# revdotcom/reverb

Hardware: AMD Instinct MI355X
Metric: RTFx (audio-sec/wall-sec) Reverb-ASR attention_rescoring (higher is better)
Workload: dtype bf16

## Files before the change

reverb_amd/_lib.py:

```python
from __future__ import annotations

import ctypes as C
import os

_HERE = os.path.dirname(os.path.abspath(__file__))
LIB_PATH = os.path.join(_HERE, "librvb.so")

RVB_F32, RVB_BF16, RVB_FP8 = 0, 1, 2
ACT_NONE, ACT_SILU, ACT_RELU = 0, 1, 2
NORM_LN, NORM_AFFINE = 0, 1


class RvbError(RuntimeError):
    pass


class AudioInfo(C.Structure):
    _fields_ = [("container", C.c_int32), ("sample_format", C.c_int32), ("channels", C.c_int32), ("sample_rate", C.c_int32),
                ("bits_per_sample", C.c_int32), ("md5_checked", C.c_int32), ("frames", C.c_int64), ("decode_threads", C.c_int32),
                ("reserved", C.c_int32)]


class _SizedCfg(C.Structure):

# ... 51 lines not shown
    "rvb_audio_decode_i16": (C.c_int64, [C.c_void_p, C.c_int64, C.c_int, _i16p, C.c_int64, C.c_int, C.POINTER(AudioInfo)]),
    "rvb_fbank": (C.c_int, [_eng, _f32p, _i64p]),
    "rvb_encode": (C.c_int, [_eng, _f32p, C.c_int64, _i32p, C.c_int, C.c_int, C.c_int, C.c_float]),
    "rvb_stream_begin": (C.c_int, [_eng]),
    "rvb_stream_chunk": (C.c_int, [_eng, _f32p, C.c_int, C.c_int, _f32p, _i32p]),
    "rvb_stream_state": (C.c_int, [_eng, _i32p, _i32p]),
    "rvb_stream_finish": (C.c_int, [_eng, C.c_int, C.c_float]),
    "rvb_encoder_frames": (C.c_int, [_eng, _i32p]),
    "rvb_get_encoder_lens": (C.c_int, [_eng, _i32p]),
    "rvb_get_encoder_out": (C.c_int, [_eng, _f32p]),
    "rvb_get_ctc_logprobs": (C.c_int, [_eng, C.c_int, _f32p]),
    "rvb_set_encoder_tap": (C.c_int, [_eng, C.c_int]),
    "rvb_get_encoder_tap": (C.c_int, [_eng, C.c_char_p, _f32p, C.c_int64]),
    "rvb_get_ctc_topk": (C.c_int, [_eng, _f32p, _i32p]),
    "rvb_ctc_greedy": (C.c_int, [_eng, _i32p, _i32p, _i32p]),
    "rvb_ctc_align": (C.c_int, [_eng, _i32p, _i32p, C.c_int, _i32p, _i32p, _i32p, _i32p, _i32p, _i32p, _f32p, _f32p]),
    "rvb_ctc_align_wild": (C.c_int, [_eng, _i32p, _i32p, C.c_int, _i32p, _i32p, C.c_float, _i32p, _i32p, _i32p, _i32p, _f32p, _f32p]),
    "rvb_ctc_align_limits": (C.c_int, [_i32p, _i32p]),
    "rvb_ctc_align_graph": (C.c_int, [_eng, _i32p, _i32p, _i32p, _i32p, _u8p, C.c_int, _i32p, _i32p, C.c_float, _i32p, _i32p, _i32p, _i32p,
                                      _i32p, _i32p, _i32p, _f32p, _f32p]),
    "rvb_ctc_align_graph_limits": (C.c_int, [_i32p, _i32p, _i32p, _i32p]),
    "rvb_ctc_score": (C.c_int, [_eng, _i32p, _i32p, C.c_int, _i32p, _i32p, _f64p, _f32p, _f32p, _f32p, _i32p]),
    "rvb_ctc_score_graph": (C.c_int, [_eng, _i32p, _i32p, _i32p, _i32p, _u8p, C.c_int, _i32p, _i32p, _f64p, _f32p, _f32p, _f32p, _f32p,
                                      _i32p]),
    "rvb_ctc_find": (C.c_int, [_eng, _i32p, _i32p, C.c_int, _f32p, _i32p, _i32p, C.c_int, C.c_int, C.c_int, _i32p, _i32p, _i32p, _f32p,
                               _i64p]),
    "rvb_ctc_prefix_beam": (C.c_int, [_eng, C.c_int]),
    "rvb_set_context_graph": (C.c_int, [_eng, _i32p, _i32p, C.c_int, C.c_double]),
    "rvb_get_nbest_count": (C.c_int, [_eng, C.c_int, _i32p, _i32p]),
    "rvb_get_nbest": (C.c_int, [_eng, C.c_int, _i32p, _i32p, _i32p, _i32p, _f64p]),
    "rvb_prepare_rescoring": (C.c_int, [_eng, C.c_int]),
    "rvb_attention_rescore": (C.c_int, [_eng, C.c_double, C.c_double]),
    "rvb_attention_score": (C.c_int, [_eng, _i32p, _i32p, C.c_int, _i32p, C.c_double, C.c_double, _f64p, _f64p, _i32p, _i32p, _f32p, _f32p,
                                      _i32p]),
    "rvb_attention_decode": (C.c_int, [_eng, C.c_int, C.c_float]),
    "rvb_get_attention_result": (C.c_int, [_eng, C.c_int, _i32p, _i32p, _f32p]),
    "rvb_get_rescored": (C.c_int, [_eng, C.c_int, _i32p, _f32p, _f64p, _f64p]),
    "rvb_get_rescored_batch": (C.c_int, [_eng, _i32p, _i32p, _i32p, _i32p, _f32p, _f64p, _f64p]),
    "rvb_fp8_recalibrate": (C.c_int, [_eng]),
    "rvb_get_fp8_scales": (C.c_int, [_eng, _f32p, _i32p]),
    "rvb_set_fp8_scales": (C.c_int, [_eng, _f32p, C.c_int32]),
    "rvb_get_fp8_saturation": (C.c_int, [_eng, C.POINTER(C.c_uint32), _i32p, C.c_int]),
    "rvb_get_fp8_subsample": (C.c_int, [_eng, C.POINTER(C.c_float), C.POINTER(C.c_uint32), C.c_int]),
    "rvb_get_rescore_stats": (C.c_int, [_eng, _i64p, _i64p]),
    "rvb_get_rescore_logp": (C.c_int, [_eng, C.c_int, C.c_int, C.c_int, _f32p]),
    "rvb_comm_unique_id": (C.c_int, [C.c_void_p]),
    "rvb_comm_init": (C.c_int, [_eng, C.c_int, C.c_int, C.c_void_p]),
    "rvb_comm_create": (C.c_int, [C.c_int, C.c_int, C.c_int, C.c_void_p, C.POINTER(C.c_void_p)]),
    "rvb_comm_allgather": (C.c_int, [C.c_void_p, C.c_void_p, C.c_int64, C.c_void_p]),
    "rvb_comm_time_allgather": (C.c_int, [C.c_void_p, C.c_int64, C.c_int, C.POINTER(C.c_double)]),
    "rvb_comm_set_timeout": (C.c_int, [C.c_void_p, C.c_double]),
    "rvb_comm_barrier": (C.c_int, [C.c_void_p]),
    "rvb_comm_max_f64": (C.c_int, [C.c_void_p, C.POINTER(C.c_double)]),
    "rvb_comm_allgather_topk": (C.c_int, [C.c_void_p, _eng, C.c_void_p, _i64p]),
    "rvb_comm_free": (C.c_int, [C.c_void_p]),
    "rvb_allgather_results": (C.c_int, [_eng, C.c_void_p, C.c_int64, C.c_void_p]),
    "rvb_comm_destroy": (C.c_int, [_eng]),
    "rvb_set_profiling": (C.c_int, [_eng, C.c_int]),
    "rvb_reset_timings": (C.c_int, [_eng]),
    "rvb_get_timing": (C.c_int, [_eng, C.c_char_p, _f64p, _f64p, _i64p]),
    "rvb_get_timing_bytes": (C.c_int, [_eng, C.c_char_p, _f64p]),
    "rvb_wer_counts": (C.c_int, [_i32p, C.c_int64, _i32p, C.c_int64, _i64p]),
}

class AttnTestArgs(C.Structure):
    _fields_ = ([(n, C.c_int32) for n in ("dtype", "heads", "dk", "nseq")] +
                [f for b in ("q", "k", "v", "out") for f in ((b, _f32p), (b[0] + "_rows", C.c_int32), (b[0] + "_stride", C.c_int32),
                                                             (b[0] + "_col", C.c_int32), ("pad_" + b, C.c_int32))] +
                [("p", _f32p), ("p_rows", C.c_int32), ("p_stride", C.c_int32), ("p_col", C.c_int32), ("p_off", C.c_int32),
                 ("bias_u", _f32p), ("bias_v", _f32p)] +
                [(n, _i32p) for n in ("q_start", "q_len", "kv_start", "kv_len", "q_pos0", "kv_index", "work")] +
                [(n, C.c_int32) for n in ("n_index", "n_work", "max_q", "q_block", "causal", "chunk", "left", "plain_order", "fold",
                                          "k_prefolded", "fold_kv_cap", "lab")] +
                [("ran", C.c_int32 * 8)])


class NormTestArgs(C.Structure):
    _fields_ = ([(n, C.c_int32) for n in ("dtype", "x_bf16", "mode", "silu", "out_f32", "out_fp8", "out2_fp8", "M", "d", "pad0")] +
                [(n, C.c_float) for n in ("eps", "eps2", "out_scale", "out2_scale")] +
                [(n, _f32p) for n in ("x", "gamma", "beta", "add", "gamma2", "beta2", "out", "out2")] +
                [("sat", C.c_uint32), ("sat2", C.c_uint32)])


class GemmTestArgs(C.Structure):
    _fields_ = ([(n, C.c_int32) for n in ("dtype", "M", "N", "K", "lda", "ldw", "ldc", "ldres", "act", "out_f32", "out_fp8", "in_fp8",
                                          "inplace", "a_row0", "c_rows", "conv", "cT1", "cF1", "cC", "cB")] +
                [(n, C.c_float) for n in ("alpha", "a_scale", "out_scale")] +
                [("path", C.c_int32), ("a_elems", C.c_int64)] +
                [(n, _f32p) for n in ("A", "W", "bias", "res", "C", "a_deq", "w_deq")])


_u32p = C.POINTER(C.c_uint32)

TEST_SIGNATURES = {
    "rvb_test_gemm_ex": (C.c_int, [C.POINTER(GemmTestArgs)]),
    "rvb_test_rownorm_ex": (C.c_int, [C.POINTER(NormTestArgs)]),
    "rvb_test_conv1_ex": (C.c_int, [C.c_int, _f32p, _f32p, _f32p, _f32p, _f32p, _f32p, C.c_int, C.c_int, C.c_int, C.c_int, C.c_float,
                                    _f32p, _u32p]),
    "rvb_test_embed": (C.c_int, [_f32p, C.c_int, _f32p, C.c_int, _i32p, _i32p, _f32p, C.c_int, C.c_int, C.c_float]),
    "rvb_test_amax_abs": (C.c_int, [C.c_int, _f32p, C.c_int64, _f32p]),
    "rvb_test_convert_f32": (C.c_int, [C.c_int, _f32p, _f32p, C.c_int64]),
    "rvb_test_gather_cache": (C.c_int, [C.c_void_p, C.c_void_p, _i32p, C.c_int, C.c_int, C.c_int, C.c_int]),
    "rvb_test_gather_pairs": (C.c_int, [_f32p, C.c_int, C.c_int64, _i32p, _i32p, C.c_int, _f32p]),
    "rvb_test_gemm": (C.c_int, [C.c_int, _f32p, _f32p, _f32p, _f32p, _f32p, C.c_int, C.c_int, C.c_int, C.c_float,
                                C.c_int, C.c_int, C.c_int, C.c_int, C.c_int, C.c_int, C.c_int]),
    "rvb_test_rownorm": (C.c_int, [C.c_int, _f32p, _f32p, _f32p, C.c_float, C.c_int, C.c_int, _f32p, _f32p, C.c_int,
                                   C.c_int, C.c_int]),
    "rvb_test_conv_block32": (C.c_int, [_f32p, _f32p, _f32p, _f32p, _f32p, _f32p, C.c_int, C.c_int, C.c_int]),
    "rvb_test_conv_s2sc": (C.c_int, [_f32p, _f32p, _f32p, _f32p, _f32p, _f32p, _f32p, C.c_int, C.c_int, C.c_int]),
    "rvb_test_conv1": (C.c_int, [C.c_int, _f32p, _f32p, _f32p, _f32p, _f32p, _f32p, C.c_int, C.c_int, C.c_int, C.c_int]),
    "rvb_test_conv_igemm_fp8": (C.c_int, [_f32p, _f32p, _f32p, _f32p, _f32p, _f32p, C.c_int, C.c_int, C.c_int, C.c_int, C.c_int, C.c_int, C.c_int,
                                           C.c_float, C.c_float, _f32p, _f32p, _f32p]),
    "rvb_test_joint_new": (C.c_void_p, [C.c_int, C.c_int, C.c_int, C.c_int, C.c_double, C.c_double, C.c_double]),
    "rvb_test_joint_free": (None, [C.c_void_p]),
    "rvb_test_joint_begin": (C.c_int, [C.c_void_p, C.c_int, _f32p, _i32p, C.c_int, C.c_float, C.c_float, _i32p, _i32p, _i32p, _i32p, _i32p,
                                       C.c_int]),
    "rvb_test_joint_finish": (C.c_int, [C.c_void_p, _f32p]),
    "rvb_test_joint_prefix": (C.c_int, [C.c_void_p, C.c_int, _i32p, _i32p]),
    "rvb_test_joint_result": (C.c_int, [C.c_void_p, _i32p, _i32p, _i32p, _f64p, _i32p, _f64p]),
    "rvb_test_glu_dwconv": (C.c_int, [C.c_int, _f32p, _f32p, _f32p, _f32p, _i32p, _f32p, C.c_int, C.c_int, C.c_int,
                                      C.c_int, C.c_int, _f32p, C.c_int]),
    "rvb_test_attention": (C.c_int, [C.c_int, _f32p, _f32p, _f32p, _f32p, _f32p, _f32p, _f32p, C.c_int, C.c_int,
                                     C.c_int, C.c_int, C.c_int, _i32p, _i32p, _i32p, _i32p, C.c_int, C.c_int]),
    "rvb_test_attention_trie": (C.c_int, [C.c_int, _f32p, _f32p, _f32p, _f32p, C.c_int, C.c_int, C.c_int, _i32p, _i32p, _i32p,
                                          _i32p, _i32p, _i32p, C.c_int, C.c_int, C.c_int]),
    "rvb_test_attention_ex": (C.c_int, [C.POINTER(AttnTestArgs)]),
    "rvb_test_attention_pos_bias": (C.c_int, [_f32p, C.c_int, C.c_int, C.c_int, C.c_int, _f32p, _f32p, C.c_int, C.c_int, C.c_float, _f32p]),
    "rvb_test_logsoftmax_topk": (C.c_int, [_f32p, C.c_int, C.c_int, C.c_int, C.c_float, C.c_int, _f32p, _i32p, _f32p]),
    "rvb_test_lse_gather": (C.c_int, [_f32p, C.c_int, C.c_int, _i32p, _f32p]),
    "rvb_test_logsoftmax_topk_ex": (C.c_int, [_f32p, C.c_int, C.c_int, C.c_int, C.c_int, C.c_float, C.c_int, _f32p, _i32p, _f32p]),
    "rvb_test_lse_gather_ex": (C.c_int, [_f32p, C.c_int, C.c_int, C.c_int, _i32p, C.c_float, C.c_int, _f32p]),
    "rvb_test_lse_gather_multi_ex": (C.c_int, [_f32p, C.c_int, C.c_int, C.c_int, _i32p, _i32p, _f32p]),
    "rvb_test_ctc_viterbi": (C.c_int, [_f32p, C.c_int, C.c_int, _i32p, C.c_int, C.c_int, C.c_int, _i32p, _f32p]),
    "rvb_test_ctc_viterbi_wild": (C.c_int, [_f32p, C.c_int, C.c_int, _f32p, C.c_float, _i32p, C.c_int, C.c_int, C.c_int, _i32p, _f32p]),
    "rvb_test_ctc_viterbi_graph": (C.c_int, [_f32p, _i32p, C.c_int, C.c_int, _f32p, C.c_float, _i32p, _i32p, _i32p, _i32p, _u8p, C.c_int,
                                             C.c_int, _i32p, _i32p, _f32p]),
    "rvb_test_ctc_score": (C.c_int, [_f32p, C.c_int, C.c_int, _i32p, C.c_int, C.c_int, C.c_int, _f64p, _f32p, _f32p, _f32p, _i32p]),
    "rvb_test_ctc_score_graph": (C.c_int, [_f32p, _i32p, C.c_int, C.c_int, _i32p, _i32p, _i32p, _i32p, _u8p, C.c_int, C.c_int, _f64p, _f32p,
                                           _f32p, _f32p, _f32p, _i32p]),
    "rvb_test_ctc_score_batch": (C.c_int, [_f32p, _i32p, C.c_int, _i32p, _i32p, C.c_int, C.c_int, C.c_int, _f64p, _f32p, _f32p, _f32p,
                                           _i32p]),
    "rvb_test_ctc_find": (C.c_int, [_f32p, _i32p, C.c_int, C.c_int, _f32p, _i32p, _i32p, C.c_int, _f32p, C.c_int, C.c_int, C.c_int, C.c_int,
                                    _i64p, _i32p, _i32p, _f32p, _i32p, _i32p, _i32p, _f32p]),
    "rvb_test_slab_windows": (C.c_int, [C.c_char_p, _i32p, _i32p, C.c_int, _i32p, C.c_int, C.c_int, _i32p, _i32p, _i32p, _i32p, _i32p]),
    "rvb_test_gemm_glu": (C.c_int, [_f32p, _f32p, _f32p, _f32p, C.c_int, C.c_int, C.c_int]),
    "rvb_test_gemm_rowadd": (C.c_int, [_f32p, _f32p, _f32p, _f32p, _f32p, C.c_int, C.c_int, C.c_int, C.c_int, C.c_int, C.c_int]),
    "rvb_test_mp3_decode": (C.c_int64, [C.c_char_p, C.c_int64, C.c_int, _f32p, C.c_int64, _i64p, _i64p, C.c_int]),
    "rvb_test_mp3_hybrid": (C.c_int, [_f32p, _f32p, C.c_int, C.c_int, _f32p]),
    "rvb_test_mp3_polyphase": (C.c_int, [_f32p, _f32p, _i32p, _f32p]),
    "rvb_test_mp3_window": (C.c_int, [_f32p]),
    "rvb_test_mp3_huffman": (C.c_int, [C.c_int, C.POINTER(C.c_uint16), C.POINTER(C.c_uint8), _i32p]),
    "rvb_test_gemm_fp8": (C.c_int, [_f32p, _f32p, _f32p, _f32p, _f32p, C.c_int, C.c_int, C.c_int, C.c_float, C.c_float, C.c_int, C.c_int,
                                    C.c_float, _f32p, _f32p]),
    "rvb_test_rownorm_fp8": (C.c_int, [_f32p, _f32p, _f32p, C.c_float, C.c_int, C.c_int, C.c_int, C.c_float, _f32p, _f32p, _f32p,
                                       C.c_float, C.c_float, _f32p, _f32p]),
    "rvb_test_lse_gather_multi": (C.c_int, [_f32p, C.c_int, C.c_int, _i32p, _i32p, C.c_int, _f32p]),
    "rvb_test_row_xent": (C.c_int, [_f32p, C.c_int, C.c_int, C.c_int, _i32p, _i32p, _f32p, _f32p, _f64p, _i32p]),
    "rvb_test_host_pool": (C.c_int, [C.c_int, C.c_int, C.c_int]),
    "rvb_test_build_trie": (C.c_int, [_i32p, _i32p, _i32p, C.c_int, C.c_int, C.c_int, C.c_int, C.c_int, _i32p, _i32p, _i32p, _i32p, _i32p, _i32p,
                                      _i32p, _i32p, _i32p, _i32p, _i32p]),
    "rvb_test_fbank": (C.c_int, [_i16p, C.c_int64, _f32p]),
    "rvb_test_fbank_ex": (C.c_int, [_i16p, _f32p, C.c_int64, _f32p]),
    "rvb_test_fbank_batch": (C.c_int, [C.POINTER(C.c_void_p), _i32p, _i64p, _i64p, C.c_int, C.c_int, _f32p]),
    "rvb_test_set_gemm_variant": (C.c_int, [C.c_int]),
    "rvb_test_set_gemm2_opts": (C.c_int, [C.c_int, C.c_int]),
    "rvb_test_gemm_timeline": (C.c_int, [C.c_int] * 6 + [C.POINTER(C.c_longlong), C.c_int, _i32p]),
    "rvb_test_gemm_bench": (C.c_int, [C.c_int, C.c_int, C.c_int, C.c_int, C.c_int, C.c_int, C.c_int, C.c_int, C.c_int,
                                      _f64p, _f64p]),
    "rvb_test_prefix_beam": (C.c_int, [_f32p, _i32p, C.c_int, C.c_int, C.c_int, _i32p, _i32p, _i32p, _i32p, _i32p,
                                       _f64p]),
    "rvb_test_prefix_beam_context": (C.c_int, [_f32p, _i32p, C.c_int, C.c_int, C.c_int, C.c_int, _i32p, _i32p, C.c_int, C.c_double,
                                               _i32p, _i32p, _i32p, _i32p, _i32p, _f64p, _f64p]),
    "rvb_test_context_walk": (C.c_int, [_i32p, _i32p, C.c_int, C.c_double, C.c_int, C.c_int, _i32p, C.c_int, _i32p, _f64p, _i32p,
                                        _f64p]),
    "rvb_test_window_stats": (C.c_int, [_f32p, C.c_int64, C.c_int64, C.c_int, C.c_int64, C.c_int, C.c_float, _f32p]),
    "rvb_test_sinc_conv": (C.c_int, [C.c_int, _f32p, C.c_int64, _f32p, C.c_int, C.c_int, C.c_int, C.c_int64, _f32p]),
    "rvb_test_pool_norm": (C.c_int, [C.c_int, C.c_int, _f32p, C.c_int, C.c_int, C.c_int, C.c_int, C.c_int, _f32p, _f32p, C.c_float,
                                     C.c_int, _f32p, C.c_int64, C.c_int64, C.c_int, _f32p, _f32p, C.c_float, C.c_float, _f32p]),
    "rvb_test_conv1d5": (C.c_int, [C.c_int, _f32p, C.c_int64, _f32p, _f32p, _f32p, C.c_int64]),
# ... 124 lines not shown
```

reverb_amd/csrc/common.h:

```cpp
#pragma once
#include <hip/hip_runtime.h>
#include <math.h>
#include <stdint.h>
#include <stdio.h>
#include <string>

namespace rvb {

typedef uint16_t bf16_t;

typedef __attribute__((ext_vector_type(8))) __bf16 bf16x8_t;
typedef __attribute__((ext_vector_type(4))) float f32x4_t;

__host__ __device__ inline float bf16_to_f32(bf16_t v) {
  union { uint32_t u; float f; } x;
  x.u = ((uint32_t)v) << 16;
  return x.f;
}
__host__ __device__ inline bf16_t f32_to_bf16(float f) {
#if defined(__HIP_DEVICE_COMPILE__)
  const __bf16 r = (__bf16)f;
  return __builtin_bit_cast(bf16_t, r);
#else
  union { uint32_t u; float f; } x;
// ... 38 lines not shown
  }
  int M = (int)nearbyintf((m * 2.f - 1.f) * 8.f);
  if (M == 8) { M = 0; E += 1; }
  if (E > 15 || (E == 15 && M == 7)) return sgn | 0x7e;
  return sgn | (uint8_t)((E << 3) | M);
}
__host__ __device__ inline float fp8_to_f32_host(uint8_t b) {
  const int E = (b >> 3) & 15, M = b & 7;
  const float v = E == 0 ? ldexpf((float)M, -9) : ldexpf(1.f + M / 8.f, E - 7);
  return (b & 0x80) ? -v : v;
}

template <typename T> struct Cvt;
template <> struct Cvt<float> {
  __host__ __device__ static inline float to_f32(float v) { return v; }
  __host__ __device__ static inline float from_f32(float v) { return v; }
};
template <> struct Cvt<fp8_t> {
  __host__ __device__ static inline float to_f32(fp8_t v) { return fp8_to_f32_host(v); }
  __host__ __device__ static inline fp8_t from_f32(float v) { return f32_to_fp8_host(v); }
};
template <> struct Cvt<bf16_t> {
  __host__ __device__ static inline float to_f32(bf16_t v) { return bf16_to_f32(v); }
  __host__ __device__ static inline bf16_t from_f32(float v) { return f32_to_bf16(v); }
};

template <typename T> struct Mma16;
template <> struct Mma16<bf16_t> {
  static constexpr int KC = 32;
  static constexpr int VE = 8;
  __device__ static inline void run(const uint4& a, const uint4& b, f32x4_t& c) {
    union U { uint4 u; bf16x8_t v; };
    U ua, ub;
    ua.u = a; ub.u = b;
    c = __builtin_amdgcn_mfma_f32_16x16x32_bf16(ua.v, ub.v, c, 0, 0, 0);
  }
};
template <> struct Mma16<float> {
  static constexpr int KC = 16;
  static constexpr int VE = 4;
  __device__ static inline void run(const uint4& a, const uint4& b, f32x4_t& c) {
    c = __builtin_amdgcn_mfma_f32_16x16x4f32(__uint_as_float(a.x), __uint_as_float(b.x), c, 0, 0, 0);
    c = __builtin_amdgcn_mfma_f32_16x16x4f32(__uint_as_float(a.y), __uint_as_float(b.y), c, 0, 0, 0);
    c = __builtin_amdgcn_mfma_f32_16x16x4f32(__uint_as_float(a.z), __uint_as_float(b.z), c, 0, 0, 0);
    c = __builtin_amdgcn_mfma_f32_16x16x4f32(__uint_as_float(a.w), __uint_as_float(b.w), c, 0, 0, 0);
  }
};

__device__ inline float wave_sum(float v) {
#pragma unroll
  for (int o = 32; o > 0; o >>= 1) v += __shfl_xor(v, o, 64);
  return v;
}
__device__ inline float wave_max(float v) {
#pragma unroll
  for (int o = 32; o > 0; o >>= 1) v = fmaxf(v, __shfl_xor(v, o, 64));
  return v;
}

__device__ inline float rows_max(float v) {
  auto a = __builtin_amdgcn_permlane16_swap(__float_as_uint(v), __float_as_uint(v), false, false);
  v = fmaxf(__uint_as_float(a[0]), __uint_as_float(a[1]));
  auto b = __builtin_amdgcn_permlane32_swap(__float_as_uint(v), __float_as_uint(v), false, false);
  return fmaxf(__uint_as_float(b[0]), __uint_as_float(b[1]));
}
__device__ inline float rows_sum(float v) {
  auto a = __builtin_amdgcn_permlane16_swap(__float_as_uint(v), __float_as_uint(v), false, false);
  v = __uint_as_float(a[0]) + __uint_as_float(a[1]);
  auto b = __builtin_amdgcn_permlane32_swap(__float_as_uint(v), __float_as_uint(v), false, false);
  return __uint_as_float(b[0]) + __uint_as_float(b[1]);
}

template <int CTRL> __device__ inline float dpp_f32(float v) {
  return __uint_as_float(__builtin_amdgcn_update_dpp(0u, __float_as_uint(v), CTRL, 0xf, 0xf, false));
}
__device__ inline float wave_sum_dpp(float v) {
  v += dpp_f32<0xB1>(v);
  v += dpp_f32<0x4E>(v);
  v += dpp_f32<0x141>(v);
  v += dpp_f32<0x140>(v);
  return rows_sum(v);
}

inline int cdiv(int64_t a, int64_t b) { return (int)((a + b - 1) / b); }

enum { OK = 0, E_ARG = -1, E_HIP = -2, E_STATE = -3, E_NOMEM = -4, E_UNSUPPORTED = -5, E_TIMEOUT = -7  };

}

#define RVB_HIP_CHECK(expr)                                                             \
  do {                                                                                  \
    hipError_t _e = (expr);                                                             \
    if (_e != hipSuccess) {                                                             \
      rvb::set_error(std::string(#expr) + ": " + hipGetErrorString(_e));                \
      return rvb::E_HIP;                                                                \
    }                                                                                   \
  } while (0)

#define RVB_TRY(expr) do { int _r = (expr); if (_r != rvb::OK) return _r; } while (0)

namespace rvb {
void set_error(const std::string& msg);
const char* last_error();
const char* lab_env(const char* name);
}
```

reverb_amd/csrc/elementwise.hip:

```cpp
#include <algorithm>

#include "common.h"
#include "kernels.h"

namespace rvb {

static constexpr int CONV1_ROWS = 4;

template <typename T>
__global__ __launch_bounds__(256) void conv1_kernel(const float* __restrict__ feats, const float* __restrict__ mean,
                                                    const float* __restrict__ istd, const float* __restrict__ w,
                                                    const float* __restrict__ bias, T* __restrict__ out, int T0,
                                                    int F0, int T1, int F1, int d, float inv_scale, unsigned* __restrict__ amax,
                                                    unsigned* __restrict__ sat) {
  extern __shared__ float s_in[];
  const int t1_0 = blockIdx.x * CONV1_ROWS, b = blockIdx.y;
  const int nrow = min(CONV1_ROWS, T1 - t1_0);
  for (int i = threadIdx.x; i < (2 * nrow + 1) * F0; i += 256) {
    const int kh = i / F0, f = i - kh * F0;
    s_in[i] = (feats[((size_t)b * T0 + 2 * t1_0 + kh) * F0 + f] - mean[f]) * istd[f];
  }
  __syncthreads();
  const int ncg = d >> 3;
  const int per = ncg < 256 ? ncg : 256;
// ... 18 lines not shown
      for (int f1 = fslot; f1 < F1; f1 += nslots) {
        float xin[9];
#pragma unroll
        for (int kh = 0; kh < 3; ++kh)
#pragma unroll
          for (int kw = 0; kw < 3; ++kw) xin[kh * 3 + kw] = in[kh * F0 + 2 * f1 + kw];
        float o[8];
        if constexpr (sizeof(T) == 4) {
#pragma unroll
          for (int c = 0; c < 8; ++c) {
            float acc = br[c];
#pragma unroll
            for (int k = 0; k < 9; ++k) acc += wr[c][k] * xin[k];
            o[c] = fmaxf(acc, 0.f);
          }
        } else {
          typedef float c1_f32x2 __attribute__((ext_vector_type(2)));
#pragma unroll
          for (int c = 0; c < 8; c += 2) {
            c1_f32x2 acc = {br[c], br[c + 1]};
#pragma unroll
            for (int k = 0; k < 9; ++k) acc = __builtin_elementwise_fma((c1_f32x2){wr[c][k], wr[c + 1][k]}, (c1_f32x2){xin[k], xin[k]}, acc);
            o[c] = fmaxf(acc.x, 0.f); o[c + 1] = fmaxf(acc.y, 0.f);
          }
        }
        T* dst = orow + (size_t)f1 * d + cg * 8;
        if (amax) {
#pragma unroll
          for (int c = 0; c < 8; ++c) vmax = fmaxf(vmax, o[c]);
        }
        if constexpr (sizeof(T) == 1) {
#pragma unroll
          for (int c = 0; c < 8; ++c) o[c] *= inv_scale;
          if (sat) nclip += fp8_clipped(o[0], o[1], o[2], o[3]) + fp8_clipped(o[4], o[5], o[6], o[7]);
          *(uint2*)dst = make_uint2(pack4_fp8(o[0], o[1], o[2], o[3]), pack4_fp8(o[4], o[5], o[6], o[7]));
        } else if constexpr (sizeof(T) == 2) {
          *(uint4*)dst = make_uint4(pack2_bf16(o[0], o[1]), pack2_bf16(o[2], o[3]), pack2_bf16(o[4], o[5]), pack2_bf16(o[6], o[7]));
        } else {
          ((float4*)dst)[0] = make_float4(o[0], o[1], o[2], o[3]);
          ((float4*)dst)[1] = make_float4(o[4], o[5], o[6], o[7]);
        }
      }
    }
  }
  if (amax) {
    vmax = wave_max(vmax);
    if ((threadIdx.x & 63) == 0 && vmax > 0.f) atomicMax(amax, __float_as_uint(vmax));
  }
  if (sat && nclip) atomicAdd(sat, nclip);
}

int subsample_conv1(hipStream_t s, int dtype, const float* feats, const float* mean, const float* istd,
                    const float* w, const float* b, void* out, int B, int T0, int F0, int d, float out_fp8_scale, unsigned* amax,
                    unsigned* sat) {
  const int T1 = (T0 - 3) / 2 + 1, F1 = (F0 - 3) / 2 + 1;
  if (B <= 0 || T1 <= 0) return OK;
  if (d % 8) { set_error("subsample_conv1: d must be a multiple of 8"); return E_ARG; }
  dim3 grid(cdiv(T1, CONV1_ROWS), B);
  const size_t sh = (2 * CONV1_ROWS + 1) * F0 * sizeof(float);
  if (out_fp8_scale > 0.f) {
    if (dtype != DT_BF16) { set_error("subsample_conv1: fp8 output belongs to the bf16 engine"); return E_ARG; }
    hipLaunchKernelGGL(conv1_kernel<fp8_t>, grid, dim3(256), sh, s, feats, mean, istd, w, b, (fp8_t*)out, T0, F0, T1, F1, d,
                       1.f / out_fp8_scale, (unsigned*)nullptr, sat);
  } else if (dtype == DT_BF16)
    hipLaunchKernelGGL(conv1_kernel<bf16_t>, grid, dim3(256), sh, s, feats, mean, istd, w, b, (bf16_t*)out, T0, F0, T1, F1, d, 1.f, amax,
                       (unsigned*)nullptr);
  else
    hipLaunchKernelGGL(conv1_kernel<float>, grid, dim3(256), sh, s, feats, mean, istd, w, b, (float*)out, T0, F0, T1, F1, d, 1.f, amax,
                       (unsigned*)nullptr);
  RVB_HIP_CHECK(hipGetLastError());
  return OK;
}

template <int NV>
__device__ inline float sq4(float dx, float dy, float dz, float dw) {
  if constexpr (NV == 4) {
#pragma clang fp contract(off)
    return dx * dx + dy * dy + dz * dz + dw * dw;
  } else {
    return fmaf(dw, dw, fmaf(dz, dz, fmaf(dx, dx, dy * dy)));
  }
}

template <typename OutT, typename AddT, int NV, bool TWO, int SW>
__global__ __launch_bounds__(256, (NV <= 4 ? 4 : 2)) void rownorm_kernel(NormArgs a) {
  constexpr bool CT = SW >= 0;
  auto wsum = [](float x) __attribute__((always_inline)) { if constexpr (sizeof(AddT) == 2) return wave_sum_dpp(x); else return wave_sum(x); };
  const bool sw_xb = CT ? (bool)(SW & 1) : (bool)a.x_bf16;
  const bool sw_ln = CT ? (bool)(SW & 2) : a.mode == NORM_LN;
  const bool sw_silu = CT ? (bool)(SW & 4) : (bool)a.silu;
  const bool sw_add = CT ? (bool)(SW & 8) : a.add != nullptr;
  const bool sw_o2f8 = CT ? (bool)(SW & 16) : (bool)a.out2_fp8;
  const int lane = threadIdx.x & 63;
  const int d = a.d;
  const int wave0 = blockIdx.x * 4 + (threadIdx.x >> 6), nwaves = gridDim.x * 4;
#define COL(i) ((((lane) + 64 * ((i) >> 1)) << 3) + (((i) & 1) << 2))
  float4 g[NV], be[NV], g2[TWO ? NV : 1], be2[TWO ? NV : 1];
#pragma unroll
  for (int i = 0; i < NV; ++i) {
    const int c = COL(i);
    const bool ok = c < d;
    g[i] = ok ? *(const float4*)(a.gamma + c) : make_float4(0.f, 0.f, 0.f, 0.f);
    be[i] = ok ? *(const float4*)(a.beta + c) : make_float4(0.f, 0.f, 0.f, 0.f);
    if constexpr (TWO) {
      g2[i] = ok ? *(const float4*)(a.gamma2 + c) : make_float4(0.f, 0.f, 0.f, 0.f);
      be2[i] = ok ? *(const float4*)(a.beta2 + c) : make_float4(0.f, 0.f, 0.f, 0.f);
    }
  }
  auto load_row = [&](int row, float4* v) {
    const int rr = min(row, a.M - 1);
    const bool rok = row < a.M;
    if (sw_xb) {
      const bf16_t* x = (const bf16_t*)a.x + (size_t)rr * d;
#pragma unroll
      for (int i = 0; i < NV; ++i) {
        const int c = COL(i);
        const uint2 u = *(const uint2*)(x + min(c, d - 4));
        const bool ok = rok && c < d;
        v[i] = make_float4(ok ? bf16_to_f32((bf16_t)(u.x & 0xffffu)) : 0.f, ok ? bf16_to_f32((bf16_t)(u.x >> 16)) : 0.f,
                           ok ? bf16_to_f32((bf16_t)(u.y & 0xffffu)) : 0.f, ok ? bf16_to_f32((bf16_t)(u.y >> 16)) : 0.f);
      }
      return;
    }
    const float* x = a.x + (size_t)rr * d;
#pragma unroll
    for (int i = 0; i < NV; ++i) {
      const int c = COL(i);
      const float4 u = *(const float4*)(x + min(c, d - 4));
      const bool ok = rok && c < d;
      v[i] = make_float4(ok ? u.x : 0.f, ok ? u.y : 0.f, ok ? u.z : 0.f, ok ? u.w : 0.f);
    }
  };
  float4 v[NV], nx[NV];
  unsigned nsat = 0, nsat2 = 0;
  load_row(wave0, v);
  for (int row = wave0; row < a.M; row += nwaves) {
    load_row(row + nwaves, nx);
    float mean = 0.f, rstd = 1.f;
    if (sw_ln) {
      float sum = 0.f;
#pragma unroll
      for (int i = 0; i < NV; ++i) sum += v[i].x + v[i].y + v[i].z + v[i].w;
      mean = wsum(sum) / (float)d;
      float sq = 0.f;
#pragma unroll
      for (int i = 0; i < NV; ++i) {
        if (COL(i) < d) {
          sq += sq4<NV>(v[i].x - mean, v[i].y - mean, v[i].z - mean, v[i].w - mean);
        }
      }
      rstd = rsqrtf(wsum(sq) / (float)d + a.eps);
    }
    if constexpr (CT) {
#pragma unroll
      for (int i = 0; i < NV; ++i)
        asm volatile("" : "+v"(nx[i].x), "+v"(nx[i].y), "+v"(nx[i].z), "+v"(nx[i].w), "+v"(rstd));
    }
    OutT* out = (OutT*)a.out + (size_t)row * d;
    const AddT* add = sw_add ? (const AddT*)a.add + (size_t)row * d : nullptr;
    float sum2 = 0.f;
#pragma unroll
    for (int i = 0; i < NV; ++i) {
      const int c = COL(i);
      if (c >= d) continue;
      float o[4] = {(v[i].x - mean) * rstd * g[i].x + be[i].x, (v[i].y - mean) * rstd * g[i].y + be[i].y,
                    (v[i].z - mean) * rstd * g[i].z + be[i].z, (v[i].w - mean) * rstd * g[i].w + be[i].w};
      if (sw_silu) {
#pragma unroll
        for (int e = 0; e < 4; ++e) {
          if constexpr (sizeof(OutT) <= 2) o[e] = o[e] * __builtin_amdgcn_rcpf(1.0f + __builtin_amdgcn_exp2f(-1.44269504f * o[e]));
          else o[e] = o[e] / (1.0f + expf(-o[e]));
        }
      }
      if (add) {
        if constexpr (sizeof(AddT) == 2) {
          const uint2 u = *(const uint2*)(add + c);
          o[0] += bf16_to_f32((bf16_t)(u.x & 0xffffu)); o[1] += bf16_to_f32((bf16_t)(u.x >> 16));
          o[2] += bf16_to_f32((bf16_t)(u.y & 0xffffu)); o[3] += bf16_to_f32((bf16_t)(u.y >> 16));
        } else {
          const float4 u = *(const float4*)(add + c);
          o[0] += u.x; o[1] += u.y; o[2] += u.z; o[3] += u.w;
        }
      }
      if constexpr (sizeof(OutT) == 4) *(float4*)(out + c) = make_float4(o[0], o[1], o[2], o[3]);
      v[i] = make_float4(o[0], o[1], o[2], o[3]);
      sum2 += o[0] + o[1] + o[2] + o[3];
    }
    if constexpr (sizeof(OutT) <= 2) {
#pragma unroll
      for (int i = 0; i < NV; i += 2) {
        const int c = COL(i);
        if (c >= d) continue;
        if constexpr (sizeof(OutT) == 1) {
          const float qs = a.out_inv_scale;
          nsat += fp8_clipped(v[i].x * qs, v[i].y * qs, v[i].z * qs, v[i].w * qs) + fp8_clipped(v[i + 1].x * qs, v[i + 1].y * qs, v[i + 1].z * qs, v[i + 1].w * qs);
          *(uint2*)(out + c) = make_uint2(pack4_fp8(v[i].x * qs, v[i].y * qs, v[i].z * qs, v[i].w * qs),
                                          pack4_fp8(v[i + 1].x * qs, v[i + 1].y * qs, v[i + 1].z * qs, v[i + 1].w * qs));
        } else {
          *(uint4*)(out + c) = make_uint4(pack2_bf16(v[i].x, v[i].y), pack2_bf16(v[i].z, v[i].w),
                                          pack2_bf16(v[i + 1].x, v[i + 1].y), pack2_bf16(v[i + 1].z, v[i + 1].w));
        }
      }
    }
    if constexpr (TWO) {
      const float mean2 = wsum(sum2) / (float)d;
      float sq = 0.f;
#pragma unroll
      for (int i = 0; i < NV; ++i) {
        if (COL(i) < d) {
          sq += sq4<NV>(v[i].x - mean2, v[i].y - mean2, v[i].z - mean2, v[i].w - mean2);
        }
      }
      const float rstd2 = rsqrtf(wsum(sq) / (float)d + a.eps2);
      AddT* o2 = (AddT*)a.out2 + (size_t)row * d;
#pragma unroll
      for (int i = 0; i < NV; i += 2) {
        const int c = COL(i);
        if (c >= d) continue;
        float q[8];
#pragma unroll
        for (int h = 0; h < 2; ++h) {
          q[4 * h + 0] = (v[i + h].x - mean2) * rstd2 * g2[i + h].x + be2[i + h].x;
          q[4 * h + 1] = (v[i + h].y - mean2) * rstd2 * g2[i + h].y + be2[i + h].y;
          q[4 * h + 2] = (v[i + h].z - mean2) * rstd2 * g2[i + h].z + be2[i + h].z;
          q[4 * h + 3] = (v[i + h].w - mean2) * rstd2 * g2[i + h].w + be2[i + h].w;
        }
        if (sw_o2f8) {
          const float qs = a.out2_inv_scale;
          nsat2 += fp8_clipped(q[0] * qs, q[1] * qs, q[2] * qs, q[3] * qs) + fp8_clipped(q[4] * qs, q[5] * qs, q[6] * qs, q[7] * qs);
          *(uint2*)((fp8_t*)a.out2 + (size_t)row * d + c) = make_uint2(pack4_fp8(q[0] * qs, q[1] * qs, q[2] * qs, q[3] * qs),
                                                                       pack4_fp8(q[4] * qs, q[5] * qs, q[6] * qs, q[7] * qs));
        } else if constexpr (sizeof(AddT) == 2) {
          *(uint4*)(o2 + c) = make_uint4(pack2_bf16(q[0], q[1]), pack2_bf16(q[2], q[3]), pack2_bf16(q[4], q[5]), pack2_bf16(q[6], q[7]));
        } else {
          *(float4*)(o2 + c) = make_float4(q[0], q[1], q[2], q[3]);
          *(float4*)(o2 + c + 4) = make_float4(q[4], q[5], q[6], q[7]);
        }
      }
    }
#pragma unroll
    for (int i = 0; i < NV; ++i) v[i] = nx[i];
  }
  if (nsat != 0 && a.sat) atomicAdd(a.sat, nsat);
  if (nsat2 != 0 && a.sat2) atomicAdd(a.sat2, nsat2);
#undef COL
}

template <typename OutT, typename AddT>
static void launch_rownorm(hipStream_t s, const NormArgs& a) {
  const int blocks = std::min(cdiv(a.M, 4), 256 * 8);
  const int sw = (a.x_bf16 ? 1 : 0) | (a.mode == NORM_LN ? 2 : 0) | (a.silu ? 4 : 0) | (a.add ? 8 : 0) | (a.out2_fp8 ? 16 : 0);
  if (a.d > 512 && a.d <= 1024) {
#define RVB_NORM_CASE(TWO_, SW_) \
    if ((a.out2 != nullptr) == (TWO_) && sw == (SW_)) { hipLaunchKernelGGL((rownorm_kernel<OutT, AddT, 4, TWO_, SW_>), dim3(blocks), dim3(256), 0, s, a); return; }
    RVB_NORM_CASE(false, 2)
    RVB_NORM_CASE(false, 2 | 4 | 1)
    RVB_NORM_CASE(false, 4 | 1)
    RVB_NORM_CASE(false, 2 | 4)
    RVB_NORM_CASE(false, 4)
    RVB_NORM_CASE(true, 2)
    RVB_NORM_CASE(true, 2 | 8)
    RVB_NORM_CASE(true, 2 | 16)
    RVB_NORM_CASE(true, 2 | 8 | 16)
#undef RVB_NORM_CASE
  }
  if (a.out2) {
    if (a.d <= 512) hipLaunchKernelGGL((rownorm_kernel<OutT, AddT, 2, true, -1>), dim3(blocks), dim3(256), 0, s, a);
    else if (a.d <= 1024) hipLaunchKernelGGL((rownorm_kernel<OutT, AddT, 4, true, -1>), dim3(blocks), dim3(256), 0, s, a);
    else hipLaunchKernelGGL((rownorm_kernel<OutT, AddT, 8, true, -1>), dim3(blocks), dim3(256), 0, s, a);
  } else {
    if (a.d <= 512) hipLaunchKernelGGL((rownorm_kernel<OutT, AddT, 2, false, -1>), dim3(blocks), dim3(256), 0, s, a);
    else if (a.d <= 1024) hipLaunchKernelGGL((rownorm_kernel<OutT, AddT, 4, false, -1>), dim3(blocks), dim3(256), 0, s, a);
    else hipLaunchKernelGGL((rownorm_kernel<OutT, AddT, 8, false, -1>), dim3(blocks), dim3(256), 0, s, a);
  }
}

int rownorm(hipStream_t s, int dtype, const NormArgs& a) {
  if (a.M <= 0) return OK;
  if (a.d % 8 || a.d > 2048) { set_error("rownorm: d must be a multiple of 8 and <= 2048"); return E_ARG; }
  if (a.x_bf16 && dtype != DT_BF16) { set_error("rownorm: bf16 input belongs to the bf16 engine"); return E_ARG; }
  if (a.out2 && (a.mode != NORM_LN || !(a.out_f32 || dtype == DT_F32))) {
    set_error("rownorm: the fused second LayerNorm follows a LayerNorm with fp32 output"); return E_ARG;
  }
  if ((a.out_fp8 || a.out2_fp8) && dtype != DT_BF16) { set_error("rownorm: fp8 outputs belong to the bf16 engine"); return E_ARG; }
  if (dtype == DT_BF16) {
    if (a.out_fp8) launch_rownorm<fp8_t, bf16_t>(s, a);
    else if (a.out_f32) launch_rownorm<float, bf16_t>(s, a);
    else launch_rownorm<bf16_t, bf16_t>(s, a);
  } else {
    launch_rownorm<float, float>(s, a);
  }
  RVB_HIP_CHECK(hipGetLastError());
  return OK;
}

static constexpr int DW_TT = 128, DW_CT = 128, DW_KMAX = 31, DW_THREADS = 512;

template <typename T> struct Gate;
template <> struct Gate<float> {
  typedef float2 pair_t;
  __device__ static inline float put(float v) { return v; }
  __device__ static inline void get(pair_t p, float& x, float& y) { x = p.x; y = p.y; }
};
template <> struct Gate<bf16_t> {
  typedef uint32_t pair_t;
  __device__ static inline bf16_t put(float v) { return f32_to_bf16(v); }
  __device__ static inline void get(pair_t p, float& x, float& y) { x = __uint_as_float(p << 16); y = __uint_as_float(p & 0xffff0000u); }
};

template <typename T>
__global__ __launch_bounds__(DW_THREADS) void glu_dw_kernel(GluDwArgs a) {
  typedef decltype(Gate<T>::put(0.f)) S;
  constexpr int rows = DW_TT + DW_KMAX - 1;
  __shared__ __attribute__((aligned(16))) S s_g[rows][DW_CT];
  const int c = threadIdx.x & 63, slot = threadIdx.x >> 6;
  const int t0 = blockIdx.x * DW_TT, c0 = blockIdx.y * DW_CT, b = blockIdx.z;
  const int ch = c0 + 2 * c;
  const bool cok = ch < a.d;
  const int K = a.K, pad = a.causal ? K - 1 : (K - 1) / 2;
  const int len = a.lens[b];
  const int lorder = K - 1;
  const T* G = (const T*)a.G;
  const bool gated = a.gated != 0;
  const size_t gstride = gated ? (size_t)a.d : (size_t)2 * a.d;
  typedef float f32x2_t __attribute__((ext_vector_type(2)));
  f32x2_t wk[DW_KMAX];
#pragma unroll
  for (int k = 0; k < DW_KMAX; ++k)
    wk[k] = (k < K && cok) ? *(const f32x2_t*)(a.dw_w + (size_t)k * a.d + ch) : (f32x2_t){0.f, 0.f};
  constexpr int VE = 16 / (int)sizeof(T);
  constexpr int NG = DW_CT / VE;
  const bool vec_ok = (a.d % VE) == 0;
  if (vec_ok) {
    constexpr int ITEMS_ALL = (rows * NG + DW_THREADS - 1) / DW_THREADS;
    constexpr int ITEMS = 3;
#pragma unroll
    for (int it0 = 0; it0 < ITEMS_ALL; it0 += ITEMS) {
    uint4 ra[ITEMS], rb[ITEMS];
#pragma unroll
    for (int it = 0; it < ITEMS; ++it) {
      const int v = min((int)threadIdx.x + (it0 + it) * DW_THREADS, rows * NG - 1);
      const int r = v / NG, grp = v - r * NG;
      const int t = t0 - pad + r;
      const int cg = min(c0 + grp * VE, a.d - VE);
      const bool from_hist = a.causal && t < 0 && t >= -a.hist_rows;
      const T* gr = from_hist ? (const T*)a.hist + (size_t)(lorder + t) * 2 * a.d
                              : G + ((size_t)b * a.T + min(max(t, 0), a.T - 1)) * gstride;
      ra[it] = *(const uint4*)(gr + cg);
      rb[it] = gated ? make_uint4(0, 0, 0, 0) : *(const uint4*)(gr + a.d + cg);
    }
#pragma unroll
    for (int it = 0; it < ITEMS; ++it) {
      const int v = threadIdx.x + (it0 + it) * DW_THREADS;
      if (v >= rows * NG) break;
      const int r = v / NG, grp = v - r * NG;
      const int t = t0 - pad + r;
      const int cg = c0 + grp * VE;
      float g[VE];
#pragma unroll
      for (int e = 0; e < VE; ++e) g[e] = 0.f;
      const bool from_hist = a.causal && t < 0 && t >= -a.hist_rows;
      if (cg < a.d && (t >= 0 || a.causal) && t < a.T && r < DW_TT + K - 1) {
        if ((t >= 0 && t < len) || from_hist) {
          T av[VE], bvv[VE];
          *(uint4*)av = ra[it];
          *(uint4*)bvv = rb[it];
#pragma unroll
// ... 181 lines not shown
```

reverb_amd/csrc/engine.h:

```cpp
#pragma once
#include <condition_variable>
#include <functional>
#include <map>
#include <memory>
#include <mutex>
#include <string>
#include <thread>
#include <vector>

#include "../../include/rvb.h"
#include "ctc_slabs.h"
#include "kernels.h"
#include "search.h"

namespace rvb {

struct HostTensor {
  std::vector<float> data;
  std::vector<int64_t> shape;
  size_t numel() const { size_t n = 1; for (auto s : shape) n *= (size_t)s; return n; }
};

struct DevBuf {
  void* p = nullptr;
// ... 167 lines not shown
  std::vector<uint8_t> h_fin;
  DevBuf d_rem, d_csum, d_loglik, d_llhat, d_coff, d_arows, d_beta, d_acc, d_succ_off, d_succs, d_fin;
  int plan(const char* who, const int32_t* node_tokens, const int32_t* n_nodes, const int32_t* pred_off, const int32_t* preds,
           const uint8_t* is_final, int n_seq, const std::vector<std::vector<int32_t>>& seq_rows, int V, int blank_id, bool posteriors);
  int begin(hipStream_t s);
  int advance(hipStream_t s, const float* lp, int ld, int r0, int nrows);
  int finish_forward(hipStream_t s, double* loglik );
  int advance_backward(hipStream_t s, const float* lp, int ld, int r0, int nrows);
  int finish_backward(hipStream_t s, float* visit, float* occupancy, float* mean_frame, float* peak_post, int32_t* peak_frame );
  void release();
};

struct CtcFinder {
  std::vector<FindSeq> seq;
  std::vector<FindPhrase> phr;
  std::vector<int32_t> h_tokens, h_rows;
  int blank = 0, max_cand = 0;
  DevBuf d_tokens, d_rows, d_seqs, d_phr, d_h, d_st, d_count, d_cend, d_cstart, d_cscore;
  int plan(const char* who, const int32_t* tokens, const int32_t* tok_lens, int n_phrases, const float* threshold,
           const std::vector<std::vector<int32_t>>& seq_rows, int V, int blank_id, int max_candidates);
  int begin(hipStream_t s);
  bool touches(int r0, int nrows) const { return slab_touches(seq, h_rows, r0, nrows); }
  int advance(hipStream_t s, const float* lp, int ld, int r0, int nrows, const float* wmax);
  int finish(hipStream_t s, int max_hits, int32_t* n_hits, int32_t* start, int32_t* end, float* score, int64_t* n_candidates,
             int32_t* raw_end = nullptr, int32_t* raw_start = nullptr, float* raw_score = nullptr);
  void release();
};

}

struct rvb_engine {
  rvb_model_cfg cfg;
  int device = 0;
  int dtype = 0;
  bool fp8 = false;
  int f8_state = 0;
  std::vector<rvb::F8Scales> f8;
  std::vector<unsigned> f8_groups;
  rvb::DevBuf d_amax;
  bool f8_conv2 = false;
  float f8_x1 = 0.f;
  rvb::DevBuf d_f8sat;
  hipStream_t stream = nullptr;
  bool finalized = false;

  std::map<std::string, rvb::HostTensor> host;

  rvb::DevBuf cmvn_mean, cmvn_istd, conv1_w, conv1_b;
  rvb::Linear conv2, embed_out, ctc;
  rvb::LNorm enc_after;
  std::vector<rvb::EncLayer> enc;
  rvb::Decoder dec_l, dec_r;
  rvb::DevBuf pe_f32;
  int pe_rows = 0;
  rvb::DevBuf fb_window, fb_twiddle, fb_melw, fb_lo, fb_hi;
  rvb::DevBuf stage;

  rvb::DevBuf pcm, feats;
  rvb::DevBuf pcm_next;
  hipStream_t copy_stream = nullptr;
  hipEvent_t pcm_ready = nullptr, pcm_free = nullptr;
  bool pcm_pending = false;
  int64_t n_samples_next = 0;
  rvb::DevBuf wave_f32, rs_kernel;
  rvb::DevBuf wave_in;
  bool pcm_is_float = false;
  int dec_chunk = 0, dec_left = -1;
  int64_t n_samples = 0, n_frames = 0, feat_rows = 0;
  bool batch = false;
  std::vector<int64_t> batch_n, batch_src;
  std::vector<int32_t> batch_is_float;
  std::vector<int64_t> h_frame0;
  std::vector<rvb::FbankRec> h_rec;
  rvb::DevBuf d_frame0, d_rec;
  int feat_kind = 0;
  bool packed = false;
  int64_t packed_rows = 0;
  rvb::DevBuf feats_packed, pc_loud, pc_rec, pc_frame0, pc_table, pc_count, pc_pieces;

  int B = 0, T0 = 0, T1 = 0, F1 = 0, T2 = 0, F2 = 0, beam = 0;
  std::vector<int32_t> in_lens, enc_lens;
  rvb::DevBuf d_feats_in, X1, X2, x, xn, y, h, ao, dconv, enc_out, logits, topv, topi;
  rvb::DevBuf d_enc_lens, d_seq_start, d_seq_len, d_aux_i32;
  float* h_topv = nullptr;
  int32_t* h_topi = nullptr;
  size_t h_top_cap = 0;
  struct Slice { int c0, nb; hipEvent_t ev; bool done; };
  std::vector<Slice> slices;
  std::vector<hipEvent_t> slice_event_pool;
  int xattn_max_rows = 0;
  const int* cur_lens = nullptr;
  std::vector<rvb::PrefixResult> nbest;
  std::shared_ptr<const rvb::ContextGraph> context_graph;
  std::vector<rvb::RescoreResult> rescored;
  std::vector<rvb::TrieBatch> trie_l;
  rvb::HostPool pool;
  std::vector<rvb::JointResult> joint;
  std::vector<rvb::DevBuf> jkv;
  rvb::DevBuf jlogp, jpair_row, jpair_tok, jpair_out;
  int64_t joint_rows = 0, joint_steps = 0;
  float last_blank_penalty = 0.f;
  std::vector<std::vector<int>> attn_tokens;
  std::vector<float> attn_scores;
  rvb::DevBuf atopv, atopi;
  std::vector<rvb::DevBuf> kcache, vcache, kcache2, vcache2, memkv;
  rvb::DevBuf dx, dxn, dy, dh, dqkv, dq, dao, kvmem, d_tok, d_pos, d_tgt, d_logp;
  rvb::DevBuf d_hq_start, d_hq_len, d_hkv_start, d_hkv_len;
  rvb::DevBuf d_hq_pos0, d_hpath_start, d_hpath_len, d_path, d_work, d_tgt_ptr;
  int64_t rescore_rows = 0, rescore_pairs = 0;
  rvb::DevBuf d_xlse, d_xsum, d_xtop;

  struct StreamState {
    bool active = false;
    int offset = 0;
    int cache_len = 0;
    std::vector<rvb::DevBuf> kv, kv2;
    int cnn_rows = 0;
    std::vector<rvb::DevBuf> cnn, cnn2;
  } stream_st;
  rvb::DevBuf d_stream_i32;

  int tap_block = -1;
  bool tap_live = false;
  struct Tap { rvb::DevBuf buf; size_t elems = 0; bool bf16 = false; };
  std::map<std::string, Tap> taps;
  std::vector<float> tap_forms;

  rvb::CtcAligner aligner;
  rvb::CtcScorer scorer;
  rvb::CtcFinder finder;
  rvb::CtcGraphAligner graph_aligner;
  rvb::CtcGraphScorer graph_scorer;
  rvb::DevBuf align_lp, align_tv, align_ti, align_row, align_col, align_out;

  void* comm = nullptr;
  int comm_world = 1, comm_rank = 0;
  rvb::DevBuf comm_send, comm_recv;

  int profiling = 0;
  std::map<std::string, rvb::ProfEntry> prof;
  struct Pending { hipEvent_t a, b; std::string name; };
  std::vector<Pending> pending;
  std::vector<hipEvent_t> event_pool;
};
```

reverb_amd/csrc/engine.hip:

```cpp
#include "engine_impl.h"

#include <algorithm>
#include <cmath>
#include <cstdlib>
#include <cstring>

namespace rvb {

static thread_local std::string g_err;
void set_error(const std::string& msg) { g_err = msg; }
const char* last_error() { return g_err.c_str(); }

int DevBuf::ensure(size_t n) {
  if (n <= bytes && p) return OK;
  if (p) { (void)hipFree(p); p = nullptr; bytes = 0; }
  if (n == 0) n = 16;
  hipError_t err = hipMalloc(&p, n);
  if (err != hipSuccess) {
    p = nullptr;
    (void)hipGetLastError();
    set_error("hipMalloc of " + std::to_string(n) + " bytes failed: " + hipGetErrorString(err));
    return E_NOMEM;
  }
  bytes = n;
  return OK;
}
void DevBuf::release() { if (p) (void)hipFree(p); p = nullptr; bytes = 0; }

static void drain_prof(rvb_engine* e) {
  if (e->pending.empty()) return;
  (void)hipStreamSynchronize(e->stream);
  for (auto& p : e->pending) {
    float ms = 0.f;
    (void)hipEventElapsedTime(&ms, p.a, p.b);
    e->prof[p.name].ms += ms;
    e->event_pool.push_back(p.a); e->event_pool.push_back(p.b);
  }
  e->pending.clear();
}

int upload_f32(rvb_engine* e, DevBuf& dst, const float* src, size_t n) {
  RVB_TRY(dst.ensure(n * 4));
  RVB_HIP_CHECK(hipMemcpyAsync(dst.p, src, n * 4, hipMemcpyHostToDevice, e->stream));
  return OK;
}
int upload_i32(rvb_engine* e, DevBuf& dst, const int32_t* src, size_t n) {
  RVB_TRY(dst.ensure(n * 4 + 16));
  if (n) RVB_HIP_CHECK(hipMemcpyAsync(dst.p, src, n * 4, hipMemcpyHostToDevice, e->stream));
  return OK;
}

const AttnArgs& with_lab(AttnArgs& a) { attention_lab_switches(a); return a; }

int reset_f8sat(rvb_engine* e) {
  static const int on = lab_env("RVB_FP8_SAT") ? atoi(lab_env("RVB_FP8_SAT")) : 1;
  if (!on) return OK;
  RVB_TRY(e->d_f8sat.ensure((e->enc.size() + 1) * 8 * 4));
  RVB_HIP_CHECK(hipMemsetAsync(e->d_f8sat.p, 0, (e->enc.size() + 1) * 8 * 4, e->stream));
  return OK;
}

double gemm_alg_bytes(const rvb_engine* e, const GemmArgs& g) {
  const double es = g.in_fp8 ? 1.0 : (double)dt_size(e->dtype);
  const double a = g.conv ? (double)(g.M / (g.cT2 * g.cF2)) * g.cT1 * g.cF1 * g.cC * es : (double)g.M * g.K * es;
  const double c = (double)g.M * (g.act == ACT_GLU ? g.N / 2 : g.N) * (g.out_fp8 ? 1.0 : (g.out_f32 ? 4.0 : (double)dt_size(e->dtype)));
  return a + (double)g.N * g.K * es + (g.bias ? 4.0 * g.N : 0.0) + c + (g.res ? 4.0 * (double)g.M * g.N : 0.0);
}

int run_gemm(rvb_engine* e, const void* A, int lda, const Linear& L, void* C, int ldc, int M, bool out_f32, float alpha,
             int act, const float* res, int ldres) {
  GemmArgs g;
  memset(&g, 0, sizeof(g));
  g.A = A; g.W = L.w.p; g.bias = L.b.as<float>(); g.res = res; g.C = C;
  g.M = M; g.N = L.out; g.K = L.in; g.lda = lda; g.ldw = L.in; g.ldc = ldc; g.ldres = ldres;
  g.alpha = alpha; g.act = act; g.out_f32 = out_f32 ? 1 : 0;
  Scope sc(e, "gemm", 2.0 * M * (double)L.out * L.in, gemm_alg_bytes(e, g));
  const int rc = gemm(e->stream, e->dtype, g);
  tap_note_gemm(e);
  return rc;
}
int tap_keep(rvb_engine* e, const char* name, const void* src, size_t elems, bool is_bf16) {
  if (!e->tap_live) return OK;
  auto& t = e->taps[name];
  const size_t bytes = elems * (is_bf16 ? 2 : 4);
  RVB_TRY(t.buf.ensure(bytes));
  t.elems = elems; t.bf16 = is_bf16;
  RVB_HIP_CHECK(hipMemcpyAsync(t.buf.p, src, bytes, hipMemcpyDeviceToDevice, e->stream));
  return OK;
}
void tap_note_gemm(rvb_engine* e) {
  if (e->tap_live) e->tap_forms.push_back((float)gemm_last_path());
}
int run_norm(rvb_engine* e, const float* x, const LNorm& n, void* out, bool out_f32, int M, int d, int mode,
             int silu, const void* add, const LNorm* second, void* out2, float out8, float out2_8, bool x_bf16, unsigned* sat,
             unsigned* sat2) {
  NormArgs a;
  a.sat = sat; a.sat2 = sat2;
  a.x_bf16 = x_bf16 ? 1 : 0;
  a.x = x; a.gamma = n.g.as<float>(); a.beta = n.b.as<float>(); a.eps = n.eps; a.mode = mode; a.silu = silu;
  a.add = add; a.out = out; a.out_f32 = out_f32 ? 1 : 0; a.M = M; a.d = d;
  if (second) { a.gamma2 = second->g.as<float>(); a.beta2 = second->b.as<float>(); a.eps2 = second->eps; a.out2 = out2; }
  if (out8 > 0.f) { a.out_fp8 = 1; a.out_inv_scale = 1.f / out8; }
  if (out2_8 > 0.f) { a.out2_fp8 = 1; a.out2_inv_scale = 1.f / out2_8; }
  Scope sc(e, "rownorm");
  return rownorm(e->stream, e->dtype, a);
}
int run_gemm8(rvb_engine* e, const void* A8, int lda, const Linear& L, void* C, int ldc, int M, float a_scale, int out_kind,
              float out_scale, float alpha, int act, const float* res, int ldres, unsigned* sat) {
  GemmArgs g;
  memset(&g, 0, sizeof(g));
  g.sat = sat;
  g.A = A8; g.W = L.w8.p; g.bias = L.b.as<float>(); g.res = res; g.C = C;
  g.M = M; g.N = L.out; g.K = L.in; g.lda = lda; g.ldw = L.in; g.ldc = ldc; g.ldres = ldres;
  g.alpha = alpha; g.act = act; g.out_f32 = out_kind == 1; g.out_fp8 = out_kind == 2; g.in_fp8 = 1;
  g.a_scale = a_scale; g.w_scale = L.wscale.as<float>(); g.out_inv_scale = 1.f / out_scale;
  if (!L.w8.p) { set_error("fp8 GEMM on a layer without fp8 weights"); return E_STATE; }
  Scope sc(e, "gemm_fp8", 2.0 * M * (double)L.out * L.in, gemm_alg_bytes(e, g));
  return gemm(e->stream, e->dtype, g);
}

void attention_lab_switches(AttnArgs& a) {
  static const int sw[2] = {
      (lab_env("RVB_ATTN_OCC") && atoi(lab_env("RVB_ATTN_OCC")) == 3 ? ATTN_LAB_OCC3 : 0) |
          (lab_env("RVB_ATTN_MF") && atoi(lab_env("RVB_ATTN_MF")) == 0 ? ATTN_LAB_MF1 : 0) |
          (lab_env("RVB_ATTN_PADK") && atoi(lab_env("RVB_ATTN_PADK")) == 16 ? ATTN_LAB_PADK16 : 0),
      lab_env("RVB_ATTN_PLAIN") ? atoi(lab_env("RVB_ATTN_PLAIN")) : 0};
  a.lab |= sw[0];
  if (sw[1]) a.plain_order = 1;
}

static int drop_pending_upload(rvb_engine* e) {
  if (e->pcm_pending) {
    RVB_HIP_CHECK(hipStreamSynchronize(e->copy_stream));
    e->pcm_pending = false;
  }
  return OK;
}

static int resample_uploaded(rvb_engine* e, bool src_float, int64_t n, int sample_rate) {
  const int target = 16000;
  std::vector<float> ker;
  int orig, nw, width, K;
  resample_taps(sample_rate, target, &ker, &orig, &nw, &width, &K);
  const int64_t n_out = (nw * n + orig - 1) / orig;
  RVB_TRY(e->rs_kernel.ensure(ker.size() * 4));
  RVB_TRY(e->wave_f32.ensure((size_t)std::max<int64_t>(n_out, 1) * 4));
  RVB_HIP_CHECK(hipMemcpyAsync(e->rs_kernel.p, ker.data(), ker.size() * 4, hipMemcpyHostToDevice, e->stream));
  {
    Scope sc(e, "resample");
    if (src_float) RVB_TRY(resample_f32(e->stream, e->wave_in.as<float>(), n, e->rs_kernel.as<float>(), orig, nw, width, K, e->wave_f32.as<float>(), n_out));
    else RVB_TRY(resample(e->stream, e->pcm.as<int16_t>(), n, e->rs_kernel.as<float>(), orig, nw, width, K, e->wave_f32.as<float>(), n_out));
  }
  RVB_HIP_CHECK(hipStreamSynchronize(e->stream));
  e->n_samples = n_out;
  e->pcm_is_float = true;
  e->batch = false;
  return OK;
}

static void fill_nbest(const PrefixResult& pr, int ml, int32_t* tokens, int32_t* lens, int32_t* times, int32_t* times_lens, double* scores) {
  for (size_t i = 0; i < pr.nbest.size(); ++i) {
    if (lens) lens[i] = (int32_t)pr.nbest[i].size();
    if (times_lens) times_lens[i] = (int32_t)pr.times[i].size();
    if (scores) scores[i] = pr.scores[i];
    for (int j = 0; j < ml; ++j) {
      if (tokens) tokens[i * ml + j] = j < (int)pr.nbest[i].size() ? pr.nbest[i][j] : -1;
      if (times) times[i * ml + j] = j < (int)pr.times[i].size() ? pr.times[i][j] : -1;
    }
  }
}

}

using namespace rvb;

extern "C" {

const char* rvb_last_error(void) { return last_error(); }
const char* rvb_version(void) { return "librvb 0.1 (gfx950)"; }

int rvb_model_cfg_size(void) { return (int)sizeof(rvb_model_cfg); }

int rvb_wer_counts(const int32_t* ref, int64_t n_ref, const int32_t* hyp, int64_t n_hyp, int64_t* counts) {
  if ((!ref && n_ref > 0) || (!hyp && n_hyp > 0) || !counts || n_ref < 0 || n_hyp < 0) { set_error("rvb_wer_counts: bad argument"); return E_ARG; }
  edit_counts(ref, n_ref, hyp, n_hyp, counts);
  return OK;
}

int rvb_create(const rvb_model_cfg* cfg, int device, rvb_engine** out) {
  if (!cfg || !out) { set_error("rvb_create: null argument"); return E_ARG; }
  if (cfg->struct_size != (int32_t)sizeof(rvb_model_cfg)) {
    set_error("rvb_create: ABI mismatch: rvb_model_cfg.struct_size is " + std::to_string(cfg->struct_size) + ", this library's struct has " +
              std::to_string(sizeof(rvb_model_cfg)) + " bytes (bind it field by field from include/rvb.h)");
    return E_ARG;
  }
  if (cfg->dtype != RVB_F32 && cfg->dtype != RVB_BF16 && cfg->dtype != RVB_FP8) { set_error("rvb_create: bad dtype"); return E_ARG; }
  if (cfg->d_model <= 0 || cfg->heads <= 0 || cfg->d_model % cfg->heads || cfg->d_model % 8 || cfg->ffn_dim % 8 ||
      cfg->dec_ffn_dim % 8 || cfg->input_dim != 80 || cfg->vocab < 2 || cfg->num_blocks < 1 ||
      cfg->cnn_kernel < 1 || cfg->cnn_kernel > 31 || (!cfg->cnn_causal && (cfg->cnn_kernel % 2) == 0) ||
      cfg->chunk_frames < 7 || cfg->max_chunks < 1 ||
      (cfg->dec_blocks > 0 && (cfg->dec_heads <= 0 || cfg->d_model % cfg->dec_heads))) {
    set_error("rvb_create: unsupported model dimensions (need d, ffn dims % 8 == 0, d % heads == 0, input_dim 80, cnn kernel <= 31 and odd unless causal)");
    return E_ARG;
  }
  int ndev = 0;
  hipError_t err = hipGetDeviceCount(&ndev);
  if (err != hipSuccess || ndev <= 0) { set_error("no HIP device available: librvb has no CPU fallback"); return E_HIP; }
  if (device < 0 || device >= ndev) { set_error("rvb_create: device index out of range"); return E_ARG; }
  RVB_HIP_CHECK(hipSetDevice(device));
  rvb_engine* e = new rvb_engine();
  e->cfg = *cfg; e->device = device;
  e->fp8 = cfg->dtype == RVB_FP8;
  e->dtype = e->fp8 ? (int)DT_BF16 : cfg->dtype;
  hipError_t se = hipStreamCreateWithFlags(&e->stream, hipStreamNonBlocking);
  if (se != hipSuccess) { delete e; set_error("hipStreamCreate failed"); return E_HIP; }
  *out = e;
  return OK;
}

void rvb_destroy(rvb_engine* e) {
  if (!e) return;
  (void)rvb_comm_destroy(e);
  (void)hipSetDevice(e->device);
  (void)hipStreamSynchronize(e->stream);
  DevBuf* bufs[] = {&e->cmvn_mean, &e->cmvn_istd, &e->conv1_w, &e->conv1_b, &e->pe_f32, &e->stage, &e->pcm, &e->feats,
                    &e->d_feats_in, &e->X1, &e->X2, &e->x, &e->xn, &e->y, &e->h, &e->ao, &e->dconv, &e->enc_out,
                    &e->logits, &e->topv, &e->topi, &e->d_enc_lens, &e->d_seq_start, &e->d_seq_len, &e->d_aux_i32,
                    &e->dx, &e->dxn, &e->dy, &e->dh, &e->dqkv, &e->dq, &e->dao, &e->kvmem, &e->d_tok, &e->d_pos,
                    &e->d_tgt, &e->d_logp, &e->d_hq_start, &e->d_hq_len, &e->d_hkv_start, &e->d_hkv_len,
                    &e->d_hq_pos0, &e->d_hpath_start, &e->d_hpath_len, &e->d_path, &e->d_work, &e->d_tgt_ptr,
                    &e->fb_window, &e->fb_twiddle, &e->fb_melw, &e->fb_lo, &e->fb_hi,
                    &e->conv2.w, &e->conv2.b, &e->embed_out.w, &e->embed_out.b, &e->ctc.w, &e->ctc.b,
                    &e->enc_after.g, &e->enc_after.b};
  for (DevBuf* b : bufs) b->release();
  e->aligner.release();
  e->graph_aligner.release();
  e->graph_scorer.release();
  e->finder.release();
  e->scorer.release();
  for (DevBuf* b : {&e->align_lp, &e->align_tv, &e->align_ti, &e->align_row, &e->align_col, &e->align_out}) b->release();
  e->d_xlse.release(); e->d_xsum.release(); e->d_xtop.release();
  e->atopv.release(); e->atopi.release(); e->d_stream_i32.release(); e->d_amax.release(); e->d_f8sat.release();
  e->wave_f32.release(); e->wave_in.release(); e->rs_kernel.release(); e->d_frame0.release(); e->d_rec.release();
  for (DevBuf* b : {&e->feats_packed, &e->pc_loud, &e->pc_rec, &e->pc_frame0, &e->pc_table, &e->pc_count, &e->pc_pieces}) b->release();
  e->jlogp.release(); e->jpair_row.release(); e->jpair_tok.release(); e->jpair_out.release();
  for (auto& b : e->jkv) b.release();
  for (auto* v : {&e->stream_st.kv, &e->stream_st.kv2, &e->stream_st.cnn, &e->stream_st.cnn2}) for (auto& b : *v) b.release();
  for (auto* v : {&e->kcache, &e->vcache, &e->kcache2, &e->vcache2, &e->memkv}) for (auto& b : *v) b.release();
  auto rel_lin = [](Linear& l) { l.w.release(); l.b.release(); l.w8.release(); l.wscale.release(); };
  auto rel_n = [](LNorm& n) { n.g.release(); n.b.release(); };
  for (auto& L : e->enc) {
    for (Linear* l : {&L.ffm1, &L.ffm2, &L.ff1, &L.ff2, &L.qkv, &L.att_out, &L.pw1, &L.pw1_glu, &L.pw2, &L.lsl}) rel_lin(*l);
    for (LNorm* n : {&L.n_ffm, &L.n_mha, &L.n_conv, &L.n_ff, &L.n_final, &L.n_cnn}) rel_n(*n);
    L.pos_keys.release(); L.pos_bias.release(); L.bias_u.release(); L.bias_v.release(); L.dw_w.release(); L.dw_b.release();
  }
  for (Decoder* D : {&e->dec_l, &e->dec_r}) {
    D->embed.release(); rel_lin(D->out); rel_n(D->after);
    for (auto& L : D->layers) {
      for (Linear* l : {&L.self_qkv, &L.self_out, &L.src_q, &L.src_kv, &L.src_out, &L.ff1, &L.ff2, &L.lsl}) rel_lin(*l);
      for (LNorm* n : {&L.n1, &L.n2, &L.n3}) rel_n(*n);
      L.kvmem.release();
    }
  }
  if (e->h_topv) (void)hipHostFree(e->h_topv);
  if (e->h_topi) (void)hipHostFree(e->h_topi);
  for (auto& sl : e->slices) if (!sl.done) (void)hipEventDestroy(sl.ev);
  for (auto ev : e->slice_event_pool) (void)hipEventDestroy(ev);
  for (auto& p : e->pending) { (void)hipEventDestroy(p.a); (void)hipEventDestroy(p.b); }
  for (auto ev : e->event_pool) (void)hipEventDestroy(ev);
  if (e->copy_stream) (void)hipStreamDestroy(e->copy_stream);
  if (e->pcm_ready) (void)hipEventDestroy(e->pcm_ready);
  if (e->pcm_free) (void)hipEventDestroy(e->pcm_free);
  e->pcm_next.release();
  for (auto& t : e->taps) t.second.buf.release();
  (void)hipStreamDestroy(e->stream);
  delete e;
}

int rvb_load_tensor(rvb_engine* e, const char* name, const float* host, const int64_t* shape, int ndim) {
  if (!e || !name || !host || ndim < 0 || (ndim > 0 && !shape)) { set_error("rvb_load_tensor: null argument"); return E_ARG; }
  HostTensor t;
  size_t n = 1;
  for (int i = 0; i < ndim; ++i) { if (shape[i] < 0) { set_error("negative dim"); return E_ARG; } t.shape.push_back(shape[i]); n *= (size_t)shape[i]; }
  t.data.assign(host, host + n);
  e->host[name] = std::move(t);
  return OK;
}

int rvb_finalize(rvb_engine* e, const float* cat_embs, int n_cat) {
  if (!e || (n_cat > 0 && !cat_embs)) { set_error("rvb_finalize: null argument"); return E_ARG; }
  return finalize_impl(e, cat_embs, n_cat);
}

int64_t rvb_num_frames(int64_t n) { return n < 400 ? 0 : 1 + (n - 400) / 160; }

int rvb_upload_pcm(rvb_engine* e, const int16_t* pcm, int64_t n) {
  if (!e || (!pcm && n > 0) || n < 0) { set_error("rvb_upload_pcm: bad argument"); return E_ARG; }
  RVB_HIP_CHECK(hipSetDevice(e->device));
  RVB_TRY(drop_pending_upload(e));
  e->packed = false;
  RVB_TRY(e->pcm.ensure((size_t)n * 2 + 16));
  if (n) RVB_HIP_CHECK(hipMemcpyAsync(e->pcm.p, pcm, (size_t)n * 2, hipMemcpyHostToDevice, e->stream));
  RVB_HIP_CHECK(hipStreamSynchronize(e->stream));
  e->n_samples = n;
  e->pcm_is_float = false;
  e->batch = false;
  return OK;
}

// ... 486 lines not shown
```

reverb_amd/csrc/engine_encode.hip:

```cpp
#include "engine_impl.h"

#include <algorithm>
#include <cmath>
#include <cstdlib>
#include <cstring>

namespace rvb {

static constexpr int GLU_FUSE_DEFAULT = 1;

static int encoder_layer(rvb_engine* e, EncLayer& L, int lidx, int M, int B, int T, const LNorm& next, void* next_out,
                         float next8 = 0.f, int li = -1) {
  const int d = e->cfg.d_model, ff = e->cfg.ffn_dim, heads = e->cfg.heads, dk = d / heads;
  float* x = e->x.as<float>();
  const bool f8 = e->fp8 && e->f8_state == 2 && li < 0;
  const bool cal = e->fp8 && e->f8_state == 1 && li < 0;
  struct TapLive { rvb_engine* e; ~TapLive() { e->tap_live = false; } } tap_guard{e};
  e->tap_live = e->tap_block == lidx && li < 0;
  const bool t16 = e->dtype == DT_BF16;
  const size_t Md = (size_t)M * d;
  RVB_TRY(tap_keep(e, "x_in", x, Md, false));
  RVB_TRY(tap_keep(e, "xn_ffm", e->xn.p, Md, t16));
  const unsigned grp = f8 ? e->f8_groups[lidx] : 0u;
  const bool f8_ffm = grp & 1u, f8_qkv = grp & 2u, f8_pw1 = grp & 4u, f8_pw2 = grp & 8u, f8_ff = (grp & 16u) && !L.is_lsl;
  const F8Scales sc8 = f8 ? e->f8[lidx] : F8Scales();
  const char* prefold_env = lab_env("RVB_ATTN_PREFOLD");
  const int prefold_on = prefold_env ? atoi(prefold_env) : 1;
  const bool prefold = prefold_on && e->dtype == DT_BF16 && li < 0 && !f8_qkv && L.pos_bias.p != nullptr && dk > 32 && dk <= 64 &&
                       T <= e->pe_rows && T <= 16384 && (d % 8) == 0;
  if (e->tap_live) {
    e->tap_forms.assign(2, 0.f);
    e->tap_forms[0] = prefold ? 1.f : 0.f;
    RVB_TRY(tap_keep(e, "pos_keys", L.pos_keys.p, (size_t)T * d, t16));
    if (L.pos_bias.p) {
      auto& t = e->taps["pos_bias"];
      RVB_TRY(t.buf.ensure((size_t)heads * T * 4));
      t.elems = (size_t)heads * T; t.bf16 = false;
      RVB_HIP_CHECK(hipMemcpy2DAsync(t.buf.p, (size_t)T * 4, L.pos_bias.p, (size_t)e->pe_rows * 4, (size_t)T * 4, heads, hipMemcpyDeviceToDevice, e->stream));
    }
  }
  auto note = [&](int slot, const void* t, size_t n) -> int {
    return cal ? amax_abs(e->stream, e->dtype, t, n, e->d_amax.as<float>() + (size_t)lidx * 8 + slot) : OK;
  };
  auto satp = [&](int slot) -> unsigned* { return e->d_f8sat.p ? e->d_f8sat.as<unsigned>() + (size_t)lidx * 8 + slot : nullptr; };
  if (f8_ffm) {
    RVB_TRY(run_gemm8(e, e->xn.p, d, L.ffm1, e->h.p, ff, M, sc8.in_ffm1, 2, sc8.h_ffm, 1.f, ACT_SILU, nullptr, 0, satp(1)));
    RVB_TRY(run_gemm8(e, e->h.p, ff, L.ffm2, x, d, M, sc8.h_ffm, 1, 1.f, 0.5f, ACT_NONE, x, d));
  } else {
    RVB_TRY(note(0, e->xn.p, (size_t)M * d));
    RVB_TRY(run_gemm(e, e->xn.p, d, L.ffm1, e->h.p, ff, M, false, 1.f, ACT_SILU));
    RVB_TRY(note(1, e->h.p, (size_t)M * ff));
    RVB_TRY(tap_keep(e, "h_ffm", e->h.p, (size_t)M * ff, t16));
    RVB_TRY(run_gemm(e, e->h.p, ff, L.ffm2, x, d, M, true, 0.5f, ACT_NONE, x, d));
  }
  RVB_TRY(tap_keep(e, "x_ffm", x, Md, false));
  if (f8_qkv) {
    RVB_TRY(run_norm(e, x, L.n_mha, e->xn.p, false, M, d, NORM_LN, 0, nullptr, nullptr, nullptr, sc8.in_qkv, 0.f, false, satp(2)));
    RVB_TRY(run_gemm8(e, e->xn.p, d, L.qkv, e->h.p, 3 * d, M, sc8.in_qkv, 0));
  } else {
    RVB_TRY(run_norm(e, x, L.n_mha, e->xn.p, false, M, d));
    RVB_TRY(note(2, e->xn.p, (size_t)M * d));
    if (prefold) {
      GemmArgs g;
      memset(&g, 0, sizeof(g));
      g.A = e->xn.p; g.W = L.qkv.w.p; g.bias = L.qkv.b.as<float>(); g.C = e->h.p;
      g.M = M; g.N = 3 * d; g.K = d; g.lda = d; g.ldw = d; g.ldc = 3 * d; g.alpha = 1.f; g.act = ACT_NONE;
      g.rowadd = L.pos_keys.p; g.rowadd_rows = T; g.rowadd_ld = d; g.rowadd_col0 = d; g.rowadd_cols = d;
      Scope sc(e, "gemm", 2.0 * M * (double)g.N * g.K, gemm_alg_bytes(e, g));
      RVB_TRY(gemm(e->stream, e->dtype, g));
      tap_note_gemm(e);
    } else {
      RVB_TRY(run_gemm(e, e->xn.p, d, L.qkv, e->h.p, 3 * d, M, false));
    }
  }
  RVB_TRY(tap_keep(e, "xn_mha", e->xn.p, Md, t16));
  RVB_TRY(tap_keep(e, "qkv", e->h.p, 3 * Md, t16));
  {
    AttnArgs a;
    memset(&a, 0, sizeof(a));
    const size_t es = dt_size(e->dtype);
    a.q = e->h.p; a.k = (const char*)e->h.p + (size_t)d * es; a.v = (const char*)e->h.p + (size_t)2 * d * es;
    a.p = L.pos_keys.p;
    {
      static const int fold = lab_env("RVB_ATTN_FOLD") ? atoi(lab_env("RVB_ATTN_FOLD")) : 0;
      const int cap = (T + 63) / 64 * 64;
      if (fold && li < 0 && L.pos_bias.p && cap <= 16384) { a.pos_bias = L.pos_bias.as<float>(); a.pos_bias_stride = e->pe_rows; a.fold_kv_cap = cap; }
      if (prefold && cap <= 16384) { a.pos_bias = L.pos_bias.as<float>(); a.pos_bias_stride = e->pe_rows; a.k_prefolded = 1; a.fold_kv_cap = cap; }
    }
    a.q_stride = a.k_stride = a.v_stride = 3 * d; a.p_stride = d; a.o_stride = d;
    a.bias_u = L.bias_u.as<float>(); a.bias_v = L.bias_v.as<float>();
    a.out = e->ao.p;
    a.q_start = e->d_seq_start.as<int>(); a.q_len = e->d_seq_len.as<int>();
    a.kv_start = e->d_seq_start.as<int>(); a.kv_len = e->cur_lens;
    a.nseq = B; a.heads = heads; a.dk = dk; a.max_q = T; a.causal = 0; a.sqrt_dk = std::sqrt((float)dk);
    a.chunk = e->dec_chunk; a.left = e->dec_left;
    { static const int qb = lab_env("RVB_ATTN_QBLOCK") ? atoi(lab_env("RVB_ATTN_QBLOCK")) : 0; a.q_block = qb; }
    double keys = T;
    if (li >= 0) {
      auto& st = e->stream_st;
      char* kvb = (char*)st.kv[li].p;
      RVB_HIP_CHECK(hipMemcpy2DAsync(kvb + (size_t)st.cache_len * 2 * d * es, (size_t)2 * d * es, (const char*)e->h.p + (size_t)d * es,
                                     (size_t)3 * d * es, (size_t)2 * d * es, M, hipMemcpyDeviceToDevice, e->stream));
      a.k = kvb; a.v = kvb + (size_t)d * es; a.k_stride = a.v_stride = 2 * d;
      a.p = (const char*)L.pos_keys.p + (size_t)(st.offset - st.cache_len) * d * es;
      if (a.pos_bias) a.pos_bias += (st.offset - st.cache_len);
      a.kv_start = e->d_stream_i32.as<int>(); a.kv_len = e->d_stream_i32.as<int>() + 1;
      a.chunk = 0; a.left = -1;
      keys = st.cache_len + M;
    }
    Scope sc(e, "attention", 6.0 * B * (double)T * keys * d);
    RVB_TRY(attention(e->stream, e->dtype, with_lab(a)));
  }
  RVB_TRY(tap_keep(e, "ao", e->ao.p, Md, t16));
  RVB_TRY(run_gemm(e, e->ao.p, d, L.att_out, x, d, M, true, 1.f, ACT_NONE, x, d));
  RVB_TRY(tap_keep(e, "x_att", x, Md, false));
  bool glu_fused = false;
  if (f8_pw1) {
    RVB_TRY(run_norm(e, x, L.n_conv, e->xn.p, false, M, d, NORM_LN, 0, nullptr, nullptr, nullptr, sc8.in_pw1, 0.f, false, satp(3)));
    RVB_TRY(run_gemm8(e, e->xn.p, d, L.pw1, e->h.p, 2 * d, M, sc8.in_pw1, 0));
  } else {
    RVB_TRY(run_norm(e, x, L.n_conv, e->xn.p, false, M, d));
    RVB_TRY(note(3, e->xn.p, (size_t)M * d));
    {
      const char* ge = lab_env("RVB_GLU_FUSE");
      const int glu_on = ge ? atoi(ge) : GLU_FUSE_DEFAULT;
      GemmArgs t;
      memset(&t, 0, sizeof(t));
      t.A = e->xn.p; t.W = L.pw1_glu.w.p; t.bias = L.pw1_glu.b.as<float>(); t.C = e->h.p; t.M = M; t.N = 2 * d; t.K = d; t.lda = d; t.ldw = d;
      t.ldc = d; t.alpha = 1.f; t.act = ACT_GLU;
      glu_fused = glu_on && li < 0 && L.pw1_glu.w.p != nullptr && !cal && gemm_glu_supported(e->dtype, t);
      if (glu_fused) {
        Scope sc(e, "gemm", 2.0 * M * (double)t.N * t.K, gemm_alg_bytes(e, t));
        RVB_TRY(gemm(e->stream, e->dtype, t));
        tap_note_gemm(e);
      } else {
        RVB_TRY(run_gemm(e, e->xn.p, d, L.pw1, e->h.p, 2 * d, M, false));
      }
    }
  }
  if (e->tap_live) e->tap_forms[1] = glu_fused ? 1.f : 0.f;
  RVB_TRY(tap_keep(e, "xn_conv", e->xn.p, Md, t16));
  RVB_TRY(tap_keep(e, "glu", e->h.p, glu_fused ? Md : 2 * Md, t16));
  {
    GluDwArgs g;
    g.gated = glu_fused ? 1 : 0;
    g.G = e->h.p; g.pw1_bias = L.pw1.b.as<float>(); g.dw_w = L.dw_w.as<float>(); g.dw_b = L.dw_b.as<float>();
    g.lens = e->cur_lens; g.out = e->dconv.as<float>(); g.B = B; g.T = T; g.d = d; g.K = e->cfg.cnn_kernel;
    g.causal = e->cfg.cnn_causal ? 1 : 0;
    g.out_bf16 = e->dtype == DT_BF16 ? 1 : 0;
    const int lorder = g.K - 1;
    const bool cached = li >= 0 && g.causal && lorder > 0;
    if (cached) { g.hist = e->stream_st.cnn[li].p; g.hist_rows = e->stream_st.cnn_rows; }
    {
      Scope sc(e, "glu_dwconv");
      RVB_TRY(glu_dwconv(e->stream, e->dtype, g));
    }
    if (cached) {
      auto& st = e->stream_st;
      const size_t es = dt_size(e->dtype), rb = (size_t)2 * d * es;
      if (M >= lorder) {
        RVB_HIP_CHECK(hipMemcpyAsync(st.cnn[li].p, (const char*)e->h.p + (size_t)(M - lorder) * rb, (size_t)lorder * rb,
                                     hipMemcpyDeviceToDevice, e->stream));
      } else {
        RVB_HIP_CHECK(hipMemcpyAsync(st.cnn2[li].p, (const char*)st.cnn[li].p + (size_t)M * rb, (size_t)(lorder - M) * rb,
                                     hipMemcpyDeviceToDevice, e->stream));
        RVB_HIP_CHECK(hipMemcpyAsync((char*)st.cnn2[li].p + (size_t)(lorder - M) * rb, e->h.p, (size_t)M * rb,
                                     hipMemcpyDeviceToDevice, e->stream));
        std::swap(st.cnn[li], st.cnn2[li]);
      }
    }
  }
  const int cmode = e->cfg.cnn_norm == 0 ? NORM_LN : NORM_AFFINE;
  const bool dw16 = e->dtype == DT_BF16;
  RVB_TRY(tap_keep(e, "dconv", e->dconv.p, Md, dw16));
  if (f8_pw2) {
    RVB_TRY(run_norm(e, e->dconv.as<float>(), L.n_cnn, e->xn.p, false, M, d, cmode, 1, nullptr, nullptr, nullptr, sc8.in_pw2, 0.f, dw16, satp(4)));
    RVB_TRY(run_gemm8(e, e->xn.p, d, L.pw2, x, d, M, sc8.in_pw2, 1, 1.f, 1.f, ACT_NONE, x, d));
  } else {
    RVB_TRY(run_norm(e, e->dconv.as<float>(), L.n_cnn, e->xn.p, false, M, d, cmode, 1, nullptr, nullptr, nullptr, 0.f, 0.f, dw16));
    RVB_TRY(note(4, e->xn.p, (size_t)M * d));
    RVB_TRY(tap_keep(e, "xn_cnn", e->xn.p, Md, t16));
    RVB_TRY(run_gemm(e, e->xn.p, d, L.pw2, x, d, M, true, 1.f, ACT_NONE, x, d));
  }
  RVB_TRY(tap_keep(e, "x_conv", x, Md, false));
  if (f8_ff) {
    RVB_TRY(run_norm(e, x, L.n_ff, e->xn.p, false, M, d, NORM_LN, 0, nullptr, nullptr, nullptr, sc8.in_ff1, 0.f, false, satp(5)));
    RVB_TRY(run_gemm8(e, e->xn.p, d, L.ff1, e->h.p, ff, M, sc8.in_ff1, 2, sc8.h_ff, 1.f, ACT_SILU, nullptr, 0, satp(6)));
    RVB_TRY(run_gemm8(e, e->h.p, ff, L.ff2, x, d, M, sc8.h_ff, 1, 1.f, 0.5f, ACT_NONE, x, d));
  } else {
    RVB_TRY(run_norm(e, x, L.n_ff, e->xn.p, false, M, d));
    RVB_TRY(tap_keep(e, "xn_ff", e->xn.p, Md, t16));
    const void* ffin = e->xn.p;
    if (L.is_lsl) {
      RVB_TRY(run_gemm(e, e->xn.p, d, L.lsl, e->y.p, d, M, false));
      RVB_TRY(tap_keep(e, "y", e->y.p, Md, t16));
      ffin = e->y.p;
    } else {
      RVB_TRY(note(5, e->xn.p, (size_t)M * d));
    }
    RVB_TRY(run_gemm(e, ffin, d, L.ff1, e->h.p, ff, M, false, 1.f, ACT_SILU));
    if (!L.is_lsl) RVB_TRY(note(6, e->h.p, (size_t)M * ff));
    RVB_TRY(tap_keep(e, "h_ff", e->h.p, (size_t)M * ff, t16));
    RVB_TRY(run_gemm(e, e->h.p, ff, L.ff2, x, d, M, true, 0.5f, ACT_NONE, x, d));
  }
  RVB_TRY(tap_keep(e, "x_ff", x, Md, false));
  RVB_TRY(run_norm(e, x, L.n_final, x, true, M, d, NORM_LN, 0, L.is_lsl ? e->y.p : nullptr, &next, next_out, 0.f, f8 ? next8 : 0.f, false,
                   nullptr, (f8 && next8 > 0.f && e->d_f8sat.p) ? e->d_f8sat.as<unsigned>() + (size_t)(lidx + 1) * 8 : nullptr));
  RVB_TRY(tap_keep(e, "x_out", x, Md, false));
  RVB_TRY(tap_keep(e, "next", next_out, Md, t16));
  return OK;
}

int encode_impl(rvb_engine* e, const float* feats, int64_t first_chunk, const int32_t* lens, int B, int T0,
                       int beam, float blank_penalty) {
  const rvb_model_cfg& c = e->cfg;
  if (!e->finalized) { set_error("rvb_encode before rvb_finalize"); return E_STATE; }
  if (B <= 0 || B > c.max_chunks || T0 < 7 || T0 > c.chunk_frames) {
    set_error("rvb_encode: need 1 <= B <= max_chunks and 7 <= T0 <= chunk_frames"); return E_ARG;
  }
  if (beam < 1 || beam > 64 || beam > c.vocab) { set_error("rvb_encode: beam must be in [1,64]"); return E_ARG; }
  int SB = B >= 16 ? (B * 7 + 9) / 10 : B;
  if (B >= 64) SB = B - 32;
  if (const char* ov = lab_env("RVB_SLICE0")) { const int v = atoi(ov); if (v > 0 && v <= B) SB = v; }
  if (e->tap_block >= 0 && (SB < B || e->fp8)) {
    set_error(SB < B ? "rvb_encode: rvb_set_encoder_tap is on, and this batch is encoded in two slices (B >= 16): tap a smaller batch"
                     : "rvb_encode: rvb_set_encoder_tap is on, and the engine runs its fp8 calibration / fp8 pass");
    return E_UNSUPPORTED;
  }
  RVB_HIP_CHECK(hipSetDevice(e->device));
  RVB_TRY(wait_slices(e, -1));
  e->stream_st.active = false;
  const int d = c.d_model, F0 = c.input_dim, V = c.vocab;
  const int T1 = (T0 - 3) / 2 + 1, F1 = (F0 - 3) / 2 + 1, T2 = (T1 - 3) / 2 + 1, F2 = (F1 - 3) / 2 + 1;
  const int M = B * T2;
  const size_t es = dt_size(e->dtype);
  e->B = B; e->T0 = T0; e->T1 = T1; e->F1 = F1; e->T2 = T2; e->F2 = F2; e->beam = beam;
  e->dec_l.kv_ready = e->dec_r.kv_ready = false;
  e->last_blank_penalty = blank_penalty;
  e->in_lens.assign(lens, lens + B);
  e->enc_lens.resize(B);
  std::vector<int32_t> starts(B), qlens(B, T2);
  for (int b = 0; b < B; ++b) {
    if (lens[b] < 0 || lens[b] > T0) { set_error("rvb_encode: lens out of range"); return E_ARG; }
    e->enc_lens[b] = lens[b] > 6 ? (lens[b] - 7) / 4 + 1 : 0;
    starts[b] = b * T2;
  }
  e->nbest.clear(); e->trie_l.clear(); e->rescored.clear();
  RVB_TRY(upload_i32(e, e->d_enc_lens, e->enc_lens.data(), B));
  RVB_TRY(upload_i32(e, e->d_seq_start, starts.data(), B));
  RVB_TRY(upload_i32(e, e->d_seq_len, qlens.data(), B));

  const float* d_feats;
  if (feats) {
    RVB_TRY(upload_f32(e, e->d_feats_in, feats, (size_t)B * T0 * F0));
    d_feats = e->d_feats_in.as<float>();
  } else {
    const DevBuf& fb = e->packed ? e->feats_packed : e->feats;
    if (!fb.p || first_chunk < 0 || (first_chunk + B) * (int64_t)T0 > (e->packed ? e->packed_rows : e->feat_rows)) {
      set_error("rvb_encode: device features missing or too short (call rvb_fbank first)"); return E_STATE;
    }
    d_feats = fb.as<float>() + (size_t)first_chunk * T0 * F0;
  }
  const int Ms = SB * T2;
  RVB_TRY(e->X1.ensure((size_t)SB * T1 * F1 * d * es));
  RVB_TRY(e->X2.ensure((size_t)SB * T2 * F2 * d * es));
  RVB_TRY(e->x.ensure((size_t)Ms * d * 4));
  RVB_TRY(e->xn.ensure((size_t)Ms * d * es));
  RVB_TRY(e->y.ensure((size_t)Ms * d * es));
  RVB_TRY(e->ao.ensure((size_t)Ms * d * es));
  RVB_TRY(e->dconv.ensure((size_t)Ms * d * 4));
  RVB_TRY(e->enc_out.ensure((size_t)M * d * es));
  RVB_TRY(e->h.ensure((size_t)Ms * std::max(c.ffn_dim, 3 * d) * es));
  const int Vld = (V + 3) & ~3;
  RVB_TRY(e->logits.ensure((size_t)LOGIT_SLAB * Vld * 4));
  RVB_TRY(e->topv.ensure((size_t)M * beam * 4));
  RVB_TRY(e->topi.ensure((size_t)M * beam * 4));
  if (e->h_top_cap < (size_t)M * beam) {
    if (e->h_topv) (void)hipHostFree(e->h_topv);
    if (e->h_topi) (void)hipHostFree(e->h_topi);
    e->h_topv = nullptr; e->h_topi = nullptr; e->h_top_cap = 0;
    RVB_HIP_CHECK(hipHostMalloc((void**)&e->h_topv, (size_t)M * beam * 4, hipHostMallocDefault));
    RVB_HIP_CHECK(hipHostMalloc((void**)&e->h_topi, (size_t)M * beam * 4, hipHostMallocDefault));
    e->h_top_cap = (size_t)M * beam;
  }
  e->slices.clear();
  if (e->fp8 && e->f8_state == 0) {
    RVB_TRY(e->d_amax.ensure((e->enc.size() + 1) * 8 * 4));
    RVB_HIP_CHECK(hipMemsetAsync(e->d_amax.p, 0, (e->enc.size() + 1) * 8 * 4, e->stream));
    RVB_TRY(reset_f8sat(e));
    e->f8_state = 1;
  }
  for (int c0 = 0; c0 < B; c0 += SB) {
    const int nb = std::min(SB, B - c0);
    const int m = nb * T2;
    const int row0 = c0 * T2;
    e->cur_lens = e->d_enc_lens.as<int>() + c0;
    const bool f8c2 = e->fp8 && e->f8_state == 2 && e->f8_conv2 && e->f8_x1 > 0.f && e->conv2.w8.p && d % 128 == 0;
    const bool calx = e->fp8 && e->f8_state == 1;
    struct TapLive { rvb_engine* e; ~TapLive() { e->tap_live = false; } } tap_guard{e};
    e->tap_live = e->tap_block == (int)e->enc.size();
    if (e->tap_live) e->tap_forms.clear();
    const bool t16 = e->dtype == DT_BF16;
    {
      Scope sc(e, "subsample");
      RVB_TRY(subsample_conv1(e->stream, e->dtype, d_feats + (size_t)c0 * T0 * F0, e->cmvn_mean.as<float>(),
                              e->cmvn_istd.as<float>(), e->conv1_w.as<float>(), e->conv1_b.as<float>(), e->X1.p, nb, T0, F0, d,
                              f8c2 ? e->f8_x1 : 0.f, calx ? e->d_amax.as<unsigned>() + e->enc.size() * 8 : nullptr,
                              (f8c2 && e->d_f8sat.p) ? e->d_f8sat.as<unsigned>() + e->enc.size() * 8 + 1 : nullptr));
    }
    {
      GemmArgs g;
      memset(&g, 0, sizeof(g));
      g.A = e->X1.p; g.W = e->conv2.w.p; g.bias = e->conv2.b.as<float>(); g.C = e->X2.p;
      g.M = nb * T2 * F2; g.N = d; g.K = 9 * d; g.lda = d; g.ldw = 9 * d; g.ldc = d;
      g.alpha = 1.f; g.act = ACT_RELU; g.conv = 1; g.cT1 = T1; g.cF1 = F1; g.cT2 = T2; g.cF2 = F2; g.cC = d;
      if (f8c2) { g.W = e->conv2.w8.p; g.in_fp8 = 1; g.a_scale = e->f8_x1; g.w_scale = e->conv2.wscale.as<float>(); }
      Scope sc(e, f8c2 ? "gemm_fp8" : "gemm", 2.0 * g.M * (double)g.N * g.K, gemm_alg_bytes(e, g));
      RVB_TRY(gemm(e->stream, e->dtype, g));
      tap_note_gemm(e);
    }
    RVB_TRY(tap_keep(e, "X1", e->X1.p, (size_t)nb * T1 * F1 * d, t16));
    RVB_TRY(tap_keep(e, "X2", e->X2.p, (size_t)m * F2 * d, t16));
    RVB_TRY(run_gemm(e, e->X2.p, F2 * d, e->embed_out, e->x.p, d, m, true, std::sqrt((float)d)));
    RVB_TRY(tap_keep(e, "x0", e->x.p, (size_t)m * d, false));
    void* eo = (char*)e->enc_out.p + (size_t)row0 * d * es;
    const bool f8 = e->fp8 && e->f8_state == 2;
    RVB_TRY(run_norm(e, e->x.as<float>(), e->enc[0].n_ffm, e->xn.p, false, m, d, NORM_LN, 0, nullptr, nullptr, nullptr,
                     (f8 && (e->f8_groups[0] & 1u)) ? e->f8[0].in_ffm1 : 0.f, 0.f, false, e->d_f8sat.as<unsigned>()));
    RVB_TRY(tap_keep(e, "xn0", e->xn.p, (size_t)m * d, t16));
    e->tap_live = false;
    for (size_t li = 0; li < e->enc.size(); ++li) {
      const bool last = li + 1 == e->enc.size();
      RVB_TRY(encoder_layer(e, e->enc[li], (int)li, m, nb, T2, last ? e->enc_after : e->enc[li + 1].n_ffm, last ? eo : e->xn.p,
                            (f8 && !last && (e->f8_groups[li + 1] & 1u)) ? e->f8[li + 1].in_ffm1 : 0.f));
    }
    for (int r0 = 0; r0 < m; r0 += LOGIT_SLAB) {
      const int rows = std::min(LOGIT_SLAB, m - r0);
      RVB_TRY(run_gemm(e, (const char*)eo + (size_t)r0 * d * es, d, e->ctc, e->logits.p, Vld, rows, true));
      Scope sc(e, "ctc_topk");
      RVB_TRY(logsoftmax_topk(e->stream, e->logits.as<float>(), rows, V, Vld, beam, blank_penalty, c.blank_id,
                              e->topv.as<float>() + (size_t)(row0 + r0) * beam, e->topi.as<int>() + (size_t)(row0 + r0) * beam, nullptr));
    }
    RVB_HIP_CHECK(hipMemcpyAsync(e->h_topv + (size_t)row0 * beam, e->topv.as<float>() + (size_t)row0 * beam, (size_t)m * beam * 4, hipMemcpyDeviceToHost, e->stream));
    RVB_HIP_CHECK(hipMemcpyAsync(e->h_topi + (size_t)row0 * beam, e->topi.as<int>() + (size_t)row0 * beam, (size_t)m * beam * 4, hipMemcpyDeviceToHost, e->stream));
    hipEvent_t ev;
    if (!e->slice_event_pool.empty()) { ev = e->slice_event_pool.back(); e->slice_event_pool.pop_back(); }
    else RVB_HIP_CHECK(hipEventCreateWithFlags(&ev, hipEventDisableTiming));
    RVB_HIP_CHECK(hipEventRecord(ev, e->stream));
    e->slices.push_back({c0, nb, ev, false});
  }
  if (e->f8_state == 1) {
    std::vector<float> am((e->enc.size() + 1) * 8);
    RVB_HIP_CHECK(hipMemcpyAsync(am.data(), e->d_amax.p, am.size() * 4, hipMemcpyDeviceToHost, e->stream));
    RVB_HIP_CHECK(hipStreamSynchronize(e->stream));
    e->f8.resize(e->enc.size());
    auto sc = [](float a) { return a > 0.f ? std::exp2(std::ceil(std::log2(2.f * a / 448.f))) : 1.f; };
    for (size_t l = 0; l < e->enc.size(); ++l) {
      const float* a = am.data() + l * 8;
      e->f8[l] = {sc(a[0]), sc(a[1]), sc(a[2]), sc(a[3]), sc(a[4]), sc(a[5]), sc(a[6])};
    }
    e->f8_x1 = am[e->enc.size() * 8] > 0.f ? sc(am[e->enc.size() * 8]) : 0.f;
    if (e->f8_groups.size() != e->enc.size()) RVB_TRY(set_fp8_policy_impl(e, -1, 0, -1));
    e->f8_state = 2;
  }
  return OK;
}

int wait_slices(rvb_engine* e, int i) {
  for (size_t k = 0; k < e->slices.size(); ++k) {
    if (i >= 0 && (int)k != i) continue;
    auto& sl = e->slices[k];
    if (sl.done) continue;
    RVB_HIP_CHECK(hipEventSynchronize(sl.ev));
    e->slice_event_pool.push_back(sl.ev);
    sl.done = true;
  }
  return OK;
}

int stream_begin_impl(rvb_engine* e) {
  if (!e->finalized) { set_error("rvb_stream_begin before rvb_finalize"); return E_STATE; }
  RVB_HIP_CHECK(hipSetDevice(e->device));
  RVB_TRY(wait_slices(e, -1));
  const int d = e->cfg.d_model;
  const size_t es = dt_size(e->dtype);
  auto& st = e->stream_st;
  st.kv.resize(e->enc.size()); st.kv2.resize(e->enc.size());
  for (size_t l = 0; l < e->enc.size(); ++l) {
    RVB_TRY(st.kv[l].ensure((size_t)e->pe_rows * 2 * d * es));
    RVB_TRY(st.kv2[l].ensure((size_t)e->pe_rows * 2 * d * es));
  }
  RVB_TRY(e->enc_out.ensure((size_t)e->pe_rows * d * es));
  if (e->cfg.cnn_causal && e->cfg.cnn_kernel > 1) {
    st.cnn.resize(e->enc.size()); st.cnn2.resize(e->enc.size());
    for (size_t l = 0; l < e->enc.size(); ++l) {
      RVB_TRY(st.cnn[l].ensure((size_t)(e->cfg.cnn_kernel - 1) * 2 * d * es));
      RVB_TRY(st.cnn2[l].ensure((size_t)(e->cfg.cnn_kernel - 1) * 2 * d * es));
    }
  }
  st.active = true; st.offset = 0; st.cache_len = 0; st.cnn_rows = 0;
  e->B = 0; e->nbest.clear(); e->trie_l.clear(); e->rescored.clear(); e->slices.clear();
  e->dec_l.kv_ready = e->dec_r.kv_ready = false;
  return OK;
}

int stream_chunk_impl(rvb_engine* e, const float* feats, int T0, int required_cache_size, float* out, int32_t* n_out) {
  const rvb_model_cfg& c = e->cfg;
  auto& st = e->stream_st;
  if (!st.active) { set_error("rvb_stream_chunk before rvb_stream_begin"); return E_STATE; }
  if (T0 < 7) { set_error("rvb_stream_chunk: a chunk needs at least 7 input frames (Conv2dSubsampling4)"); return E_ARG; }
  if (e->tap_block >= 0) { set_error("rvb_stream_chunk: rvb_set_encoder_tap is on (the taps are the offline encoder's)"); return E_UNSUPPORTED; }
  RVB_HIP_CHECK(hipSetDevice(e->device));
  const int d = c.d_model, F0 = c.input_dim;
  const int T1 = (T0 - 3) / 2 + 1, F1 = (F0 - 3) / 2 + 1, T2 = (T1 - 3) / 2 + 1, F2 = (F1 - 3) / 2 + 1;
  const int M = T2;
  const size_t es = dt_size(e->dtype);
  if (st.offset + M > e->pe_rows) {
    set_error("rvb_stream_chunk: more than " + std::to_string(e->pe_rows) + " encoder frames in one stream (the reference's positional "
              "table has max_len 5000 rows, embedding.py:33)");
    return E_UNSUPPORTED;
  }
  RVB_TRY(e->X1.ensure((size_t)T1 * F1 * d * es));
  RVB_TRY(e->X2.ensure((size_t)T2 * F2 * d * es));
  RVB_TRY(e->x.ensure((size_t)M * d * 4));
  RVB_TRY(e->xn.ensure((size_t)M * d * es));
  RVB_TRY(e->y.ensure((size_t)M * d * es));
  RVB_TRY(e->ao.ensure((size_t)M * d * es));
  RVB_TRY(e->dconv.ensure((size_t)M * d * 4));
  RVB_TRY(e->h.ensure((size_t)M * std::max(c.ffn_dim, 3 * d) * es));
  RVB_TRY(upload_f32(e, e->d_feats_in, feats, (size_t)T0 * F0));
  const int32_t zero = 0, mm = M, kv[2] = {0, st.cache_len + M};
  RVB_TRY(upload_i32(e, e->d_seq_start, &zero, 1));
  RVB_TRY(upload_i32(e, e->d_seq_len, &mm, 1));
  RVB_TRY(upload_i32(e, e->d_enc_lens, &mm, 1));
  RVB_TRY(upload_i32(e, e->d_stream_i32, kv, 2));
  e->cur_lens = e->d_enc_lens.as<int>();
  {
    Scope sc(e, "subsample");
    RVB_TRY(subsample_conv1(e->stream, e->dtype, e->d_feats_in.as<float>(), e->cmvn_mean.as<float>(), e->cmvn_istd.as<float>(),
                            e->conv1_w.as<float>(), e->conv1_b.as<float>(), e->X1.p, 1, T0, F0, d));
  }
  {
    GemmArgs g;
    memset(&g, 0, sizeof(g));
    g.A = e->X1.p; g.W = e->conv2.w.p; g.bias = e->conv2.b.as<float>(); g.C = e->X2.p;
    g.M = T2 * F2; g.N = d; g.K = 9 * d; g.lda = d; g.ldw = 9 * d; g.ldc = d;
    g.alpha = 1.f; g.act = ACT_RELU; g.conv = 1; g.cT1 = T1; g.cF1 = F1; g.cT2 = T2; g.cF2 = F2; g.cC = d;
    Scope sc(e, "gemm", 2.0 * g.M * (double)g.N * g.K, gemm_alg_bytes(e, g));
    RVB_TRY(gemm(e->stream, e->dtype, g));
  }
  RVB_TRY(run_gemm(e, e->X2.p, F2 * d, e->embed_out, e->x.p, d, M, true, std::sqrt((float)d)));
  void* eo = (char*)e->enc_out.p + (size_t)st.offset * d * es;
  RVB_TRY(run_norm(e, e->x.as<float>(), e->enc[0].n_ffm, e->xn.p, false, M, d));
  for (size_t li = 0; li < e->enc.size(); ++li) {
    const bool last = li + 1 == e->enc.size();
    RVB_TRY(encoder_layer(e, e->enc[li], (int)li, M, 1, M, last ? e->enc_after : e->enc[li + 1].n_ffm, last ? eo : e->xn.p, 0.f, (int)li));
  }
  if (out) {
    if (e->dtype == DT_F32) {
      RVB_HIP_CHECK(hipMemcpyAsync(out, eo, (size_t)M * d * 4, hipMemcpyDeviceToHost, e->stream));
      RVB_HIP_CHECK(hipStreamSynchronize(e->stream));
    } else {
      std::vector<bf16_t> tmp((size_t)M * d);
      RVB_HIP_CHECK(hipMemcpyAsync(tmp.data(), eo, tmp.size() * 2, hipMemcpyDeviceToHost, e->stream));
      RVB_HIP_CHECK(hipStreamSynchronize(e->stream));
      for (size_t i = 0; i < tmp.size(); ++i) out[i] = bf16_to_f32(tmp[i]);
    }
  }
  const int key_size = st.cache_len + M;
  int start = 0;
  if (required_cache_size == 0) start = key_size;
  else if (required_cache_size > 0) start = std::max(key_size - required_cache_size, 0);
  const int keep = key_size - start;
  if (start > 0 && keep > 0) {
    for (size_t l = 0; l < e->enc.size(); ++l) {
      RVB_HIP_CHECK(hipMemcpyAsync(st.kv2[l].p, (const char*)st.kv[l].p + (size_t)start * 2 * d * es, (size_t)keep * 2 * d * es,
                                   hipMemcpyDeviceToDevice, e->stream));
      std::swap(st.kv[l], st.kv2[l]);
    }
  }
  st.cache_len = keep;
  st.cnn_rows = std::min(st.cnn_rows + M, std::max(c.cnn_kernel - 1, 0));
  st.offset += M;
  if (n_out) *n_out = M;
  return OK;
}

int stream_finish_impl(rvb_engine* e, int beam, float blank_penalty) {
  const rvb_model_cfg& c = e->cfg;
  auto& st = e->stream_st;
  if (!st.active) { set_error("rvb_stream_finish before rvb_stream_begin"); return E_STATE; }
  if (beam < 1 || beam > 64 || beam > c.vocab) { set_error("rvb_stream_finish: beam must be in [1,64]"); return E_ARG; }
  RVB_HIP_CHECK(hipSetDevice(e->device));
  const int d = c.d_model, V = c.vocab, M = st.offset;
  const size_t es = dt_size(e->dtype);
  if (M <= 0) { set_error("rvb_stream_finish: the stream produced no encoder frame"); return E_STATE; }
  e->B = 1; e->T2 = M; e->beam = beam; e->T0 = 0;
  e->dec_l.kv_ready = e->dec_r.kv_ready = false;
  e->last_blank_penalty = blank_penalty;
  e->in_lens.assign(1, 0); e->enc_lens.assign(1, M);
  e->nbest.clear(); e->trie_l.clear(); e->rescored.clear();
  const int Vld = (V + 3) & ~3;
  RVB_TRY(e->logits.ensure((size_t)LOGIT_SLAB * Vld * 4));
  RVB_TRY(e->topv.ensure((size_t)M * beam * 4));
  RVB_TRY(e->topi.ensure((size_t)M * beam * 4));
  if (e->h_top_cap < (size_t)M * beam) {
    if (e->h_topv) (void)hipHostFree(e->h_topv);
    if (e->h_topi) (void)hipHostFree(e->h_topi);
    e->h_topv = nullptr; e->h_topi = nullptr; e->h_top_cap = 0;
    RVB_HIP_CHECK(hipHostMalloc((void**)&e->h_topv, (size_t)M * beam * 4, hipHostMallocDefault));
    RVB_HIP_CHECK(hipHostMalloc((void**)&e->h_topi, (size_t)M * beam * 4, hipHostMallocDefault));
    e->h_top_cap = (size_t)M * beam;
  }
  for (int r0 = 0; r0 < M; r0 += LOGIT_SLAB) {
    const int rows = std::min(LOGIT_SLAB, M - r0);
    RVB_TRY(run_gemm(e, (const char*)e->enc_out.p + (size_t)r0 * d * es, d, e->ctc, e->logits.p, Vld, rows, true));
    Scope sc(e, "ctc_topk");
    RVB_TRY(logsoftmax_topk(e->stream, e->logits.as<float>(), rows, V, Vld, beam, blank_penalty, c.blank_id,
                            e->topv.as<float>() + (size_t)r0 * beam, e->topi.as<int>() + (size_t)r0 * beam, nullptr));
  }
  RVB_HIP_CHECK(hipMemcpyAsync(e->h_topv, e->topv.p, (size_t)M * beam * 4, hipMemcpyDeviceToHost, e->stream));
  RVB_HIP_CHECK(hipMemcpyAsync(e->h_topi, e->topi.p, (size_t)M * beam * 4, hipMemcpyDeviceToHost, e->stream));
  RVB_HIP_CHECK(hipStreamSynchronize(e->stream));
  e->slices.clear();
  e->slices.push_back({0, 1, nullptr, true});
  st.active = false;
  return OK;
}

}
```

reverb_amd/csrc/engine_impl.h:

```cpp
#pragma once
#include "engine.h"

namespace rvb {

struct Scope {
  rvb_engine* e; hipEvent_t a = nullptr, b = nullptr; std::string name;
  Scope(rvb_engine* e_, const char* n, double flops = 0.0, double bytes = 0.0) : e(e_), name(n) {
    auto& pe = e->prof[name];
    pe.launches += 1; pe.flops += flops; pe.bytes += bytes;
    if (e->profiling == 0 || (e->profiling == 2 && name != "gemm" && name != "gemm_fp8")) return;
    auto get = [&]() { hipEvent_t ev; if (!e->event_pool.empty()) { ev = e->event_pool.back(); e->event_pool.pop_back(); } else (void)hipEventCreate(&ev); return ev; };
    a = get(); b = get();
    (void)hipEventRecord(a, e->stream);
  }
  ~Scope() {
    if (!a) return;
    (void)hipEventRecord(b, e->stream);
    e->pending.push_back({a, b, name});
  }
};
int upload_f32(rvb_engine* e, DevBuf& dst, const float* src, size_t n);
int upload_i32(rvb_engine* e, DevBuf& dst, const int32_t* src, size_t n);
const AttnArgs& with_lab(AttnArgs& a);
int reset_f8sat(rvb_engine* e);
double gemm_alg_bytes(const rvb_engine* e, const GemmArgs& g);
int run_gemm(rvb_engine* e, const void* A, int lda, const Linear& L, void* C, int ldc, int M, bool out_f32,
             float alpha = 1.f, int act = ACT_NONE, const float* res = nullptr, int ldres = 0);
int run_norm(rvb_engine* e, const float* x, const LNorm& n, void* out, bool out_f32, int M, int d,
             int mode = NORM_LN, int silu = 0, const void* add = nullptr, const LNorm* second = nullptr,
             void* out2 = nullptr, float out8 = 0.f, float out2_8 = 0.f, bool x_bf16 = false, unsigned* sat = nullptr,
             unsigned* sat2 = nullptr);
int run_gemm8(rvb_engine* e, const void* A8, int lda, const Linear& L, void* C, int ldc, int M, float a_scale, int out_kind,
              float out_scale = 1.f, float alpha = 1.f, int act = ACT_NONE, const float* res = nullptr, int ldres = 0,
              unsigned* sat = nullptr);

int tap_keep(rvb_engine* e, const char* name, const void* src, size_t elems, bool is_bf16);
void tap_note_gemm(rvb_engine* e);
int gemm_last_path();

int make_fbank_tables(rvb_engine* e);
int finalize_impl(rvb_engine* e, const float* cat, int ncat);
int set_fp8_policy_impl(rvb_engine* e, int groups, int first_block, int last_block);

constexpr int LOGIT_SLAB = 8192;
int wait_slices(rvb_engine* e, int i);
int encode_impl(rvb_engine* e, const float* feats, int64_t first_chunk, const int32_t* lens, int B, int T0, int beam, float blank_penalty);
int stream_begin_impl(rvb_engine* e);
int stream_chunk_impl(rvb_engine* e, const float* feats, int T0, int required_cache_size, float* out, int32_t* n_out);
int stream_finish_impl(rvb_engine* e, int beam, float blank_penalty);

int prefix_beam_impl(rvb_engine* e, int beam);
int decoder_memory_kv(rvb_engine* e, Decoder& D, int M);
int rescore_impl(rvb_engine* e, double ctc_weight, double reverse_weight);
int attention_decode_impl(rvb_engine* e, int N, float length_penalty);
int joint_decode_impl(rvb_engine* e, int beam, double ctc_weight, double pre_beam_ratio, double length_bonus);

}
```

reverb_amd/csrc/gemm.hip:

```cpp
#include "common.h"
#include "kernels.h"

namespace rvb {

static constexpr int BM = 128, BN = 128;
static constexpr int ROWB = 128;
static constexpr int LDSB = 144;
static constexpr int GEMM_LDS = 2 * (BM + BN) * LDSB;

__device__ inline float act_apply(float v, int act) {
  if (act == ACT_SILU) return v / (1.0f + expf(-v));
  if (act == ACT_RELU) return fmaxf(v, 0.0f);
  if (act == ACT_LRELU) return v > 0.0f ? v : 0.01f * v;
  return v;
}

template <typename T, typename OutT, bool CONV>
__global__ __launch_bounds__(256) void gemm_kernel(GemmArgs p) {
  extern __shared__ __attribute__((aligned(16))) char smem[];
  constexpr int VE = Mma16<T>::VE;
  constexpr int BKE = ROWB / sizeof(T);
  const int tid = threadIdx.x;
  const int lane = tid & 63;
  const int wave = tid >> 6;
// ... 75 lines not shown
  __syncthreads();

  const int frow = lane & 15;
  const int fk = (lane >> 4) * 16;
  for (int kt = 0; kt < nk; ++kt) {
    const int cur = kt & 1;
    if (kt + 1 < nk) load_tile((kt + 1) * BKE);
    const char* sA = smem + cur * (BM + BN) * LDSB + (wr * 64 + frow) * LDSB + fk;
    const char* sB = smem + cur * (BM + BN) * LDSB + BM * LDSB + (wc * 64 + frow) * LDSB + fk;
#pragma unroll
    for (int ch = 0; ch < 2; ++ch) {
      uint4 a[4], b[4];
#pragma unroll
      for (int i = 0; i < 4; ++i) {
        a[i] = *(const uint4*)(sA + i * 16 * LDSB + ch * 64);
        b[i] = *(const uint4*)(sB + i * 16 * LDSB + ch * 64);
      }
#pragma unroll
      for (int i = 0; i < 4; ++i)
#pragma unroll
        for (int j = 0; j < 4; ++j) Mma16<T>::run(a[i], b[j], acc[i][j]);
    }
    if (kt + 1 < nk) store_tile(cur ^ 1);
    __syncthreads();
  }

  OutT* __restrict__ C = (OutT*)p.C;
  const int crow = (lane >> 4) * 4;
  const int ccol = lane & 15;
#pragma unroll
  for (int j = 0; j < 4; ++j) {
    const int col = n0 + wc * 64 + j * 16 + ccol;
    if (col >= p.N) continue;
    const float bv = p.bias ? p.bias[col] : 0.0f;
#pragma unroll
    for (int i = 0; i < 4; ++i) {
#pragma unroll
      for (int r = 0; r < 4; ++r) {
        const int row = m0 + wr * 64 + i * 16 + crow + r;
        if (row >= p.M) continue;
        float v = acc[i][j][r] + bv;
        v = act_apply(v, p.act) * p.alpha;
        if (p.res) v += p.res[(size_t)row * p.ldres + col];
        if (p.rowadd && col >= p.rowadd_col0 && col < p.rowadd_col0 + p.rowadd_cols)
          v += bf16_to_f32(((const bf16_t*)p.rowadd)[(size_t)(row % p.rowadd_rows) * p.rowadd_ld + (col - p.rowadd_col0)]);
        C[(size_t)row * p.ldc + col] = Cvt<OutT>::from_f32(v);
      }
    }
  }
}

template <typename T, typename OutT, bool CONV>
static int launch(hipStream_t s, const GemmArgs& p) {
  static bool attr_set = false;
  auto kern = gemm_kernel<T, OutT, CONV>;
  if (!attr_set) {
    RVB_HIP_CHECK(hipFuncSetAttribute((const void*)kern, hipFuncAttributeMaxDynamicSharedMemorySize, GEMM_LDS));
    attr_set = true;
  }
  const int tiles = cdiv(p.M, BM) * cdiv(p.N, BN);
  if (tiles <= 0) return OK;
  hipLaunchKernelGGL(kern, dim3(tiles), dim3(256), GEMM_LDS, s, p);
  RVB_HIP_CHECK(hipGetLastError());
  return OK;
}

int g_gemm_variant = 0;

static thread_local int t_last_path = 0;
int gemm_last_path() { return t_last_path; }

int gemm(hipStream_t s, int dtype, const GemmArgs& p) {
  const int ve = dtype == DT_BF16 ? 8 : 4;
  if (p.M < 0 || p.N <= 0 || p.K <= 0 || (p.K % ve) || (p.lda % ve) || (p.ldw % ve) ||
      (p.conv && (p.cC % ve))) {
    set_error("gemm: K, lda, ldw (and conv channels) must be multiples of the 16-byte vector width");
    return E_ARG;
  }
  if (p.M == 0) return OK;
  if (p.rowadd && (dtype != DT_BF16 || p.out_f32 || p.in_fp8 || p.out_fp8 || p.rowadd_rows <= 0)) {
    set_error("gemm: the row-periodic addend exists for bf16 operands and bf16 output only");
    return E_UNSUPPORTED;
  }
  if (p.act == ACT_GLU) {
    if (g_gemm_variant == 1 || !gemm_glu_supported(dtype, p)) { set_error("gemm: ACT_GLU needs the bf16 LDS-DMA kernel (see gemm_glu_supported)"); return E_UNSUPPORTED; }
    t_last_path = 2;
    return gemm2(s, dtype, p);
  }
  if (p.in_fp8) {
    if (!gemm2_applicable(dtype, p)) { set_error("gemm: fp8 operands need the bf16 engine, K % 128 == 0 and per-channel weight scales"); return E_ARG; }
    t_last_path = 2;
    return gemm2(s, dtype, p);
  }
  if (g_gemm_variant != 1 && (dtype == DT_BF16 || g_gemm_variant == 2) && gemm2_applicable(dtype, p)) {
    t_last_path = 2;
    return gemm2(s, dtype, p);
  }
  t_last_path = 1;
  if (dtype == DT_BF16) {
    if (p.out_f32) return p.conv ? launch<bf16_t, float, true>(s, p) : launch<bf16_t, float, false>(s, p);
    return p.conv ? launch<bf16_t, bf16_t, true>(s, p) : launch<bf16_t, bf16_t, false>(s, p);
  }
  return p.conv ? launch<float, float, true>(s, p) : launch<float, float, false>(s, p);
}

}
```

reverb_amd/csrc/gemm2.hip:

```cpp
#include "kernels.h"
#include "wave_asm.h"

#include <cstdlib>
#include <type_traits>

namespace rvb {

static constexpr int B2M = 256, B2N = 256;
static constexpr int ROW2 = 128;
static constexpr int STAGE2 = (B2M + B2N) * ROW2;
static constexpr int GEMM2_LDS = 2 * STAGE2;
static constexpr int GEMM2_DEFAULT_FLAGS = 0;
static constexpr int GROUP_M_AUTO = -2, GEMM2_DEFAULT_GROUP_M = GROUP_M_AUTO;

__device__ inline float act_apply2(float v, int act) {
  if (act == ACT_SILU) return v / (1.0f + expf(-v));
  if (act == ACT_RELU) return fmaxf(v, 0.0f);
  return v;
}

__device__ inline void glds16(const void* g, char* lds_wave_base) {
  __builtin_amdgcn_global_load_lds((const __attribute__((address_space(1))) void*)g,
                                   (__attribute__((address_space(3))) void*)lds_wave_base, 16, 0, 0);
}
// ... 544 lines not shown
      } else {
        finish_v(actf);
      }
    };
    if (p.act == ACT_SILU) {
      if constexpr (sizeof(T) <= 2) run([](float x) { return x * __builtin_amdgcn_rcpf(1.0f + __builtin_amdgcn_exp2f(-1.44269504f * x)); });
      else run([](float x) { return x / (1.0f + expf(-x)); });
    } else if (p.act == ACT_RELU) {
      run([](float x) { return fmaxf(x, 0.0f); });
    } else {
      run([](float x) { return x; });
    }
    if (p.dbg && tid == 0) { wait_vm<0>(); p.dbg[blockIdx.x * 6 + 3] = wall_clock64(); }
    return;
  }
  if constexpr (M32) {
    auto finish32 = [&](auto actf) {
#pragma unroll
      for (int bi = 0; bi < 4; ++bi)
#pragma unroll
        for (int bj = 0; bj < 2; ++bj) {
          const int col = n0 + wc * 64 + bj * 32 + (lane & 31);
          const float bvv = (p.bias && col < p.N) ? p.bias[col] : 0.0f;
#pragma unroll
          for (int r = 0; r < 16; ++r) {
            const int row = m0 + wr * 128 + bi * 32 + (r & 3) + 8 * (r >> 2) + 4 * (lane >> 5);
            if (row >= p.M || col >= p.N) continue;
            float av = acc32[bi][bj][r];
            if constexpr (F8) av *= (col < p.N ? p.a_scale * p.w_scale[col] : 0.f);
            float v = actf(av + bvv) * p.alpha;
            if (p.res) v += p.res[(size_t)row * p.ldres + col];
            if constexpr (sizeof(OutT) == 1) C[(size_t)row * p.ldc + col] = (OutT)(pack4_fp8(v * p.out_inv_scale, 0.f, 0.f, 0.f) & 0xffu);
            else C[(size_t)row * p.ldc + col] = Cvt<OutT>::from_f32(v);
          }
        }
    };
    if (p.act == ACT_SILU) finish32([](float v) { return v * __builtin_amdgcn_rcpf(1.0f + __builtin_amdgcn_exp2f(-1.44269504f * v)); });
    else if (p.act == ACT_RELU) finish32([](float v) { return fmaxf(v, 0.0f); });
    else finish32([](float v) { return v; });
    return;
  }
  if constexpr (!M32) {
  float bv[4];
#pragma unroll
  for (int j = 0; j < 4; ++j) {
    const int col = n0 + wc * 64 + j * 16 + ccol;
    bv[j] = (p.bias && col < p.N) ? p.bias[col] : 0.0f;
  }
  auto finish = [&](auto actf) {
#pragma unroll
    for (int i = 0; i < 8; ++i) {
#pragma unroll
      for (int r = 0; r < 4; ++r) {
        const int row = m0 + wr * 128 + i * 16 + crow + r;
        if (!full && row >= p.M) continue;
        const float* rrow = (p.res && !res_acc) ? p.res + (size_t)row * p.ldres : nullptr;
        OutT* crow_p = C + (size_t)row * p.ldc;
#pragma unroll
        for (int j = 0; j < 4; ++j) {
          const int col = n0 + wc * 64 + j * 16 + ccol;
          if (!full && col >= p.N) continue;
          float v = actf(acc[i][j][r] + bv[j]) * p.alpha;
          if (rrow) v += rrow[col];
          crow_p[col] = Cvt<OutT>::from_f32(v);
        }
      }
    }
  };
  if (p.act == ACT_SILU) {
    if constexpr (sizeof(T) == 2) finish([](float v) { return v * __builtin_amdgcn_rcpf(1.0f + __builtin_amdgcn_exp2f(-1.44269504f * v)); });
    else finish([](float v) { return v / (1.0f + expf(-v)); });
  } else if (p.act == ACT_RELU) {
    finish([](float v) { return fmaxf(v, 0.0f); });
  } else {
    finish([](float v) { return v; });
  }
  }
}

extern int g_gemm2_flags;
static constexpr int P_NSLOT = 7, P_HT = 128 * ROW2, P_LEAD = P_NSLOT - 2, P_DEPTH = P_LEAD - 2;
static constexpr int P_SROW = 64 * 4 + 16;
static constexpr int GEMM2P_LDS = P_NSLOT * P_HT + 8 * 16 * P_SROW;

template <typename T, typename OutT, bool CONV, int PMODE = 0, bool M32 = false, bool PH2 = false>
__global__ __launch_bounds__(512) void gemm2p_kernel(GemmArgs p) {
  static_assert(!PH2 || (sizeof(T) == 2 && !M32 && PMODE == 0), "PH2: bf16, 16x16x32 fragments, one tile per workgroup");
  static_assert(!M32 || sizeof(T) == 2, "M32 is the bf16 form");
  constexpr bool PERSIST = PMODE != 0;
  constexpr bool XPF = PMODE == 1;
  static_assert(!(PERSIST && CONV), "the persistent form reuses the per-lane DMA offsets from tile to tile");
  extern __shared__ __attribute__((aligned(16))) char smem[];
  constexpr bool F8 = std::is_same<T, fp8_t>::value;
  constexpr bool B32 = F8 || M32;
  constexpr int BKE = ROW2 / (int)sizeof(T);
  const int tid = threadIdx.x;
  const int lane = tid & 63;
  const int wave = __builtin_amdgcn_readfirstlane(tid >> 6);
  const int wr = wave >> 2, wc = wave & 3;
  const int tiles_n = (p.N + B2N - 1) / B2N, tiles_m = (p.M + B2M - 1) / B2M;
  int lin, lin_end, lin_step;
  {
    const int ntile = PERSIST ? tiles_m * tiles_n : (int)gridDim.x;
    const int q = ntile >> 3, r = ntile & 7;
    const int xcd = blockIdx.x & 7, idx = blockIdx.x >> 3;
    const int start = xcd < r ? xcd * (q + 1) : r * (q + 1) + (xcd - r) * q;
    lin = start + idx;
    lin_end = PERSIST ? start + q + (xcd < r ? 1 : 0) : lin + 1;
    lin_step = PERSIST ? (int)(gridDim.x >> 3) : 1;
  }
  auto tile_of = [&](int bid, int& tm, int& tn) __attribute__((always_inline)) {
    if (p.group_m > 1) {
      const int per_group = p.group_m * tiles_n;
      const int g = bid / per_group;
      const int first_m = g * p.group_m;
      const int gsz = min(tiles_m - first_m, p.group_m);
      const int in_g = bid - g * per_group;
      tm = first_m + in_g % gsz;
      tn = in_g / gsz;
    } else {
      tm = bid / tiles_n; tn = bid - tm * tiles_n;
    }
  };
  const unsigned lds_base = (unsigned)(size_t)(__attribute__((address_space(3))) char*)smem;
  int s_cur = 0;
  int s_rd = 1;
  int s_st = P_LEAD;
  bool first_tile = true;
  if constexpr (!XPF) {
    if (p.stagger_ticks > 0 && blockIdx.x < (unsigned)p.stagger_first && ((blockIdx.x >> 5) & 1)) {
      const long long t0 = wall_clock64();
      while (wall_clock64() - t0 < p.stagger_ticks) __builtin_amdgcn_s_sleep(32);
    }
  }
  for (;;) {
  const int dbg_i = PERSIST ? lin : (int)blockIdx.x;
  if (p.dbg && tid == 0) {
    p.dbg[dbg_i * 6 + 0] = wall_clock64();
    p.dbg[dbg_i * 6 + 4] = __builtin_amdgcn_s_getreg(63492);
    p.dbg[dbg_i * 6 + 5] = __builtin_amdgcn_s_getreg(63508);
  }
  int tm, tn;
  tile_of(lin, tm, tn);
  const int m0 = tm * B2M, n0 = tn * B2N;
  const bool has_next = PERSIST && lin + lin_step < lin_end;

  auto a_elem = [&](int m) -> size_t {
    if (CONV) {
      const int tf = p.cT2 * p.cF2;
      const int b = m / tf;
      const int rem = m - b * tf;
      const int t2 = rem / p.cF2, f2 = rem - t2 * p.cF2;
      return (((size_t)b * p.cT1 + 2 * t2) * p.cF1 + 2 * f2) * (size_t)p.cC;
    }
    return (size_t)m * p.lda;
  };
  const size_t a_row0 = a_elem(m0);
  const int lr = lane >> 3, lc = lane & 7;
  unsigned offA[2][2], offW[2][2];
#pragma unroll
  for (int i = 0; i < 2; ++i) {
    const int r = 16 * wave + 8 * i + lr;
    const unsigned col = (unsigned)((lc ^ ((r >> 1) & 7)) * 16);
#pragma unroll
    for (int hlf = 0; hlf < 2; ++hlf) {
      const int m = min(m0 + (r >> 6) * 128 + hlf * 64 + (r & 63), p.M - 1);
      const int n = min(n0 + (r >> 5) * 64 + hlf * 32 + (r & 31), p.N - 1);
      offA[hlf][i] = (unsigned)((a_elem(m) - a_row0) * sizeof(T)) + col;
      offW[hlf][i] = (unsigned)((size_t)(n - n0) * p.ldw * sizeof(T)) + col;
    }
  }
  const char* a_base = uniform_ptr((const char*)((const T*)p.A + a_row0));
  const char* w_base = uniform_ptr((const char*)((const T*)p.W + (size_t)n0 * p.ldw));
  const char* a_next = a_base;
  const char* w_next = w_base;
  if (XPF && has_next) {
    int tm2, tn2;
    tile_of(lin + lin_step, tm2, tn2);
    a_next = uniform_ptr((const char*)((const T*)p.A + (size_t)tm2 * B2M * p.lda));
    w_next = uniform_ptr((const char*)((const T*)p.W + (size_t)tn2 * B2N * p.ldw));
  }
  const int nk = p.K / BKE, nh = 4 * nk;
  const bool k_rev = !CONV && !PERSIST && p.k_serp && ((blockIdx.x >> 8) & 1);
  const unsigned lds_wave = lds_base + wave * 2048;
  const int row_steps = CONV ? 3 * p.cC / BKE : 0x7fffffff;
  const size_t row_jump = CONV ? (size_t)(p.cF1 - 3) * p.cC * sizeof(T) : 0;
  auto advance = [&](size_t& off, int& cnt) __attribute__((always_inline)) {
    off += ROW2;
    if (++cnt == row_steps) { cnt = 0; off += row_jump; }
  };
  size_t ak1 = 0, ak2 = 0;
  int ac1 = 0, ac2 = 0;
  advance(ak1, ac1);
  ak2 = ak1; ac2 = ac1;
  advance(ak2, ac2);
  auto stage_ty = [&](auto tyc, int t, size_t ak, int slot) __attribute__((always_inline)) {
    constexpr int ty = decltype(tyc)::value;
    if constexpr (!CONV && !PERSIST) {
      if (k_rev) { t = nk - 1 - t; ak = (size_t)t * ROW2; }
    }
    const unsigned dst = __builtin_amdgcn_readfirstlane(lds_wave + slot * P_HT);
    if constexpr (ty == 0) lds_dma2(offA[0][0], offA[0][1], uniform_ptr(a_base + ak), dst);
    else if constexpr (ty == 1) lds_dma2(offW[0][0], offW[0][1], uniform_ptr(w_base + (size_t)t * ROW2), dst);
    else if constexpr (ty == 2) lds_dma2(offW[1][0], offW[1][1], uniform_ptr(w_base + (size_t)t * ROW2), dst);
    else lds_dma2(offA[1][0], offA[1][1], uniform_ptr(a_base + ak), dst);
  };
  auto stage_next = [&](auto tyc, int t2, int slot) __attribute__((always_inline)) {
    constexpr int ty = decltype(tyc)::value;
    const unsigned dst = __builtin_amdgcn_readfirstlane(lds_wave + slot * P_HT);
    if constexpr (ty == 0) lds_dma2(offA[0][0], offA[0][1], uniform_ptr(a_next + (size_t)t2 * ROW2), dst);
    else if constexpr (ty == 1) lds_dma2(offW[0][0], offW[0][1], uniform_ptr(w_next + (size_t)t2 * ROW2), dst);
    else if constexpr (ty == 2) lds_dma2(offW[1][0], offW[1][1], uniform_ptr(w_next + (size_t)t2 * ROW2), dst);
    else lds_dma2(offA[1][0], offA[1][1], uniform_ptr(a_next + (size_t)t2 * ROW2), dst);
  };
  auto stage = [&](int h, int slot) __attribute__((always_inline)) {
    const int t = h >> 2, ty = h & 3;
    const size_t ak = t == 0 ? 0 : ak1;
    if (ty == 0) stage_ty(std::integral_constant<int, 0>(), t, ak, slot);
    else if (ty == 1) stage_ty(std::integral_constant<int, 1>(), t, ak, slot);
    else if (ty == 2) stage_ty(std::integral_constant<int, 2>(), t, ak, slot);
    else stage_ty(std::integral_constant<int, 3>(), t, ak, slot);
  };
  static_assert(P_LEAD - 1 < 8, "the prologue requests half-tiles of K steps 0 and 1 only");
  static_assert(P_DEPTH == 3, "the tail's counted waits enumerate the counts below P_DEPTH");

  f32x4_t acc[B32 ? 1 : 8][B32 ? 1 : 4];
  f32x16_t acc32[B32 ? 4 : 1][B32 ? 2 : 1];
  const bool res_acc = !PH2 && !p.res_epilogue && p.res != nullptr && p.act == ACT_NONE && p.alpha != 0.f && (p.N & 3) == 0 && (p.ldres & 3) == 0 &&
                       ((size_t)p.res & 15) == 0;
  if constexpr (PMODE == 2) { s_cur = 0; s_rd = 1; s_st = P_LEAD; }
  if constexpr (PH2) {
    for (int h = 0; h < 4; ++h) stage(h, h);
  } else if (first_tile || !XPF) {
    for (int h = 0; h < P_LEAD && h < nh; ++h) stage(h, h);
  }
  if (res_acc) {
    const float inv_alpha = 1.0f / p.alpha;
    const int lr4 = lane >> 4, lc4 = (lane & 15) * 4;
    const int colr = min(n0 + wc * 64 + lc4, p.N - 4);
    char* tb = smem + P_NSLOT * P_HT + wave * (16 * P_SROW);
    float csc[2] = {inv_alpha, inv_alpha};
    if constexpr (F8) {
#pragma unroll
      for (int bj = 0; bj < 2; ++bj) {
        const int col = n0 + wc * 64 + bj * 32 + (lane & 31);
        const float sc = col < p.N ? p.a_scale * p.w_scale[col] : 1.0f;
        csc[bj] = sc != 0.f ? inv_alpha / sc : 0.f;
      }
    }
    constexpr int NPART = B32 ? 2 : 1, QP = 32 / NPART;
#pragma unroll
    for (int part = 0; part < NPART; ++part) {
      f32x4_t rv[QP];
#pragma unroll
      for (int q = 0; q < QP; ++q) {
        const int qq = part * QP + q;
        const int row = min(m0 + wr * 128 + (qq >> 2) * 16 + (qq & 3) * 4 + lr4, p.M - 1);
        rv[q] = *(const f32x4_t*)(p.res + (size_t)row * p.ldres + colr);
      }
#pragma unroll
      for (int ii = 0; ii < 8 / NPART; ++ii) {
        const int i = part * (8 / NPART) + ii;
#pragma unroll
        for (int q = 0; q < 4; ++q) *(f32x4_t*)(tb + (q * 4 + lr4) * P_SROW + lc4 * 4) = rv[ii * 4 + q];
        __builtin_amdgcn_wave_barrier();
        if constexpr (B32) {
          const int bi = i >> 1, hh = i & 1;
          const int r32 = 4 * (lane >> 5), c32 = lane & 31;
#pragma unroll
          for (int bj = 0; bj < 2; ++bj)
#pragma unroll
            for (int qq = 0; qq < 2; ++qq)
#pragma unroll
              for (int r = 0; r < 4; ++r)
                acc32[bi][bj][8 * hh + 4 * qq + r] = *(const float*)(tb + (8 * qq + r32 + r) * P_SROW + (bj * 32 + c32) * 4) * csc[bj];
        } else {
#pragma unroll
          for (int j = 0; j < 4; ++j)
#pragma unroll
            for (int r = 0; r < 4; ++r) acc[i][j][r] = *(const float*)(tb + (lr4 * 4 + r) * P_SROW + (j * 16 + (lane & 15)) * 4) * inv_alpha;
        }
        __builtin_amdgcn_wave_barrier();
      }
    }
  } else {
    if constexpr (B32) {
#pragma unroll
      for (int i = 0; i < 4; ++i)
#pragma unroll
        for (int j = 0; j < 2; ++j)
#pragma unroll
          for (int r = 0; r < 16; ++r) acc32[i][j][r] = 0.f;
    } else {
#pragma unroll
      for (int i = 0; i < 8; ++i)
#pragma unroll
        for (int j = 0; j < 4; ++j) acc[i][j] = (f32x4_t){0.f, 0.f, 0.f, 0.f};
    }
  }
  if constexpr (PH2) {
    wait_vm<2>();
  } else if (first_tile || !XPF) {
    const int infl = (nh < P_LEAD ? nh : P_LEAD) - 2;
    if (infl >= P_DEPTH) wait_vm<2 * P_DEPTH>(); else wait_vm<0>();
  }
  __builtin_amdgcn_s_barrier();
  if (p.dbg && tid == 0) p.dbg[dbg_i * 6 + 1] = wall_clock64();

  const int frow = B32 ? (lane & 31) : (lane & 15), lgrp = B32 ? (lane >> 5) : (lane >> 4);
  const int swz = (frow >> 1) & 7;
  const int ro0 = F8 ? ((0 * 4 + 2 * lgrp) ^ swz) << 4 : ((0 * 4 + lgrp) ^ swz) << 4;
// ... 135 lines not shown
    auto ph_wait = [&](auto jc) __attribute__((always_inline)) {
      constexpr int j = decltype(jc)::value;
      if constexpr (TAIL) {
        constexpr int infl = 4 * R - 3 - j;
        if constexpr (infl >= P_DEPTH) wait_vm<2 * P_DEPTH>();
        else if constexpr (infl >= 0) wait_vm<2 * (infl < 0 ? 0 : infl)>();
      } else if constexpr (MODE == 4 && j < 3) {
        wait_vm<2 * P_DEPTH + NST>();
      } else {
        wait_vm<2 * P_DEPTH>();
      }
    };
    ph_head(std::integral_constant<int, 0>());
    if constexpr (F8) {
      read_a_half(h1, fa_hi, s_cur); read_b(fb0, s_rd);
    } else {
      read_b_khalf(h0, fb0, s_rd); read_a_half(h1, fa_hi, s_cur); read_b_khalf(h1, fb0, s_rd);
    }
    ph_wait(std::integral_constant<int, 0>());
    mid(); mma_q(c0, c0, fh, fa_hi, fb0); end(); adv();
    ph_head(std::integral_constant<int, 1>()); read_b(fb1, s_rd); ph_wait(std::integral_constant<int, 1>());
    mid(); mma_q(c0, c1, fh, fa_hi, fb1); end(); adv();
    ph_head(std::integral_constant<int, 2>()); read_a_half(h0, fa_lo, s_rd); read_a_half(h1, fa_hi, s_rd); ph_wait(std::integral_constant<int, 2>());
    mid(); mma_q(c1, c1, fa_lo, fa_hi, fb1); end(); adv();
    ph_head(std::integral_constant<int, 3>()); if constexpr (MODE == 0 || MODE == 2 || MODE == 4 || (MODE == 1 && R > 1)) read_a_half(h0, fh, s_rd); ph_wait(std::integral_constant<int, 3>());
    mid(); mma_q(c1, c0, fa_lo, fa_hi, fb0); end(); adv();
    ak1 = ak2; ac1 = ac2;
    advance(ak2, ac2);
  };
  constexpr int NTAIL = (P_LEAD + 3) / 4 + 1;
  int t = 0;
  if constexpr (XPF) {
    if (!first_tile) { kstep(std::integral_constant<int, 4>(), c0, 0); t = 1; }
    for (; t < nk - 2; ++t) kstep(std::integral_constant<int, 0>(), c0, t);
    kstep(std::integral_constant<int, 2>(), c0, nk - 2);
    kstep(std::integral_constant<int, 3>(), c0, nk - 1);
  } else {
    static_assert(NTAIL == 3, "the tail is unrolled by hand: K steps with 3, 2 and 1 steps left");
    for (; t < nk - NTAIL; ++t) kstep(std::integral_constant<int, 0>(), c0, t);
    if (nk >= 3) kstep(c1, std::integral_constant<int, 3>(), nk - 3);
    if (nk >= 2) kstep(c1, std::integral_constant<int, 2>(), nk - 2);
    kstep(c1, c1, nk - 1);
  }
  }
  if (wr == 0) __builtin_amdgcn_s_barrier();
  if (p.dbg && tid == 0) p.dbg[dbg_i * 6 + 2] = wall_clock64();
  auto epilogue = [&]() __attribute__((always_inline)) {

  OutT* __restrict__ C = (OutT*)p.C;
  const int crow = (lane >> 4) * 4;
  const int ccol = lane & 15;
  const bool full = (m0 + B2M <= p.M) && (n0 + B2N <= p.N);
  const bool vec_ok = ((p.ldc * (int)sizeof(OutT)) % 16 == 0) && (((size_t)p.C & 15) == 0) &&
                      (p.res == nullptr || ((p.ldres % 4) == 0 && ((size_t)p.res & 15) == 0));
  if (vec_ok) {
    char* slab = smem + (PH2 ? 0 : P_NSLOT * P_HT) + wave * (16 * P_SROW);
    constexpr int CPL = sizeof(OutT) == 4 ? 4 : (sizeof(OutT) == 2 ? 8 : 16);
    constexpr int LPR = 64 / CPL;
    constexpr int RPP = 64 / LPR;
    constexpr int NQ = 16 / RPP;
    const int orow = lane / LPR;
    const int ocol = (lane % LPR) * CPL;
    const int col0 = n0 + wc * 64 + ocol;
    float biasv[CPL], scv[F8 ? CPL : 1];
#pragma unroll
    for (int e = 0; e < CPL; ++e) biasv[e] = (p.bias && col0 + e < p.N) ? p.bias[col0 + e] : 0.0f;
    if constexpr (F8) {
#pragma unroll
      for (int e = 0; e < CPL; ++e) scv[e] = col0 + e < p.N ? p.a_scale * p.w_scale[col0 + e] : 0.0f;
    }
    const bool seg_full = col0 + CPL <= p.N;
    constexpr bool RA_OK = sizeof(OutT) == 2 && !F8;
    const bool glu = sizeof(OutT) == 2 && !F8 && p.act == ACT_GLU;
    const bool ra_any = RA_OK && p.rowadd != nullptr && n0 < p.rowadd_col0 + p.rowadd_cols && n0 + B2N > p.rowadd_col0;
    const bool ra_tile = ra_any && n0 >= p.rowadd_col0 && n0 + B2N <= p.rowadd_col0 + p.rowadd_cols && (p.rowadd_ld & 7) == 0 &&
                         ((p.rowadd_col0 - n0) & 7) == 0 && ((size_t)p.rowadd & 15) == 0;
    const int ra_t0 = ra_any ? (m0 + wr * 128) % p.rowadd_rows : 0;
    auto ra_row = [&](int local) __attribute__((always_inline)) -> int {
      int t = ra_t0 + local;
      if (t >= p.rowadd_rows) { t -= p.rowadd_rows; if (t >= p.rowadd_rows) t %= p.rowadd_rows; }
      return t;
    };
    const bf16_t* ra_base = (const bf16_t*)p.rowadd + (col0 - p.rowadd_col0);
    constexpr int RING = sizeof(OutT) == 4 ? 3 : 2, RV = NQ * (CPL / 4);
    float4 rring[RING][RV];
    const bool res_pre = p.res != nullptr && !res_acc && seg_full;
    const int colc = min(col0, p.N - CPL);
    auto res_issue = [&](int i, int slot) __attribute__((always_inline)) {
#pragma unroll
      for (int q = 0; q < NQ; ++q) {
        const int row = min(m0 + wr * 128 + i * 16 + q * RPP + orow, p.M - 1);
        const float4* rp = (const float4*)(p.res + (size_t)row * p.ldres + colc);
#pragma unroll
        for (int c4 = 0; c4 < CPL / 4; ++c4) rring[slot][q * (CPL / 4) + c4] = rp[c4];
      }
    };
    auto finish_v = [&](auto actf) {
      if (res_pre) {
#pragma unroll
        for (int i = 0; i < RING; ++i) res_issue(i, i);
      }
#pragma unroll
      for (int i = 0; i < 8; ++i) {
        __builtin_amdgcn_wave_barrier();
        if constexpr (B32) {
          const int bi = i >> 1, hh = i & 1;
          const int r32 = 4 * (lane >> 5), c32 = lane & 31;
#pragma unroll
          for (int bj = 0; bj < 2; ++bj)
#pragma unroll
            for (int qq = 0; qq < 2; ++qq)
#pragma unroll
              for (int r = 0; r < 4; ++r)
                *(float*)(slab + (8 * qq + r32 + r) * P_SROW + (bj * 32 + c32) * 4) = acc32[bi][bj][8 * hh + 4 * qq + r];
        } else {
#pragma unroll
          for (int j = 0; j < 4; ++j)
#pragma unroll
            for (int r = 0; r < 4; ++r)
              *(float*)(slab + (crow + r) * P_SROW + (j * 16 + ccol) * 4) = acc[i][j][r];
        }
        __builtin_amdgcn_wave_barrier();
#pragma unroll
        for (int q = 0; q < NQ; ++q) {
          const int srow = q * RPP + orow;
          float v[CPL];
#pragma unroll
          for (int c4 = 0; c4 < CPL / 4; ++c4) {
            const float4 tt = *(const float4*)(slab + srow * P_SROW + (ocol + c4 * 4) * 4);
            v[c4 * 4 + 0] = tt.x; v[c4 * 4 + 1] = tt.y; v[c4 * 4 + 2] = tt.z; v[c4 * 4 + 3] = tt.w;
          }
          const int row = m0 + wr * 128 + i * 16 + srow;
          if (row >= p.M || col0 >= p.N) continue;
          if constexpr (F8) {
#pragma unroll
            for (int e = 0; e < CPL; ++e) v[e] *= scv[e];
          }
#pragma unroll
          for (int e = 0; e < CPL; ++e) v[e] = actf(v[e] + biasv[e]) * p.alpha;
          OutT* cp = C + (size_t)row * p.ldc + col0;
          if (seg_full) {
            if (res_pre) {
#pragma unroll
              for (int c4 = 0; c4 < CPL / 4; ++c4) {
                const float4 tt = rring[i % RING][q * (CPL / 4) + c4];
                v[c4 * 4 + 0] += tt.x; v[c4 * 4 + 1] += tt.y; v[c4 * 4 + 2] += tt.z; v[c4 * 4 + 3] += tt.w;
              }
            }
            if constexpr (RA_OK) {
              if (ra_any) {
                const bf16_t* ar = ra_base + (size_t)ra_row(i * 16 + srow) * p.rowadd_ld;
#pragma unroll
                for (int e = 0; e < CPL; ++e)
                  if (col0 + e >= p.rowadd_col0 && col0 + e < p.rowadd_col0 + p.rowadd_cols) v[e] += bf16_to_f32(ar[e]);
              }
            }
            if constexpr (sizeof(OutT) == 1) {
              const float qs = p.out_inv_scale;
              if (p.sat) {
                float mx = fmaxf(fabsf(v[0]), fabsf(v[1]));
#pragma unroll
                for (int e2 = 2; e2 < 16; ++e2) mx = fmaxf(mx, fabsf(v[e2]));
                if (mx * qs > 448.f) {
                  const unsigned ns = fp8_clipped(v[0] * qs, v[1] * qs, v[2] * qs, v[3] * qs) + fp8_clipped(v[4] * qs, v[5] * qs, v[6] * qs, v[7] * qs) +
                                      fp8_clipped(v[8] * qs, v[9] * qs, v[10] * qs, v[11] * qs) + fp8_clipped(v[12] * qs, v[13] * qs, v[14] * qs, v[15] * qs);
                  atomicAdd(p.sat, ns);
                }
              }
              *(uint4*)cp = make_uint4(pack4_fp8(v[0] * qs, v[1] * qs, v[2] * qs, v[3] * qs), pack4_fp8(v[4] * qs, v[5] * qs, v[6] * qs, v[7] * qs),
                                       pack4_fp8(v[8] * qs, v[9] * qs, v[10] * qs, v[11] * qs), pack4_fp8(v[12] * qs, v[13] * qs, v[14] * qs, v[15] * qs));
            } else if constexpr (sizeof(OutT) == 2) {
              if (glu) {
                uint2 o0;
                o0.x = pack2_bf16(glu_gate(v[0], v[1]), glu_gate(v[2], v[3]));
                o0.y = pack2_bf16(glu_gate(v[4], v[5]), glu_gate(v[6], v[7]));
                *(uint2*)(C + (size_t)row * p.ldc + (col0 >> 1)) = o0;
              } else {
                uint4 o0;
                o0.x = pack2_bf16(v[0], v[1]);
                o0.y = pack2_bf16(v[2], v[3]);
                o0.z = pack2_bf16(v[4], v[5]);
                o0.w = pack2_bf16(v[6], v[7]);
                *(uint4*)cp = o0;
              }
            } else {
              *(float4*)cp = make_float4(v[0], v[1], v[2], v[3]);
            }
          } else {
            for (int e = 0; e < CPL && col0 + e < p.N; ++e) {
              float o = v[e];
              if (p.res && !res_acc) o += p.res[(size_t)row * p.ldres + col0 + e];
              if constexpr (RA_OK) {
                if (ra_any && col0 + e >= p.rowadd_col0 && col0 + e < p.rowadd_col0 + p.rowadd_cols)
                  o += bf16_to_f32(ra_base[(size_t)ra_row(i * 16 + srow) * p.rowadd_ld + e]);
              }
              if constexpr (sizeof(OutT) == 1) cp[e] = (OutT)(pack4_fp8(o * p.out_inv_scale, 0.f, 0.f, 0.f) & 0xffu);
              else cp[e] = Cvt<OutT>::from_f32(o);
            }
          }
        }
        if (res_pre && i + RING < 8) res_issue(i + RING, i % RING);
      }
    };
    auto finish_fast = [&](auto actf, auto resc, auto addc) {
      constexpr bool HR = decltype(resc)::value;
      constexpr bool RA = decltype(addc)::value && RA_OK;
      uint4 aring[RA ? RING : 1][RA ? NQ : 1];
      auto add_issue = [&](int i, int slot) __attribute__((always_inline)) {
#pragma unroll
        for (int q = 0; q < NQ; ++q)
          aring[RA ? slot : 0][RA ? q : 0] = *(const uint4*)(ra_base + (size_t)ra_row(i * 16 + q * RPP + orow) * p.rowadd_ld);
      };
      if constexpr (RA) {
#pragma unroll
        for (int i = 0; i < RING; ++i) add_issue(i, i);
      }
      auto res_issue_f = [&](int i, int slot) __attribute__((always_inline)) {
#pragma unroll
        for (int q = 0; q < NQ; ++q) {
          const float4* rp = (const float4*)(p.res + (size_t)(m0 + wr * 128 + i * 16 + q * RPP + orow) * p.ldres + col0);
#pragma unroll
          for (int c4 = 0; c4 < CPL / 4; ++c4) rring[slot][q * (CPL / 4) + c4] = rp[c4];
        }
      };
      if constexpr (HR) {
#pragma unroll
        for (int i = 0; i < RING; ++i) res_issue_f(i, i);
      }
#pragma unroll
      for (int i = 0; i < 8; ++i) {
        __builtin_amdgcn_wave_barrier();
        if constexpr (B32) {
          const int bi = i >> 1, hh = i & 1;
          const int r32 = 4 * (lane >> 5), c32 = lane & 31;
#pragma unroll
          for (int bj = 0; bj < 2; ++bj)
#pragma unroll
            for (int qq = 0; qq < 2; ++qq)
#pragma unroll
              for (int r = 0; r < 4; ++r)
                *(float*)(slab + (8 * qq + r32 + r) * P_SROW + (bj * 32 + c32) * 4) = acc32[bi][bj][8 * hh + 4 * qq + r];
        } else {
#pragma unroll
          for (int j = 0; j < 4; ++j)
#pragma unroll
            for (int r = 0; r < 4; ++r)
              *(float*)(slab + (crow + r) * P_SROW + (j * 16 + ccol) * 4) = acc[i][j][r];
        }
        __builtin_amdgcn_wave_barrier();
#pragma unroll
        for (int q = 0; q < NQ; ++q) {
          const int srow = q * RPP + orow;
          float v[CPL];
#pragma unroll
          for (int c4 = 0; c4 < CPL / 4; ++c4) {
            const float4 tt = *(const float4*)(slab + srow * P_SROW + (ocol + c4 * 4) * 4);
            v[c4 * 4 + 0] = tt.x; v[c4 * 4 + 1] = tt.y; v[c4 * 4 + 2] = tt.z; v[c4 * 4 + 3] = tt.w;
          }
          if constexpr (F8) {
#pragma unroll
            for (int e = 0; e < CPL; ++e) v[e] *= scv[e];
          }
#pragma unroll
          for (int e = 0; e < CPL; ++e) v[e] = actf(v[e] + biasv[e]) * p.alpha;
          if constexpr (HR) {
#pragma unroll
            for (int c4 = 0; c4 < CPL / 4; ++c4) {
              const float4 tt = rring[i % RING][q * (CPL / 4) + c4];
              v[c4 * 4 + 0] += tt.x; v[c4 * 4 + 1] += tt.y; v[c4 * 4 + 2] += tt.z; v[c4 * 4 + 3] += tt.w;
            }
          }
          if constexpr (RA) {
            const uint4 av = aring[i % RING][q];
            v[0] += __uint_as_float(av.x << 16); v[1] += __uint_as_float(av.x & 0xffff0000u);
            v[2] += __uint_as_float(av.y << 16); v[3] += __uint_as_float(av.y & 0xffff0000u);
            v[4] += __uint_as_float(av.z << 16); v[5] += __uint_as_float(av.z & 0xffff0000u);
            v[6] += __uint_as_float(av.w << 16); v[7] += __uint_as_float(av.w & 0xffff0000u);
          }
          OutT* cp = C + (size_t)(m0 + wr * 128 + i * 16 + srow) * p.ldc + col0;
          if constexpr (sizeof(OutT) == 1) {
            const float qs = p.out_inv_scale;
            if (p.sat) {
              float mx = fmaxf(fabsf(v[0]), fabsf(v[1]));
#pragma unroll
              for (int e2 = 2; e2 < 16; ++e2) mx = fmaxf(mx, fabsf(v[e2]));
              if (mx * qs > 448.f) {
                const unsigned ns = fp8_clipped(v[0] * qs, v[1] * qs, v[2] * qs, v[3] * qs) + fp8_clipped(v[4] * qs, v[5] * qs, v[6] * qs, v[7] * qs) +
                                    fp8_clipped(v[8] * qs, v[9] * qs, v[10] * qs, v[11] * qs) + fp8_clipped(v[12] * qs, v[13] * qs, v[14] * qs, v[15] * qs);
                atomicAdd(p.sat, ns);
              }
            }
            store16_hidden(cp, pack4_fp8(v[0] * qs, v[1] * qs, v[2] * qs, v[3] * qs), pack4_fp8(v[4] * qs, v[5] * qs, v[6] * qs, v[7] * qs),
                           pack4_fp8(v[8] * qs, v[9] * qs, v[10] * qs, v[11] * qs), pack4_fp8(v[12] * qs, v[13] * qs, v[14] * qs, v[15] * qs));
          } else if constexpr (sizeof(OutT) == 2) {
            if (glu) store8_hidden(C + (size_t)(m0 + wr * 128 + i * 16 + srow) * p.ldc + (col0 >> 1),
                                   pack2_bf16(glu_gate(v[0], v[1]), glu_gate(v[2], v[3])), pack2_bf16(glu_gate(v[4], v[5]), glu_gate(v[6], v[7])));
            else store16_hidden(cp, pack2_bf16(v[0], v[1]), pack2_bf16(v[2], v[3]), pack2_bf16(v[4], v[5]), pack2_bf16(v[6], v[7]));
          } else {
            store16_hidden(cp, __float_as_uint(v[0]), __float_as_uint(v[1]), __float_as_uint(v[2]), __float_as_uint(v[3]));
          }
        }
        if constexpr (HR) {
          if (i + RING < 8) res_issue_f(i + RING, i % RING);
        }
        if constexpr (RA) {
          if (i + RING < 8) add_issue(i + RING, i % RING);
        }
      }
    };
    const bool hr = p.res != nullptr && !res_acc;
    const bool fast = full && (p.fast_epilogue & (hr ? 2 : 1)) && (!ra_any || (ra_tile && !hr));
    auto run = [&](auto actf) __attribute__((always_inline)) {
      if (fast) {
        if (hr) finish_fast(actf, std::true_type(), std::false_type());
        else if (ra_any) finish_fast(actf, std::false_type(), std::true_type());
        else finish_fast(actf, std::false_type(), std::false_type());
      } else {
        finish_v(actf);
      }
    };
    if (p.act == ACT_SILU) run([](float x) { return x * __builtin_amdgcn_rcpf(1.0f + __builtin_amdgcn_exp2f(-1.44269504f * x)); });
    else if (p.act == ACT_RELU) run([](float x) { return fmaxf(x, 0.0f); });
    else run([](float x) { return x; });
    if (p.dbg && tid == 0) { if (!has_next) wait_vm<0>(); p.dbg[dbg_i * 6 + 3] = wall_clock64(); }
    return;
  }
  if constexpr (B32) {
    auto finish32 = [&](auto actf) {
#pragma unroll
      for (int bi = 0; bi < 4; ++bi)
#pragma unroll
        for (int bj = 0; bj < 2; ++bj) {
          const int col = n0 + wc * 64 + bj * 32 + (lane & 31);
          const float bvv = (p.bias && col < p.N) ? p.bias[col] : 0.0f;
          float sc = 1.f;
          if constexpr (F8) sc = col < p.N ? p.a_scale * p.w_scale[col] : 0.f;
#pragma unroll
          for (int r = 0; r < 16; ++r) {
            const int row = m0 + wr * 128 + bi * 32 + (r & 3) + 8 * (r >> 2) + 4 * (lane >> 5);
            if (row >= p.M || col >= p.N) continue;
            float v = actf(acc32[bi][bj][r] * sc + bvv) * p.alpha;
            if (p.res && !res_acc) v += p.res[(size_t)row * p.ldres + col];
            if constexpr (sizeof(OutT) == 2 && !F8) {
              if (p.rowadd && col >= p.rowadd_col0 && col < p.rowadd_col0 + p.rowadd_cols)
                v += bf16_to_f32(((const bf16_t*)p.rowadd)[(size_t)(row % p.rowadd_rows) * p.rowadd_ld + (col - p.rowadd_col0)]);
            }
            if constexpr (sizeof(OutT) == 1) C[(size_t)row * p.ldc + col] = (OutT)(pack4_fp8(v * p.out_inv_scale, 0.f, 0.f, 0.f) & 0xffu);
            else C[(size_t)row * p.ldc + col] = Cvt<OutT>::from_f32(v);
          }
        }
    };
// ... 13 lines not shown
    for (int i = 0; i < 8; ++i) {
#pragma unroll
      for (int r = 0; r < 4; ++r) {
        const int row = m0 + wr * 128 + i * 16 + crow + r;
        if (!full && row >= p.M) continue;
        const float* rrow = (p.res && !res_acc) ? p.res + (size_t)row * p.ldres : nullptr;
        OutT* crow_p = C + (size_t)row * p.ldc;
#pragma unroll
        for (int j = 0; j < 4; ++j) {
          const int col = n0 + wc * 64 + j * 16 + ccol;
          if (!full && col >= p.N) continue;
          float v = actf(acc[i][j][r] + bv[j]) * p.alpha;
          if (rrow) v += rrow[col];
          if constexpr (sizeof(OutT) == 2) {
            if (p.rowadd && col >= p.rowadd_col0 && col < p.rowadd_col0 + p.rowadd_cols)
              v += bf16_to_f32(((const bf16_t*)p.rowadd)[(size_t)(row % p.rowadd_rows) * p.rowadd_ld + (col - p.rowadd_col0)]);
          }
          crow_p[col] = Cvt<OutT>::from_f32(v);
        }
      }
    }
  };
  if (p.act == ACT_SILU) finish([](float v) { return v * __builtin_amdgcn_rcpf(1.0f + __builtin_amdgcn_exp2f(-1.44269504f * v)); });
  else if (p.act == ACT_RELU) finish([](float v) { return fmaxf(v, 0.0f); });
  else finish([](float v) { return v; });
  }
  };
  epilogue();
  if (!has_next) {
    if (XPF) wait_vm<0>();
    break;
  }
  lin += lin_step;
  first_tile = false;
  }
}

template <typename T, typename OutT, bool CONV, bool M32 = false, bool PH2 = false>
static int launch2p(hipStream_t s, const GemmArgs& p) {
  static bool attr_set = false;
  static int ncu = 0;
  auto kern = gemm2p_kernel<T, OutT, CONV, 0, M32, PH2>;
  if (!attr_set) {
    RVB_HIP_CHECK(hipFuncSetAttribute((const void*)kern, hipFuncAttributeMaxDynamicSharedMemorySize, GEMM2P_LDS));
    if constexpr (!CONV && !M32 && !PH2 && std::is_same<T, bf16_t>::value) {
      RVB_HIP_CHECK(hipFuncSetAttribute((const void*)gemm2p_kernel<T, OutT, false, 1>, hipFuncAttributeMaxDynamicSharedMemorySize, GEMM2P_LDS));
      RVB_HIP_CHECK(hipFuncSetAttribute((const void*)gemm2p_kernel<T, OutT, false, 2>, hipFuncAttributeMaxDynamicSharedMemorySize, GEMM2P_LDS));
    }
    int dev = 0;
    hipDeviceProp_t pr;
    RVB_HIP_CHECK(hipGetDevice(&dev));
    RVB_HIP_CHECK(hipGetDeviceProperties(&pr, dev));
    ncu = pr.multiProcessorCount & ~7;
    attr_set = true;
  }
  const int tiles = cdiv(p.M, B2M) * cdiv(p.N, B2N);
  if constexpr (!CONV && !M32 && !PH2 && std::is_same<T, bf16_t>::value) {
    if ((g_gemm2_flags & (16 | 4096)) && ncu >= 8 && p.M % B2M == 0 && p.N % B2N == 0 && tiles >= 2 * ncu && p.K >= 4 * (ROW2 / 2)) {
      if (g_gemm2_flags & 16) hipLaunchKernelGGL((gemm2p_kernel<T, OutT, false, 1>), dim3(ncu), dim3(512), GEMM2P_LDS, s, p);
      else hipLaunchKernelGGL((gemm2p_kernel<T, OutT, false, 2>), dim3(ncu), dim3(512), GEMM2P_LDS, s, p);
      RVB_HIP_CHECK(hipGetLastError());
      return OK;
    }
  }
  hipLaunchKernelGGL(kern, dim3(tiles), dim3(512), GEMM2P_LDS, s, p);
  RVB_HIP_CHECK(hipGetLastError());
  return OK;
}

template <typename T, typename OutT, bool CONV, bool MMA32 = false>
static int launch2(hipStream_t s, const GemmArgs& p) {
  static bool attr_set = false;
  auto kern = gemm2_kernel<T, OutT, CONV, MMA32>;
  if (!attr_set) {
    RVB_HIP_CHECK(hipFuncSetAttribute((const void*)kern, hipFuncAttributeMaxDynamicSharedMemorySize, GEMM2_LDS));
    attr_set = true;
  }
  const int tiles = cdiv(p.M, B2M) * cdiv(p.N, B2N);
  hipLaunchKernelGGL(kern, dim3(tiles), dim3(512), GEMM2_LDS, s, p);
  RVB_HIP_CHECK(hipGetLastError());
  return OK;
}

bool gemm_glu_supported(int dtype, const GemmArgs& p) {
  return dtype == DT_BF16 && p.act == ACT_GLU && gemm2_applicable(dtype, p) && !p.in_fp8 && !p.out_fp8 && !p.out_f32 && !p.conv && p.res == nullptr &&
         p.rowadd == nullptr && (p.N % 16) == 0 && p.ldc >= p.N / 2 && (p.ldc % 8) == 0 && ((size_t)p.C & 15) == 0 && p.alpha == 1.f;
}

bool gemm2_applicable(int dtype, const GemmArgs& p) {
  if (p.in_fp8 && p.conv) return dtype == DT_BF16 && p.K % 128 == 0 && p.cC % 128 == 0 && p.ldw % 16 == 0 && p.M >= 1 && p.N >= 64 &&
                                 p.act != ACT_LRELU && p.w_scale != nullptr && !p.out_f32 && !p.out_fp8 && p.res == nullptr;
  if (p.in_fp8) return dtype == DT_BF16 && p.K % 128 == 0 && p.lda % 16 == 0 && p.ldw % 16 == 0 && p.M >= 1 && p.N >= 64 &&
                       p.act != ACT_LRELU && p.w_scale != nullptr;
  const int bke = dtype == DT_BF16 ? 64 : 32;
  if (p.K % bke || p.lda % (bke / 8) || p.ldw % (bke / 8)) return false;
  if (p.conv && (p.cC % bke)) return false;
  if (p.M < 128 || p.N < 64 || p.act == ACT_LRELU) return false;
  return true;
}

#ifndef GEMM2_STAGGER_DEFAULT
#define GEMM2_STAGGER_DEFAULT 1
#endif
int g_gemm2_flags = -1, g_gemm2_group_m = -1;
static void gemm2_opts_from_env() {
  if (g_gemm2_flags < 0) { const char* e = lab_env("RVB_GEMM2_FLAGS"); g_gemm2_flags = e ? atoi(e) : GEMM2_DEFAULT_FLAGS; }
  if (g_gemm2_group_m == -1) { const char* e = lab_env("RVB_GEMM2_GROUP_M"); g_gemm2_group_m = e ? atoi(e) : GEMM2_DEFAULT_GROUP_M; }
}

int gemm2(hipStream_t s, int dtype, const GemmArgs& p0) {
  gemm2_opts_from_env();
  GemmArgs p = p0;
  if (p.rowadd && (dtype != DT_BF16 || p.in_fp8 || p.out_f32 || p.out_fp8 || (g_gemm2_flags & (1 | 4)))) {
    set_error("gemm2: the row-periodic addend exists on the phase-interleaved bf16 kernel with bf16 output only");
    return E_UNSUPPORTED;
  }
  if (p.act == ACT_GLU && (!gemm_glu_supported(dtype, p) || (g_gemm2_flags & (1 | 4 | 16 | 4096 | 8192 | 16384)))) {
    set_error("gemm2: ACT_GLU runs on the default phase-interleaved bf16 kernel only (bf16 output, no residual / addend / fp8, N % 16 == 0)");
    return E_UNSUPPORTED;
  }
  p.group_m = g_gemm2_group_m == GROUP_M_AUTO ? (p.K * (p.in_fp8 ? 1 : 2) >= 4096 ? 0 : 8) : g_gemm2_group_m;
  p.prio = (g_gemm2_flags >> 1) & 1;
  p.res_epilogue = ((g_gemm2_flags >> 5) & 1) ^ 1;
  p.fast_epilogue = (g_gemm2_flags & 1024) ? 0 : (1 | ((!(g_gemm2_flags & 2048) || p.K * (p.in_fp8 ? 1 : 2) <= 4096) ? 2 : 0));
  p.k_serp = (g_gemm2_flags & 128) ? 1 : ((g_gemm2_flags & 256) ? (p.N <= 2048 ? 1 : 0) : 0);
  {
    static int mode = -1, ncu = 0;
    if (mode < 0) {
      const char* e = lab_env("RVB_GEMM2_STAGGER"); mode = e ? atoi(e) : GEMM2_STAGGER_DEFAULT;
      int dev = 0; hipDeviceProp_t pr;
      if (hipGetDevice(&dev) == hipSuccess && hipGetDeviceProperties(&pr, dev) == hipSuccess) ncu = pr.multiProcessorCount;
    }
    p.stagger_ticks = 0; p.stagger_first = 0;
    if (mode > 0 && ncu > 0 && p.res != nullptr && p.out_f32 && !p.in_fp8 && dtype == DT_BF16 && !p.conv && (p.fast_epilogue & 2)) {
      const long long tiles = (long long)cdiv(p.M, B2M) * cdiv(p.N, B2N);
      const long long last = tiles % ncu;
      if (tiles > ncu && last > 0 && last <= ncu / 2) {
        const double us = mode > 1 ? (double)mode : 0.5 * (1.4 * (p.K * 2 / ROW2) + 18.0);
        p.stagger_ticks = (int)(us * 100.0);
        p.stagger_first = ncu;
      }
    }
  }
  if (p.in_fp8 && p.conv) return launch2p<fp8_t, bf16_t, true>(s, p);
  if (p.in_fp8 && (g_gemm2_flags & 8)) {
    if (p.out_fp8) return launch2p<fp8_t, fp8_t, false>(s, p);
    if (p.out_f32) return launch2p<fp8_t, float, false>(s, p);
    return launch2p<fp8_t, bf16_t, false>(s, p);
  }
  if (p.in_fp8) {
    if (p.out_fp8) return launch2<fp8_t, fp8_t, false, true>(s, p);
    if (p.out_f32) return launch2<fp8_t, float, false, true>(s, p);
    return launch2<fp8_t, bf16_t, false, true>(s, p);
  }
  if (dtype == DT_BF16) {
    if (g_gemm2_flags & 1) {
      if (p.out_f32) return p.conv ? launch2<bf16_t, float, true, true>(s, p) : launch2<bf16_t, float, false, true>(s, p);
      return p.conv ? launch2<bf16_t, bf16_t, true, true>(s, p) : launch2<bf16_t, bf16_t, false, true>(s, p);
    }
#ifdef RVB_GEMM2_PH2
    if (!(g_gemm2_flags & 4) && (g_gemm2_flags & 16384) && p.res_epilogue) {
      if (p.out_f32) return p.conv ? launch2p<bf16_t, float, true, false, true>(s, p) : launch2p<bf16_t, float, false, false, true>(s, p);
      return p.conv ? launch2p<bf16_t, bf16_t, true, false, true>(s, p) : launch2p<bf16_t, bf16_t, false, false, true>(s, p);
    }
#endif
    if (!(g_gemm2_flags & 4) && (g_gemm2_flags & 8192) && !p.conv) {
      return p.out_f32 ? launch2p<bf16_t, float, false, true>(s, p) : launch2p<bf16_t, bf16_t, false, true>(s, p);
    }
    if (!(g_gemm2_flags & 4)) {
      if (p.out_f32) return p.conv ? launch2p<bf16_t, float, true>(s, p) : launch2p<bf16_t, float, false>(s, p);
      return p.conv ? launch2p<bf16_t, bf16_t, true>(s, p) : launch2p<bf16_t, bf16_t, false>(s, p);
    }
    if (p.out_f32) return p.conv ? launch2<bf16_t, float, true>(s, p) : launch2<bf16_t, float, false>(s, p);
    return p.conv ? launch2<bf16_t, bf16_t, true>(s, p) : launch2<bf16_t, bf16_t, false>(s, p);
  }
  return p.conv ? launch2<float, float, true>(s, p) : launch2<float, float, false>(s, p);
}

}
```

reverb_amd/csrc/kernels.h:

```cpp
#pragma once
#include <vector>
#include "common.h"

namespace rvb {

enum { DT_F32 = 0, DT_BF16 = 1 };
enum { ACT_NONE = 0, ACT_SILU = 1, ACT_RELU = 2, ACT_LRELU = 3  };
enum { ACT_GLU = 4 };

inline size_t dt_size(int dt) { return dt == DT_BF16 ? 2 : 4; }

struct GemmArgs {
  const void* A;
  const void* W;
  const float* bias;
  const float* res;
  void* C;
  int M, N, K;
  int lda, ldw, ldc, ldres;
  float alpha;
  int act;
  int out_f32;
  int conv;
  int cT1, cF1, cT2, cF2, cC;
  int group_m, prio;
  int res_epilogue;
  int fast_epilogue;
  int stagger_ticks, stagger_first;
  int k_serp;
  int in_fp8, out_fp8;
  float a_scale, out_inv_scale;
  const float* w_scale;
  unsigned* sat;
  long long* dbg;
  const void* rowadd;
  int rowadd_rows, rowadd_ld, rowadd_col0, rowadd_cols;
};
int gemm(hipStream_t s, int dtype, const GemmArgs& a);
bool gemm2_applicable(int dtype, const GemmArgs& a);
bool gemm_glu_supported(int dtype, const GemmArgs& a);
int gemm2(hipStream_t s, int dtype, const GemmArgs& a);
extern int g_gemm_variant;
extern int g_gemm2_flags, g_gemm2_group_m;

struct FbankTables {
  const float* window;
  const float* twiddle;
  const float* mel_w;
  const int* mel_lo;
  const int* mel_hi;
};
int fbank(hipStream_t s, const int16_t* pcm, int64_t n_frames, float* feats, const FbankTables& t);
int fbank_f32(hipStream_t s, const float* wave, int64_t n_frames, float* feats, const FbankTables& t);
struct FbankRec {
  int64_t src;
  int64_t row0;
  int32_t is_float;
  int32_t reserved;
};
int fbank_batch(hipStream_t s, const int16_t* pcm, const float* wave, const int64_t* frame0, const FbankRec* rec, int n_rec,
                int64_t total_frames, float* feats, int64_t n_rows, const FbankTables& t);
void resample_taps(int sample_rate, int target, std::vector<float>* ker, int* orig, int* new_, int* width, int* K);
int round_to_i16(hipStream_t s, const float* x, int64_t n, int16_t* out);
int resample(hipStream_t s, const int16_t* pcm, int64_t n_in, const float* ker, int orig, int new_, int width, int K, float* out,
             int64_t n_out);
int resample_f32(hipStream_t s, const float* wave, int64_t n_in, const float* ker, int orig, int new_, int width, int K, float* out,
             int64_t n_out);

int subsample_conv1(hipStream_t s, int dtype, const float* feats, const float* mean, const float* istd,
                    const float* w , const float* b , void* out, int B, int T0, int F0,
                    int d, float out_fp8_scale = 0.f , unsigned* amax = nullptr ,
                    unsigned* sat = nullptr );

enum { NORM_LN = 0, NORM_AFFINE = 1 };
struct NormArgs {
  const float* x;
  int x_bf16 = 0;
  const float* gamma;
  const float* beta;
  float eps;
  int mode;
  int silu;
  const void* add;
  void* out;
  int out_f32;
  int M, d;
  const float* gamma2 = nullptr;
  const float* beta2 = nullptr;
  float eps2 = 0.f;
  void* out2 = nullptr;
  int out_fp8 = 0, out2_fp8 = 0;
  float out_inv_scale = 1.f, out2_inv_scale = 1.f;
  unsigned* sat = nullptr;
  unsigned* sat2 = nullptr;
};
int rownorm(hipStream_t s, int dtype, const NormArgs& a);

struct GluDwArgs {
  const void* G;
  const float* pw1_bias;
  const float* dw_w;
  const float* dw_b;
  const int* lens;
  float* out;
  int B, T, d, K;
  int out_bf16 = 0;
  int gated = 0;
  int causal = 0;
  const void* hist = nullptr;
  int hist_rows = 0;
};
int glu_dwconv(hipStream_t s, int dtype, const GluDwArgs& a);

int embed_tokens(hipStream_t s, const float* E, const float* pe, const int* tok, const int* pos, float* out,
                 int rows, int d, float scale);

int logsoftmax_topk(hipStream_t s, const float* logits, int M, int V, int ld, int k, float blank_penalty,
                    int blank_id, float* topk_val, int* topk_idx, float* logp_out);

int lse_gather(hipStream_t s, const float* logits, int R, int V, int ld, const int* target, float* out, float blank_penalty = 0.f,
               int blank_id = -1);
int lse_gather_multi(hipStream_t s, const float* logits, int R, int V, int ld, const int* ptr, const int* target, float* out);
int row_xent(hipStream_t s, const float* logits, int R, int V, int ld, const int* ptr, const int* target, float* logp, float* lse,
             double* sum_x, int* top1);

int gather_pairs(hipStream_t s, const float* table, size_t ld, const int* row, const int* col, int n, float* out);

int gather_cache(hipStream_t s, const void* src, void* dst, const int* parent, int R, int L, int rows, int row_bytes);

int amax_abs(hipStream_t s, int dtype, const void* x, size_t n, float* slot);

int convert_f32(hipStream_t s, int dtype, const float* src, void* dst, size_t n);

enum { CTC_ALIGN_MAX_TOKENS = 16383,
       CTC_ALIGN_MAX_STATES = 2 * CTC_ALIGN_MAX_TOKENS + 1,
       CTC_ALIGN_MAX_FRAMES = 1 << 20 };
inline int ctc_spt_for(int S) { return S <= 4096 ? 4 : S <= 16384 ? 16 : 32; }
inline int ctc_graph_npt_for(int N) { return N <= 1024 ? 1 : N <= 2048 ? 2 : N <= 4096 ? 4 : 8; }
inline int ctc_threads(int n, int per_thread) { const int t = ((n + per_thread - 1) / per_thread + 63) / 64 * 64; return t < 1024 ? t : 1024; }
struct VitSeq {
  int L, S, T;
  int tok_off;
  int frame_off;
  int f0, f1;
  int pad_;
  long long alpha_off;
  long long bp_off;
  long long bp_stride;
};
int ctc_viterbi_forward(hipStream_t s, const VitSeq* seqs, int n_seq, int max_S, const float* lp, int ld, int r0, const int* rows,
                        const int* tokens, int blank, float* alpha, uint8_t* bp, const float* wmax = nullptr, float bias = 0.f);
int ctc_viterbi_backtrace(hipStream_t s, const VitSeq* seqs, int n_seq, const float* alpha, const uint8_t* bp, int* states, float* score);

enum { CTC_GRAPH_MAX_NODES = 8192,
       CTC_GRAPH_MAX_IN_DEGREE = 64,
       CTC_GRAPH_MAX_ARCS = 32768 };
struct GraphSeq {
  int N, T;
  int index;
  int node_off;
  int arc_off;
  int frame_off;
  int fin_off, n_final;
  int f0, f1;
  long long alpha_off;
  long long bp_off;
  long long bp_stride;
};
constexpr unsigned ARC_SLOT = 0x3fffu, ARC_T = 0x8000u;
int ctc_graph_forward(hipStream_t s, const GraphSeq* seqs, int n_seq, int max_N, const float* lp, int ld, int r0, const int* rows,
                      const int* node_tok, const int* arc_off, const unsigned* arcs, int blank, float* alpha, uint8_t* bp,
                      const float* wmax = nullptr, float bias = 0.f);
int ctc_graph_backtrace(hipStream_t s, const GraphSeq* seqs, int n_seq, const int* arc_off, const unsigned* arcs, const int* finals,
                        const float* alpha, const uint8_t* bp, int* states, float* score);

int ctc_graph_sum_forward(hipStream_t s, const GraphSeq* seqs, int n_seq, int max_N, const float* lp, int ld, int r0, const int* rows,
                          const int* node_tok, const int* arc_off, const unsigned* arcs, const unsigned* rem, int blank, double* alpha,
                          double* csum, float* coff, float* arows);
int ctc_graph_sum_loglik(hipStream_t s, const GraphSeq* seqs, int n_seq, const int* finals, const double* alpha, const double* csum,
// ... 181 lines not shown
```

Before: 27890.

## Defer final LayerNorm output write and fuse normalisation into next layer's FFN GEMM residual

The encoder layer's final LayerNorm no longer writes its normalised fp32 residual stream back to x. It stores only per-row mean/rstd, and the next layer's second macaron-FFN GEMM applies the affine normalisation to the residual in its epilogue. In the last layer the fp32 write is skipped entirely because only the fused second norm output is consumed. This removes one full fp32 write of the residual per layer, at the cost of extra LDS staging and arithmetic in the GEMM epilogue and a smaller residual prefetch ring.

```diff
diff --git a/reverb_amd/_lib.py b/reverb_amd/_lib.py
--- a/reverb_amd/_lib.py
+++ b/reverb_amd/_lib.py
@@ -157,6 +157,13 @@
                 [("sat", C.c_uint32), ("sat2", C.c_uint32)])
 
 
+class NormDeferTestArgs(C.Structure):
+    _fields_ = ([(n, C.c_int32) for n in ("M", "N", "K", "defer")] +
+                [(n, C.c_float) for n in ("eps", "eps2", "alpha")] +
+                [(n, C.c_int32) for n in ("supported", "norm_stats_launches", "norm_skip_launches", "gemm_resnorm_launches", "pad0")] +
+                [(n, _f32p) for n in ("x", "gamma", "beta", "add", "gamma2", "beta2", "A", "W", "bias", "x_mid", "out2", "stats", "x_out")])
+
+
 class GemmTestArgs(C.Structure):
     _fields_ = ([(n, C.c_int32) for n in ("dtype", "M", "N", "K", "lda", "ldw", "ldc", "ldres", "act", "out_f32", "out_fp8", "in_fp8",
                                           "inplace", "a_row0", "c_rows", "conv", "cT1", "cF1", "cC", "cB")] +
@@ -170,6 +177,8 @@
 TEST_SIGNATURES = {
     "rvb_test_gemm_ex": (C.c_int, [C.POINTER(GemmTestArgs)]),
     "rvb_test_rownorm_ex": (C.c_int, [C.POINTER(NormTestArgs)]),
+    "rvb_test_norm_defer": (C.c_int, [C.POINTER(NormDeferTestArgs)]),
+    "rvb_test_norm_defer_counts": (C.c_int, [_i32p, C.c_int]),
     "rvb_test_conv1_ex": (C.c_int, [C.c_int, _f32p, _f32p, _f32p, _f32p, _f32p, _f32p, C.c_int, C.c_int, C.c_int, C.c_int, C.c_float,
                                     _f32p, _u32p]),
     "rvb_test_embed": (C.c_int, [_f32p, C.c_int, _f32p, C.c_int, _i32p, _i32p, _f32p, C.c_int, C.c_int, C.c_float]),
diff --git a/reverb_amd/csrc/common.h b/reverb_amd/csrc/common.h
--- a/reverb_amd/csrc/common.h
+++ b/reverb_amd/csrc/common.h
@@ -144,6 +144,10 @@
   return rows_sum(v);
 }
 
+__device__ inline float ln_affine(float v, float mean, float rstd, float g, float be) {
+  return __builtin_fmaf((v - mean) * rstd, g, be);
+}
+
 inline int cdiv(int64_t a, int64_t b) { return (int)((a + b - 1) / b); }
 
 enum { OK = 0, E_ARG = -1, E_HIP = -2, E_STATE = -3, E_NOMEM = -4, E_UNSUPPORTED = -5, E_TIMEOUT = -7  };
diff --git a/reverb_amd/csrc/elementwise.hip b/reverb_amd/csrc/elementwise.hip
--- a/reverb_amd/csrc/elementwise.hip
+++ b/reverb_amd/csrc/elementwise.hip
@@ -124,8 +124,9 @@
   }
 }
 
-template <typename OutT, typename AddT, int NV, bool TWO, int SW>
+template <typename OutT, typename AddT, int NV, bool TWO, int SW, int DEFER = NORM_DEFER_NONE>
 __global__ __launch_bounds__(256, (NV <= 4 ? 4 : 2)) void rownorm_kernel(NormArgs a) {
+  static_assert(DEFER == NORM_DEFER_NONE || (TWO && sizeof(OutT) == 4 && sizeof(AddT) == 2), "deferred first output: two-stage, fp32, bf16 engine");
   constexpr bool CT = SW >= 0;
   auto wsum = [](float x) __attribute__((always_inline)) { if constexpr (sizeof(AddT) == 2) return wave_sum_dpp(x); else return wave_sum(x); };
   const bool sw_xb = CT ? (bool)(SW & 1) : (bool)a.x_bf16;
@@ -198,6 +199,7 @@
       for (int i = 0; i < NV; ++i)
         asm volatile("" : "+v"(nx[i].x), "+v"(nx[i].y), "+v"(nx[i].z), "+v"(nx[i].w), "+v"(rstd));
     }
+    if constexpr (DEFER == NORM_DEFER_STATS) *(float2*)(a.stats + 2 * (size_t)row) = make_float2(mean, rstd);
     OutT* out = (OutT*)a.out + (size_t)row * d;
     const AddT* add = sw_add ? (const AddT*)a.add + (size_t)row * d : nullptr;
     float sum2 = 0.f;
@@ -205,8 +207,8 @@
     for (int i = 0; i < NV; ++i) {
       const int c = COL(i);
       if (c >= d) continue;
-      float o[4] = {(v[i].x - mean) * rstd * g[i].x + be[i].x, (v[i].y - mean) * rstd * g[i].y + be[i].y,
-                    (v[i].z - mean) * rstd * g[i].z + be[i].z, (v[i].w - mean) * rstd * g[i].w + be[i].w};
+      float o[4] = {ln_affine(v[i].x, mean, rstd, g[i].x, be[i].x), ln_affine(v[i].y, mean, rstd, g[i].y, be[i].y),
+                    ln_affine(v[i].z, mean, rstd, g[i].z, be[i].z), ln_affine(v[i].w, mean, rstd, g[i].w, be[i].w)};
       if (sw_silu) {
 #pragma unroll
         for (int e = 0; e < 4; ++e) {
@@ -224,7 +226,7 @@
           o[0] += u.x; o[1] += u.y; o[2] += u.z; o[3] += u.w;
         }
       }
-      if constexpr (sizeof(OutT) == 4) *(float4*)(out + c) = make_float4(o[0], o[1], o[2], o[3]);
+      if constexpr (sizeof(OutT) == 4 && DEFER == NORM_DEFER_NONE) *(float4*)(out + c) = make_float4(o[0], o[1], o[2], o[3]);
       v[i] = make_float4(o[0], o[1], o[2], o[3]);
       sum2 += o[0] + o[1] + o[2] + o[3];
     }
@@ -262,10 +264,10 @@
         float q[8];
 #pragma unroll
         for (int h = 0; h < 2; ++h) {
-          q[4 * h + 0] = (v[i + h].x - mean2) * rstd2 * g2[i + h].x + be2[i + h].x;
-          q[4 * h + 1] = (v[i + h].y - mean2) * rstd2 * g2[i + h].y + be2[i + h].y;
-          q[4 * h + 2] = (v[i + h].z - mean2) * rstd2 * g2[i + h].z + be2[i + h].z;
-          q[4 * h + 3] = (v[i + h].w - mean2) * rstd2 * g2[i + h].w + be2[i + h].w;
+          q[4 * h + 0] = ln_affine(v[i + h].x, mean2, rstd2, g2[i + h].x, be2[i + h].x);
+          q[4 * h + 1] = ln_affine(v[i + h].y, mean2, rstd2, g2[i + h].y, be2[i + h].y);
+          q[4 * h + 2] = ln_affine(v[i + h].z, mean2, rstd2, g2[i + h].z, be2[i + h].z);
+          q[4 * h + 3] = ln_affine(v[i + h].w, mean2, rstd2, g2[i + h].w, be2[i + h].w);
         }
         if (sw_o2f8) {
           const float qs = a.out2_inv_scale;
@@ -288,10 +290,39 @@
 #undef COL
 }
 
+static thread_local int t_defer_count[2] = {0, 0};
+int rownorm_defer_count(int which, bool reset) {
+  int& c = t_defer_count[which == NORM_DEFER_STATS ? 0 : 1];
+  const int n = c;
+  if (reset) c = 0;
+  return n;
+}
+
 template <typename OutT, typename AddT>
 static void launch_rownorm(hipStream_t s, const NormArgs& a) {
   const int blocks = std::min(cdiv(a.M, 4), 256 * 8);
   const int sw = (a.x_bf16 ? 1 : 0) | (a.mode == NORM_LN ? 2 : 0) | (a.silu ? 4 : 0) | (a.add ? 8 : 0) | (a.out2_fp8 ? 16 : 0);
+  if constexpr (sizeof(OutT) == 4 && sizeof(AddT) == 2) {
+    if (a.defer != NORM_DEFER_NONE) {
+      const bool stats = a.defer == NORM_DEFER_STATS;
+      ++t_defer_count[stats ? 0 : 1];
+#define RVB_NORM_DEFER_CASE(NV_, SW_, DEFER_) \
+      hipLaunchKernelGGL((rownorm_kernel<OutT, AddT, NV_, true, SW_, DEFER_>), dim3(blocks), dim3(256), 0, s, a)
+      if (a.d > 512 && a.d <= 1024 && sw == 2) {
+        if (stats) RVB_NORM_DEFER_CASE(4, 2, NORM_DEFER_STATS); else RVB_NORM_DEFER_CASE(4, 2, NORM_DEFER_SKIP);
+      } else if (a.d > 512 && a.d <= 1024 && sw == (2 | 8) && !stats) {
+        RVB_NORM_DEFER_CASE(4, 2 | 8, NORM_DEFER_SKIP);
+      } else if (a.d <= 512) {
+        if (stats) RVB_NORM_DEFER_CASE(2, -1, NORM_DEFER_STATS); else RVB_NORM_DEFER_CASE(2, -1, NORM_DEFER_SKIP);
+      } else if (a.d <= 1024) {
+        if (stats) RVB_NORM_DEFER_CASE(4, -1, NORM_DEFER_STATS); else RVB_NORM_DEFER_CASE(4, -1, NORM_DEFER_SKIP);
+      } else {
+        if (stats) RVB_NORM_DEFER_CASE(8, -1, NORM_DEFER_STATS); else RVB_NORM_DEFER_CASE(8, -1, NORM_DEFER_SKIP);
+      }
+#undef RVB_NORM_DEFER_CASE
+      return;
+    }
+  }
   if (a.d > 512 && a.d <= 1024) {
 #define RVB_NORM_CASE(TWO_, SW_) \
     if ((a.out2 != nullptr) == (TWO_) && sw == (SW_)) { hipLaunchKernelGGL((rownorm_kernel<OutT, AddT, 4, TWO_, SW_>), dim3(blocks), dim3(256), 0, s, a); return; }
@@ -325,6 +356,14 @@
     set_error("rownorm: the fused second LayerNorm follows a LayerNorm with fp32 output"); return E_ARG;
   }
   if ((a.out_fp8 || a.out2_fp8) && dtype != DT_BF16) { set_error("rownorm: fp8 outputs belong to the bf16 engine"); return E_ARG; }
+  if (a.defer != NORM_DEFER_NONE) {
+    const bool stats = a.defer == NORM_DEFER_STATS;
+    if ((!stats && a.defer != NORM_DEFER_SKIP) || dtype != DT_BF16 || !a.out2 || !a.out_f32 || a.out_fp8 || a.x_bf16 || a.silu ||
+        (stats && (a.add || !a.stats))) {
+      set_error("rownorm: a deferred first output needs the bf16 engine's two-stage form with an fp32 first output (with statistics: no `add`)");
+      return E_ARG;
+    }
+  }
   if (dtype == DT_BF16) {
     if (a.out_fp8) launch_rownorm<fp8_t, bf16_t>(s, a);
     else if (a.out_f32) launch_rownorm<float, bf16_t>(s, a);
diff --git a/reverb_amd/csrc/engine.h b/reverb_amd/csrc/engine.h
--- a/reverb_amd/csrc/engine.h
+++ b/reverb_amd/csrc/engine.h
@@ -273,6 +273,8 @@
   std::vector<int32_t> in_lens, enc_lens;
   rvb::DevBuf d_feats_in, X1, X2, x, xn, y, h, ao, dconv, enc_out, logits, topv, topi;
   rvb::DevBuf d_enc_lens, d_seq_start, d_seq_len, d_aux_i32;
+  rvb::DevBuf x_stats;
+  bool x_deferred = false;
   float* h_topv = nullptr;
   int32_t* h_topi = nullptr;
   size_t h_top_cap = 0;
diff --git a/reverb_amd/csrc/engine.hip b/reverb_amd/csrc/engine.hip
--- a/reverb_amd/csrc/engine.hip
+++ b/reverb_amd/csrc/engine.hip
@@ -67,13 +67,19 @@
   return a + (double)g.N * g.K * es + (g.bias ? 4.0 * g.N : 0.0) + c + (g.res ? 4.0 * (double)g.M * g.N : 0.0);
 }
 
-int run_gemm(rvb_engine* e, const void* A, int lda, const Linear& L, void* C, int ldc, int M, bool out_f32, float alpha,
-             int act, const float* res, int ldres) {
+GemmArgs gemm_args(const rvb_engine* e, const void* A, int lda, const Linear& L, void* C, int ldc, int M, bool out_f32, float alpha,
+                   int act, const float* res, int ldres, const LNorm* res_norm) {
   GemmArgs g;
   memset(&g, 0, sizeof(g));
   g.A = A; g.W = L.w.p; g.bias = L.b.as<float>(); g.res = res; g.C = C;
   g.M = M; g.N = L.out; g.K = L.in; g.lda = lda; g.ldw = L.in; g.ldc = ldc; g.ldres = ldres;
   g.alpha = alpha; g.act = act; g.out_f32 = out_f32 ? 1 : 0;
+  if (res_norm) { g.res_stats = e->x_stats.as<float>(); g.res_gamma = res_norm->g.as<float>(); g.res_beta = res_norm->b.as<float>(); }
+  return g;
+}
+int run_gemm(rvb_engine* e, const void* A, int lda, const Linear& L, void* C, int ldc, int M, bool out_f32, float alpha,
+             int act, const float* res, int ldres, const LNorm* res_norm) {
+  const GemmArgs g = gemm_args(e, A, lda, L, C, ldc, M, out_f32, alpha, act, res, ldres, res_norm);
   Scope sc(e, "gemm", 2.0 * M * (double)L.out * L.in, gemm_alg_bytes(e, g));
   const int rc = gemm(e->stream, e->dtype, g);
   tap_note_gemm(e);
@@ -93,9 +99,14 @@
 }
 int run_norm(rvb_engine* e, const float* x, const LNorm& n, void* out, bool out_f32, int M, int d, int mode,
              int silu, const void* add, const LNorm* second, void* out2, float out8, float out2_8, bool x_bf16, unsigned* sat,
-             unsigned* sat2) {
+             unsigned* sat2, int defer) {
   NormArgs a;
   a.sat = sat; a.sat2 = sat2;
+  a.defer = defer;
+  if (defer == NORM_DEFER_STATS) {
+    if (e->x_stats.bytes < (size_t)M * 2 * 4) { set_error("run_norm: the statistics buffer is smaller than the slice"); return E_STATE; }
+    a.stats = e->x_stats.as<float>();
+  }
   a.x_bf16 = x_bf16 ? 1 : 0;
   a.x = x; a.gamma = n.g.as<float>(); a.beta = n.b.as<float>(); a.eps = n.eps; a.mode = mode; a.silu = silu;
   a.add = add; a.out = out; a.out_f32 = out_f32 ? 1 : 0; a.M = M; a.d = d;
@@ -224,7 +235,7 @@
   (void)hipSetDevice(e->device);
   (void)hipStreamSynchronize(e->stream);
   DevBuf* bufs[] = {&e->cmvn_mean, &e->cmvn_istd, &e->conv1_w, &e->conv1_b, &e->pe_f32, &e->stage, &e->pcm, &e->feats,
-                    &e->d_feats_in, &e->X1, &e->X2, &e->x, &e->xn, &e->y, &e->h, &e->ao, &e->dconv, &e->enc_out,
+                    &e->d_feats_in, &e->X1, &e->X2, &e->x, &e->xn, &e->y, &e->h, &e->ao, &e->dconv, &e->enc_out, &e->x_stats,
                     &e->logits, &e->topv, &e->topi, &e->d_enc_lens, &e->d_seq_start, &e->d_seq_len, &e->d_aux_i32,
                     &e->dx, &e->dxn, &e->dy, &e->dh, &e->dqkv, &e->dq, &e->dao, &e->kvmem, &e->d_tok, &e->d_pos,
                     &e->d_tgt, &e->d_logp, &e->d_hq_start, &e->d_hq_len, &e->d_hkv_start, &e->d_hkv_len,
diff --git a/reverb_amd/csrc/engine_encode.hip b/reverb_amd/csrc/engine_encode.hip
--- a/reverb_amd/csrc/engine_encode.hip
+++ b/reverb_amd/csrc/engine_encode.hip
@@ -8,6 +8,13 @@
 namespace rvb {
 
 static constexpr int GLU_FUSE_DEFAULT = 1;
+static constexpr int NORM_DEFER_DEFAULT = 1;
+
+static GemmArgs ffm2_args(const rvb_engine* e, const EncLayer& L, int M, const LNorm* res_norm) {
+  float* x = e->x.as<float>();
+  const int d = e->cfg.d_model;
+  return gemm_args(e, e->h.p, e->cfg.ffn_dim, L.ffm2, x, d, M, true, 0.5f, ACT_NONE, x, d, res_norm);
+}
 
 static int encoder_layer(rvb_engine* e, EncLayer& L, int lidx, int M, int B, int T, const LNorm& next, void* next_out,
                          float next8 = 0.f, int li = -1) {
@@ -43,6 +50,9 @@
     return cal ? amax_abs(e->stream, e->dtype, t, n, e->d_amax.as<float>() + (size_t)lidx * 8 + slot) : OK;
   };
   auto satp = [&](int slot) -> unsigned* { return e->d_f8sat.p ? e->d_f8sat.as<unsigned>() + (size_t)lidx * 8 + slot : nullptr; };
+  const LNorm* x_norm = e->x_deferred ? &e->enc[lidx - 1].n_final : nullptr;
+  e->x_deferred = false;
+  if (x_norm && (f8_ffm || e->tap_live || li >= 0)) { set_error("encoder_layer: x arrived un-normalised at a block that cannot normalise it"); return E_STATE; }
   if (f8_ffm) {
     RVB_TRY(run_gemm8(e, e->xn.p, d, L.ffm1, e->h.p, ff, M, sc8.in_ffm1, 2, sc8.h_ffm, 1.f, ACT_SILU, nullptr, 0, satp(1)));
     RVB_TRY(run_gemm8(e, e->h.p, ff, L.ffm2, x, d, M, sc8.h_ffm, 1, 1.f, 0.5f, ACT_NONE, x, d));
@@ -51,7 +61,7 @@
     RVB_TRY(run_gemm(e, e->xn.p, d, L.ffm1, e->h.p, ff, M, false, 1.f, ACT_SILU));
     RVB_TRY(note(1, e->h.p, (size_t)M * ff));
     RVB_TRY(tap_keep(e, "h_ffm", e->h.p, (size_t)M * ff, t16));
-    RVB_TRY(run_gemm(e, e->h.p, ff, L.ffm2, x, d, M, true, 0.5f, ACT_NONE, x, d));
+    RVB_TRY(run_gemm(e, e->h.p, ff, L.ffm2, x, d, M, true, 0.5f, ACT_NONE, x, d, x_norm));
   }
   RVB_TRY(tap_keep(e, "x_ffm", x, Md, false));
   if (f8_qkv) {
@@ -204,8 +214,19 @@
     RVB_TRY(run_gemm(e, e->h.p, ff, L.ff2, x, d, M, true, 0.5f, ACT_NONE, x, d));
   }
   RVB_TRY(tap_keep(e, "x_ff", x, Md, false));
+  int defer = NORM_DEFER_NONE;
+  {
+    const char* de = lab_env("RVB_NORM_DEFER");
+    const bool last = lidx + 1 == (int)e->enc.size();
+    if ((de ? atoi(de) : NORM_DEFER_DEFAULT) && e->dtype == DT_BF16 && li < 0 && e->tap_block < 0 && !cal && !(f8 && next8 > 0.f)) {
+      if (last) defer = NORM_DEFER_SKIP;
+      else if (!L.is_lsl && !(f8 && (e->f8_groups[lidx + 1] & 1u)) &&
+               gemm_resnorm_supported(e->dtype, ffm2_args(e, e->enc[lidx + 1], M, &L.n_final))) defer = NORM_DEFER_STATS;
+    }
+  }
   RVB_TRY(run_norm(e, x, L.n_final, x, true, M, d, NORM_LN, 0, L.is_lsl ? e->y.p : nullptr, &next, next_out, 0.f, f8 ? next8 : 0.f, false,
-                   nullptr, (f8 && next8 > 0.f && e->d_f8sat.p) ? e->d_f8sat.as<unsigned>() + (size_t)(lidx + 1) * 8 : nullptr));
+                   nullptr, (f8 && next8 > 0.f && e->d_f8sat.p) ? e->d_f8sat.as<unsigned>() + (size_t)(lidx + 1) * 8 : nullptr, defer));
+  e->x_deferred = defer == NORM_DEFER_STATS;
   RVB_TRY(tap_keep(e, "x_out", x, Md, false));
   RVB_TRY(tap_keep(e, "next", next_out, Md, t16));
   return OK;
@@ -265,6 +286,7 @@
   RVB_TRY(e->X1.ensure((size_t)SB * T1 * F1 * d * es));
   RVB_TRY(e->X2.ensure((size_t)SB * T2 * F2 * d * es));
   RVB_TRY(e->x.ensure((size_t)Ms * d * 4));
+  RVB_TRY(e->x_stats.ensure((size_t)Ms * 2 * 4));
   RVB_TRY(e->xn.ensure((size_t)Ms * d * es));
   RVB_TRY(e->y.ensure((size_t)Ms * d * es));
   RVB_TRY(e->ao.ensure((size_t)Ms * d * es));
@@ -329,6 +351,7 @@
                      (f8 && (e->f8_groups[0] & 1u)) ? e->f8[0].in_ffm1 : 0.f, 0.f, false, e->d_f8sat.as<unsigned>()));
     RVB_TRY(tap_keep(e, "xn0", e->xn.p, (size_t)m * d, t16));
     e->tap_live = false;
+    e->x_deferred = false;
     for (size_t li = 0; li < e->enc.size(); ++li) {
       const bool last = li + 1 == e->enc.size();
       RVB_TRY(encoder_layer(e, e->enc[li], (int)li, m, nb, T2, last ? e->enc_after : e->enc[li + 1].n_ffm, last ? eo : e->xn.p,
@@ -452,6 +475,7 @@
   RVB_TRY(run_gemm(e, e->X2.p, F2 * d, e->embed_out, e->x.p, d, M, true, std::sqrt((float)d)));
   void* eo = (char*)e->enc_out.p + (size_t)st.offset * d * es;
   RVB_TRY(run_norm(e, e->x.as<float>(), e->enc[0].n_ffm, e->xn.p, false, M, d));
+  e->x_deferred = false;
   for (size_t li = 0; li < e->enc.size(); ++li) {
     const bool last = li + 1 == e->enc.size();
     RVB_TRY(encoder_layer(e, e->enc[li], (int)li, M, 1, M, last ? e->enc_after : e->enc[li + 1].n_ffm, last ? eo : e->xn.p, 0.f, (int)li));
diff --git a/reverb_amd/csrc/engine_impl.h b/reverb_amd/csrc/engine_impl.h
--- a/reverb_amd/csrc/engine_impl.h
+++ b/reverb_amd/csrc/engine_impl.h
@@ -25,11 +25,13 @@
 int reset_f8sat(rvb_engine* e);
 double gemm_alg_bytes(const rvb_engine* e, const GemmArgs& g);
 int run_gemm(rvb_engine* e, const void* A, int lda, const Linear& L, void* C, int ldc, int M, bool out_f32,
-             float alpha = 1.f, int act = ACT_NONE, const float* res = nullptr, int ldres = 0);
+             float alpha = 1.f, int act = ACT_NONE, const float* res = nullptr, int ldres = 0, const LNorm* res_norm = nullptr);
+GemmArgs gemm_args(const rvb_engine* e, const void* A, int lda, const Linear& L, void* C, int ldc, int M, bool out_f32, float alpha,
+                   int act, const float* res, int ldres, const LNorm* res_norm);
 int run_norm(rvb_engine* e, const float* x, const LNorm& n, void* out, bool out_f32, int M, int d,
              int mode = NORM_LN, int silu = 0, const void* add = nullptr, const LNorm* second = nullptr,
              void* out2 = nullptr, float out8 = 0.f, float out2_8 = 0.f, bool x_bf16 = false, unsigned* sat = nullptr,
-             unsigned* sat2 = nullptr);
+             unsigned* sat2 = nullptr, int defer = NORM_DEFER_NONE);
 int run_gemm8(rvb_engine* e, const void* A8, int lda, const Linear& L, void* C, int ldc, int M, float a_scale, int out_kind,
               float out_scale = 1.f, float alpha = 1.f, int act = ACT_NONE, const float* res = nullptr, int ldres = 0,
               unsigned* sat = nullptr);
diff --git a/reverb_amd/csrc/gemm.hip b/reverb_amd/csrc/gemm.hip
--- a/reverb_amd/csrc/gemm.hip
+++ b/reverb_amd/csrc/gemm.hip
@@ -181,6 +181,10 @@
     set_error("gemm: the row-periodic addend exists for bf16 operands and bf16 output only");
     return E_UNSUPPORTED;
   }
+  if (p.res_stats && !gemm_resnorm_supported(dtype, p)) {
+    set_error("gemm: res_stats needs the bf16 LDS-DMA kernel with fp32 output (see gemm_resnorm_supported)");
+    return E_UNSUPPORTED;
+  }
   if (p.act == ACT_GLU) {
     if (g_gemm_variant == 1 || !gemm_glu_supported(dtype, p)) { set_error("gemm: ACT_GLU needs the bf16 LDS-DMA kernel (see gemm_glu_supported)"); return E_UNSUPPORTED; }
     t_last_path = 2;
diff --git a/reverb_amd/csrc/gemm2.hip b/reverb_amd/csrc/gemm2.hip
--- a/reverb_amd/csrc/gemm2.hip
+++ b/reverb_amd/csrc/gemm2.hip
@@ -650,10 +650,12 @@
 static constexpr int P_NSLOT = 7, P_HT = 128 * ROW2, P_LEAD = P_NSLOT - 2, P_DEPTH = P_LEAD - 2;
 static constexpr int P_SROW = 64 * 4 + 16;
 static constexpr int GEMM2P_LDS = P_NSLOT * P_HT + 8 * 16 * P_SROW;
-
-template <typename T, typename OutT, bool CONV, int PMODE = 0, bool M32 = false, bool PH2 = false>
+static constexpr int RN_WAVE_LDS = 1024 + 2 * 256;
+
+template <typename T, typename OutT, bool CONV, int PMODE = 0, bool M32 = false, bool PH2 = false, bool RN = false>
 __global__ __launch_bounds__(512) void gemm2p_kernel(GemmArgs p) {
   static_assert(!PH2 || (sizeof(T) == 2 && !M32 && PMODE == 0), "PH2: bf16, 16x16x32 fragments, one tile per workgroup");
+  static_assert(!RN || (std::is_same<T, bf16_t>::value && sizeof(OutT) == 4 && !CONV && PMODE == 0 && !M32 && !PH2), "RN: the encoder's fp32 residual GEMMs");
   static_assert(!M32 || sizeof(T) == 2, "M32 is the bf16 form");
   constexpr bool PERSIST = PMODE != 0;
   constexpr bool XPF = PMODE == 1;
@@ -794,7 +796,7 @@
 
   f32x4_t acc[B32 ? 1 : 8][B32 ? 1 : 4];
   f32x16_t acc32[B32 ? 4 : 1][B32 ? 2 : 1];
-  const bool res_acc = !PH2 && !p.res_epilogue && p.res != nullptr && p.act == ACT_NONE && p.alpha != 0.f && (p.N & 3) == 0 && (p.ldres & 3) == 0 &&
+  const bool res_acc = !PH2 && !RN && !p.res_epilogue && p.res != nullptr && p.act == ACT_NONE && p.alpha != 0.f && (p.N & 3) == 0 && (p.ldres & 3) == 0 &&
                        ((size_t)p.res & 15) == 0;
   if constexpr (PMODE == 2) { s_cur = 0; s_rd = 1; s_st = P_LEAD; }
   if constexpr (PH2) {
@@ -1096,10 +1098,37 @@
       return t;
     };
     const bf16_t* ra_base = (const bf16_t*)p.rowadd + (col0 - p.rowadd_col0);
-    constexpr int RING = sizeof(OutT) == 4 ? 3 : 2, RV = NQ * (CPL / 4);
+    constexpr int RING = (sizeof(OutT) == 4 && !RN) ? 3 : 2, RV = NQ * (CPL / 4);
     float4 rring[RING][RV];
     const bool res_pre = p.res != nullptr && !res_acc && seg_full;
     const int colc = min(col0, p.N - CPL);
+    float2 stv[2];
+    float gbv[2];
+    char* sst = smem + GEMM2P_LDS + wave * RN_WAVE_LDS;
+    if constexpr (RN) {
+#pragma unroll
+      for (int h = 0; h < 2; ++h) stv[h] = *(const float2*)(p.res_stats + 2 * (size_t)min(m0 + wr * 128 + 2 * lane + h, p.M - 1));
+      const int gcol = n0 + wc * 64 + lane;
+      gbv[0] = gcol < p.N ? p.res_gamma[gcol] : 0.0f;
+      gbv[1] = gcol < p.N ? p.res_beta[gcol] : 0.0f;
+    }
+    auto stats_stage = [&]() __attribute__((always_inline)) {
+      if constexpr (RN) {
+        *(float4*)(sst + lane * 16) = make_float4(stv[0].x, stv[0].y, stv[1].x, stv[1].y);
+        *(float*)(sst + 1024 + lane * 4) = gbv[0];
+        *(float*)(sst + 1280 + lane * 4) = gbv[1];
+        __builtin_amdgcn_wave_barrier();
+      }
+    };
+    auto res_norm4 = [&](float4 tt, int i, int q, int c4) __attribute__((always_inline)) -> float4 {
+      if constexpr (RN) {
+        const float2 st = *(const float2*)(sst + (i * 16 + q * RPP + orow) * 8);
+        const float4 g4 = *(const float4*)(sst + 1024 + (ocol + c4 * 4) * 4), b4 = *(const float4*)(sst + 1280 + (ocol + c4 * 4) * 4);
+        tt.x = ln_affine(tt.x, st.x, st.y, g4.x, b4.x); tt.y = ln_affine(tt.y, st.x, st.y, g4.y, b4.y);
+        tt.z = ln_affine(tt.z, st.x, st.y, g4.z, b4.z); tt.w = ln_affine(tt.w, st.x, st.y, g4.w, b4.w);
+      }
+      return tt;
+    };
     auto res_issue = [&](int i, int slot) __attribute__((always_inline)) {
 #pragma unroll
       for (int q = 0; q < NQ; ++q) {
@@ -1114,6 +1143,7 @@
 #pragma unroll
         for (int i = 0; i < RING; ++i) res_issue(i, i);
       }
+      stats_stage();
 #pragma unroll
       for (int i = 0; i < 8; ++i) {
         __builtin_amdgcn_wave_barrier();
@@ -1157,7 +1187,7 @@
             if (res_pre) {
 #pragma unroll
               for (int c4 = 0; c4 < CPL / 4; ++c4) {
-                const float4 tt = rring[i % RING][q * (CPL / 4) + c4];
+                const float4 tt = res_norm4(rring[i % RING][q * (CPL / 4) + c4], i, q, c4);
                 v[c4 * 4 + 0] += tt.x; v[c4 * 4 + 1] += tt.y; v[c4 * 4 + 2] += tt.z; v[c4 * 4 + 3] += tt.w;
               }
             }
@@ -1203,7 +1233,12 @@
           } else {
             for (int e = 0; e < CPL && col0 + e < p.N; ++e) {
               float o = v[e];
+              if constexpr (RN) {
+                const float2 st = *(const float2*)(sst + (i * 16 + srow) * 8);
+                o += ln_affine(p.res[(size_t)row * p.ldres + col0 + e], st.x, st.y, *(const float*)(sst + 1024 + (ocol + e) * 4), *(const float*)(sst + 1280 + (ocol + e) * 4));
+              } else {
               if (p.res && !res_acc) o += p.res[(size_t)row * p.ldres + col0 + e];
+              }
               if constexpr (RA_OK) {
                 if (ra_any && col0 + e >= p.rowadd_col0 && col0 + e < p.rowadd_col0 + p.rowadd_cols)
                   o += bf16_to_f32(ra_base[(size_t)ra_row(i * 16 + srow) * p.rowadd_ld + e]);
@@ -1241,6 +1276,7 @@
 #pragma unroll
         for (int i = 0; i < RING; ++i) res_issue_f(i, i);
       }
+      stats_stage();
 #pragma unroll
       for (int i = 0; i < 8; ++i) {
         __builtin_amdgcn_wave_barrier();
@@ -1280,7 +1316,7 @@
           if constexpr (HR) {
 #pragma unroll
             for (int c4 = 0; c4 < CPL / 4; ++c4) {
-              const float4 tt = rring[i % RING][q * (CPL / 4) + c4];
+              const float4 tt = res_norm4(rring[i % RING][q * (CPL / 4) + c4], i, q, c4);
               v[c4 * 4 + 0] += tt.x; v[c4 * 4 + 1] += tt.y; v[c4 * 4 + 2] += tt.z; v[c4 * 4 + 3] += tt.w;
             }
           }
@@ -1460,6 +1496,35 @@
   return OK;
 }
 
+static int launch2p_resnorm(hipStream_t s, const GemmArgs& p) {
+  static bool attr_set = false;
+  constexpr int LDS = GEMM2P_LDS + 8 * RN_WAVE_LDS;
+  static_assert(LDS <= 160 * 1024, "gemm2p RN: LDS");
+  auto kern = gemm2p_kernel<bf16_t, float, false, 0, false, false, true>;
+  if (!attr_set) {
+    RVB_HIP_CHECK(hipFuncSetAttribute((const void*)kern, hipFuncAttributeMaxDynamicSharedMemorySize, LDS));
+    attr_set = true;
+  }
+  const int tiles = cdiv(p.M, B2M) * cdiv(p.N, B2N);
+  hipLaunchKernelGGL(kern, dim3(tiles), dim3(512), LDS, s, p);
+  RVB_HIP_CHECK(hipGetLastError());
+  return OK;
+}
+
+static void gemm2_opts_from_env();
+bool gemm_resnorm_supported(int dtype, const GemmArgs& p) {
+  gemm2_opts_from_env();
+  return dtype == DT_BF16 && g_gemm_variant != 1 && gemm2_applicable(dtype, p) && !p.in_fp8 && !p.out_fp8 && p.out_f32 && !p.conv &&
+         p.act != ACT_GLU && p.res != nullptr && p.rowadd == nullptr && (p.N % 4) == 0 && (p.ldc % 4) == 0 && (p.ldres % 4) == 0 &&
+         ((size_t)p.C & 15) == 0 && ((size_t)p.res & 15) == 0 && !(g_gemm2_flags & (1 | 4 | 16 | 32 | 4096 | 8192 | 16384));
+}
+static thread_local int t_resnorm_count = 0;
+int gemm_resnorm_count(bool reset) {
+  const int n = t_resnorm_count;
+  if (reset) t_resnorm_count = 0;
+  return n;
+}
+
 bool gemm_glu_supported(int dtype, const GemmArgs& p) {
   return dtype == DT_BF16 && p.act == ACT_GLU && gemm2_applicable(dtype, p) && !p.in_fp8 && !p.out_fp8 && !p.out_f32 && !p.conv && p.res == nullptr &&
          p.rowadd == nullptr && (p.N % 16) == 0 && p.ldc >= p.N / 2 && (p.ldc % 8) == 0 && ((size_t)p.C & 15) == 0 && p.alpha == 1.f;
@@ -1497,6 +1562,10 @@
     set_error("gemm2: ACT_GLU runs on the default phase-interleaved bf16 kernel only (bf16 output, no residual / addend / fp8, N % 16 == 0)");
     return E_UNSUPPORTED;
   }
+  if (p.res_stats && (!gemm_resnorm_supported(dtype, p) || !p.res_gamma || !p.res_beta)) {
+    set_error("gemm2: res_stats runs on the default phase-interleaved bf16 kernel only (fp32 output, aligned residual; see gemm_resnorm_supported)");
+    return E_UNSUPPORTED;
+  }
   p.group_m = g_gemm2_group_m == GROUP_M_AUTO ? (p.K * (p.in_fp8 ? 1 : 2) >= 4096 ? 0 : 8) : g_gemm2_group_m;
   p.prio = (g_gemm2_flags >> 1) & 1;
   p.res_epilogue = ((g_gemm2_flags >> 5) & 1) ^ 1;
@@ -1545,6 +1614,7 @@
     if (!(g_gemm2_flags & 4) && (g_gemm2_flags & 8192) && !p.conv) {
       return p.out_f32 ? launch2p<bf16_t, float, false, true>(s, p) : launch2p<bf16_t, bf16_t, false, true>(s, p);
     }
+    if (p.res_stats) { ++t_resnorm_count; return launch2p_resnorm(s, p); }
     if (!(g_gemm2_flags & 4)) {
       if (p.out_f32) return p.conv ? launch2p<bf16_t, float, true>(s, p) : launch2p<bf16_t, float, false>(s, p);
       return p.conv ? launch2p<bf16_t, bf16_t, true>(s, p) : launch2p<bf16_t, bf16_t, false>(s, p);
diff --git a/reverb_amd/csrc/kernels.h b/reverb_amd/csrc/kernels.h
--- a/reverb_amd/csrc/kernels.h
+++ b/reverb_amd/csrc/kernels.h
@@ -35,10 +35,15 @@
   long long* dbg;
   const void* rowadd;
   int rowadd_rows, rowadd_ld, rowadd_col0, rowadd_cols;
+  const float* res_stats;
+  const float* res_gamma;
+  const float* res_beta;
 };
 int gemm(hipStream_t s, int dtype, const GemmArgs& a);
 bool gemm2_applicable(int dtype, const GemmArgs& a);
 bool gemm_glu_supported(int dtype, const GemmArgs& a);
+bool gemm_resnorm_supported(int dtype, const GemmArgs& a);
+int gemm_resnorm_count(bool reset);
 int gemm2(hipStream_t s, int dtype, const GemmArgs& a);
 extern int g_gemm_variant;
 extern int g_gemm2_flags, g_gemm2_group_m;
@@ -93,8 +98,12 @@
   float out_inv_scale = 1.f, out2_inv_scale = 1.f;
   unsigned* sat = nullptr;
   unsigned* sat2 = nullptr;
-};
+  int defer = 0;
+  float* stats = nullptr;
+};
+enum { NORM_DEFER_NONE = 0, NORM_DEFER_STATS = 1, NORM_DEFER_SKIP = 2 };
 int rownorm(hipStream_t s, int dtype, const NormArgs& a);
+int rownorm_defer_count(int which, bool reset);
 
 struct GluDwArgs {
   const void* G;
```

After: 28090, median of 6. Within noise of the previous version (+0.7%).
